# Glaciohound/Chimera-ST

Measured on AMD Instinct MI355X. Metric: train utterances/sec, MuST-C EN-DE s2t_transformer_m, 1/2/4/8 MI355X, higher is better.
Workload: dtype bf16

## Files before the change

chimera-st_amd/csrc/gemm.hip:

```cpp
#include "gemm_common.h"
#include <vector>
#include <stdlib.h>
#include <string.h>
#include <type_traits>

namespace {
using namespace cstg;

template <int BM_, int BN_, int WM_, int WN_, int KV_ = 8>
struct Cfg {
  static constexpr int BM = BM_, BN = BN_, WM = WM_, WN = WN_, NT = 64 * WM_ * WN_, TM = BM_ / WM_ / 32, TN = BN_ / WN_ / 32;
  static constexpr int KV = KV_;
  static_assert(BM_ <= GEMM_MAX_BM && GEMM_MAX_BM % BM_ == 0, "conv0.hip (cst_conv_row_limits) sizes live frames from GEMM_MAX_BM");
};
using CfgSmall = Cfg<128, 128, 2, 2>;
using CfgSkinny = Cfg<64, 64, 2, 2>;
using CfgNarrowN = Cfg<128, 64, 2, 2>;
using CfgNarrowM = Cfg<64, 128, 2, 2>;
using CfgLarge = Cfg<256, 256, 4, 4>;

template <typename T, bool A_KMAJOR, bool B_KMAJOR, bool SEG, typename C, bool CS = false>
__global__ __launch_bounds__(C::NT) void gemm_kernel(GemmParams p) {
  constexpr int BM = C::BM, BN = C::BN, NTHREADS = C::NT, TM = C::TM, TN = C::TN;
  constexpr int VEC = DT<T>::VEC;
  constexpr int KV = C::KV, BK = KV * VEC;
  constexpr int LDK = BK + VEC;
  constexpr int LDMA = sizeof(T) == 2 ? BM + 32 : BM + VEC;
  constexpr int LDMB = sizeof(T) == 2 ? BN + 32 : BN + VEC;
  constexpr int A_ELEMS = A_KMAJOR ? BM * LDK : BK * LDMA;
  constexpr int B_ELEMS = B_KMAJOR ? BN * LDK : BK * LDMB;
  constexpr int MVA = BM / VEC, MVB = BN / VEC;
  constexpr int NVA = BM * KV / NTHREADS, NVB = BN * KV / NTHREADS;
  extern __shared__ __attribute__((aligned(16))) char smem_raw[];
  T* smem = reinterpret_cast<T*>(smem_raw);
  constexpr int STAGE = A_ELEMS + B_ELEMS;

  const int tid = threadIdx.x, lane = tid & 63, wave = tid >> 6;
  const int wm = wave / C::WN, wn = wave % C::WN;

  const int ntiles = p.tiles_m * p.tiles_n;
  int tm, tn, z;
  if (p.split_order) {
    const int total = ntiles * p.splits, L = (int)blockIdx.x + (int)gridDim.x * (int)blockIdx.z;
    const int q = total / 8, r = total % 8, xcd = L % 8, loc = L / 8;
    const int item = (xcd < r ? xcd * (q + 1) : r * (q + 1) + (xcd - r) * q) + loc;
    z = item / ntiles;
    const int t = item % ntiles;
    tm = t / p.tiles_n;
    tn = t % p.tiles_n;
  } else {
    int id = blockIdx.x;
    {
      const int q = ntiles / 8, r = ntiles % 8, xcd = id % 8, loc = id / 8;
      id = (xcd < r ? xcd * (q + 1) : r * (q + 1) + (xcd - r) * q) + loc;
    }
    constexpr int GROUP_M = 8;
    const int per_group = GROUP_M * p.tiles_n;
    const int grp = id / per_group, rem = id % per_group;
    const int gm0 = grp * GROUP_M;
    const int gsz = (p.tiles_m - gm0 < GROUP_M) ? (p.tiles_m - gm0) : GROUP_M;
    tm = gm0 + rem % gsz;
    tn = rem / gsz;
    z = blockIdx.z;
  }
  const int64_t m0 = (int64_t)tm * BM, n0 = (int64_t)tn * BN;

  const int split = z % p.splits;
  const int64_t bidx = z / p.splits;
  const int64_t b0 = bidx / p.batch1, b1 = bidx % p.batch1;
  const T* A = (const T*)p.A + b0 * p.sa0 + b1 * p.sa1;
  const T* B = (const T*)p.B + b0 * p.sb0 + b1 * p.sb1;
  const int64_t cofs = b0 * p.sc0 + b1 * p.sc1;
  const int64_t bofs = b0 * p.sbias0 + b1 * p.sbias1;

  int ktiles = (int)((p.K + BK - 1) / BK);
  const int kfull = (int)(p.K / BK);
  if (p.k_len) {
    typedef const __attribute__((address_space(4))) int32_t* cptr_t;
    const int kl = ((cptr_t)p.k_len)[b0];
    const int live = kl <= 0 ? 0 : (kl + BK - 1) / BK;
    ktiles = live < ktiles ? live : ktiles;
  }
  const int per = (ktiles + p.splits - 1) / p.splits;
  const int kt0 = split * per;
  const int kt1 = (kt0 + per < ktiles) ? kt0 + per : ktiles;

  u32x4 ra[NVA], rb[NVB];
  const T* pa[NVA];
  const T* pb[NVB];
  int ka[NVA], kb[NVB];
  int aq[NVA], ar[NVA], bq[NVB], br[NVB];
#pragma unroll
  for (int i = 0; i < NVA; ++i) {
    const int v = tid + NTHREADS * i;
    if (A_KMAJOR) {
      int64_t row = m0 + v / KV;
      row = row < p.M ? row : p.M - 1;
      ka[i] = kt0 * BK + (v % KV) * VEC;
      if (SEG && p.a_seg) { aq[i] = ka[i] / (int)p.a_seg; ar[i] = ka[i] % (int)p.a_seg; pa[i] = A + row * p.lda; }
      else { aq[i] = 0; ar[i] = 0; pa[i] = A + row * p.lda + ka[i]; }
    } else {
      int64_t m = m0 + (int64_t)(v % MVA) * VEC;
      m = m < p.M ? m : p.M - VEC;
      ka[i] = kt0 * BK + v / MVA;
      aq[i] = 0; ar[i] = 0;
      pa[i] = A + (int64_t)ka[i] * p.lda + segaddr(m, p.a_seg, p.a_seg_stride);
    }
  }
#pragma unroll
  for (int i = 0; i < NVB; ++i) {
    const int v = tid + NTHREADS * i;
    if (B_KMAJOR) {
      int64_t row = n0 + v / KV;
      row = row < p.N ? row : p.N - 1;
      kb[i] = kt0 * BK + (v % KV) * VEC;
      if (SEG && p.b_seg) { bq[i] = kb[i] / (int)p.b_seg; br[i] = kb[i] % (int)p.b_seg; pb[i] = B + row * p.ldb; }
      else { bq[i] = 0; br[i] = 0; pb[i] = B + row * p.ldb + kb[i]; }
    } else {
      int64_t n = n0 + (int64_t)(v % MVB) * VEC;
      n = n < p.N ? n : p.N - VEC;
      kb[i] = kt0 * BK + v / MVB;
      bq[i] = 0; br[i] = 0;
      pb[i] = B + (int64_t)kb[i] * p.ldb + segaddr(n, p.b_seg, p.b_seg_stride);
    }
  }
  const int64_t step_a = A_KMAJOR ? (int64_t)BK : (int64_t)BK * p.lda;
  const int64_t step_b = B_KMAJOR ? (int64_t)BK : (int64_t)BK * p.ldb;

  auto load_tile = [&](auto tail_tag) {
    constexpr bool TAIL = decltype(tail_tag)::value;
    const u32x4 zero = {0, 0, 0, 0};
#pragma unroll
    for (int i = 0; i < NVA; ++i) {
      const T* qa = pa[i];
      if (SEG && A_KMAJOR && p.a_seg) qa = pa[i] + (int64_t)aq[i] * p.a_seg_stride + ar[i];
      if (TAIL) {
        const bool oka = ka[i] < p.K;
        const u32x4 va = *reinterpret_cast<const u32x4*>(oka ? qa : A);
        ra[i] = oka ? va : zero;
      } else {
        ra[i] = *reinterpret_cast<const u32x4*>(qa);
      }
      ka[i] += BK;
      if (SEG && A_KMAJOR && p.a_seg) { ar[i] += BK; while (ar[i] >= (int)p.a_seg) { ar[i] -= (int)p.a_seg; ++aq[i]; } }
      else pa[i] += step_a;
    }
#pragma unroll
    for (int i = 0; i < NVB; ++i) {
      const T* qb = pb[i];
      if (SEG && B_KMAJOR && p.b_seg) qb = pb[i] + (int64_t)bq[i] * p.b_seg_stride + br[i];
      if (TAIL) {
        const bool okb = kb[i] < p.K;
        const u32x4 vb = *reinterpret_cast<const u32x4*>(okb ? qb : B);
        rb[i] = okb ? vb : zero;
      } else {
        rb[i] = *reinterpret_cast<const u32x4*>(qb);
      }
      kb[i] += BK;
      if (SEG && B_KMAJOR && p.b_seg) { br[i] += BK; while (br[i] >= (int)p.b_seg) { br[i] -= (int)p.b_seg; ++bq[i]; } }
      else pb[i] += step_b;
    }
  };
  auto load_any = [&](int kt) {
    if (kt < kfull) load_tile(std::false_type{});
    else load_tile(std::true_type{});
  };
  static_assert(!CS || (!A_KMAJOR && NTHREADS % MVA == 0), "a thread must stage the same columns of an mn-major A in every vector");
  const bool do_cs = CS && tn == 0;
  float cs[VEC];
#pragma unroll
  for (int e = 0; e < VEC; ++e) cs[e] = 0.0f;
  auto store_tile = [&](int buf) {
#pragma unroll
    for (int i = 0; i < NVA; ++i) {
      const int v = tid + NTHREADS * i;
      T* da = smem + buf * STAGE + (A_KMAJOR ? (v / KV) * LDK + (v % KV) * VEC : (v / MVA) * LDMA + (v % MVA) * VEC);
      *reinterpret_cast<u32x4*>(da) = ra[i];
      if (CS && do_cs) {
        if (sizeof(T) == 2) {
#pragma unroll
          for (int e = 0; e < 4; ++e) {
            cs[2 * e] += __uint_as_float(ra[i][e] << 16);
            cs[2 * e + 1] += __uint_as_float(ra[i][e] & 0xffff0000u);
          }
        } else {
#pragma unroll
          for (int e = 0; e < 4; ++e) cs[e] += __uint_as_float(ra[i][e]);
        }
      }
    }
#pragma unroll
    for (int i = 0; i < NVB; ++i) {
      const int v = tid + NTHREADS * i;
      T* db = smem + buf * STAGE + A_ELEMS + (B_KMAJOR ? (v / KV) * LDK + (v % KV) * VEC : (v / MVB) * LDMB + (v % MVB) * VEC);
      *reinterpret_cast<u32x4*>(db) = rb[i];
    }
  };

  f32x16 acc[TM][TN];
#pragma unroll
  for (int i = 0; i < TM; ++i)
#pragma unroll
    for (int j = 0; j < TN; ++j)
#pragma unroll
      for (int r = 0; r < 16; ++r) acc[i][j][r] = 0.0f;

  constexpr int KLIST_MAX = 1000;
  __shared__ int klist[KLIST_MAX];
  __shared__ int klist_n;
  const bool kskip = !SEG && BK == 64 && p.k_live != nullptr && per <= KLIST_MAX;
  int nk = kt1 > kt0 ? kt1 - kt0 : 0;
  if (kskip) {
    if (wave == 0) {
      int total = 0;
      for (int base = 0; base < ktiles; base += 64) {
        const int kt = base + lane;
        total += __builtin_popcountll(__builtin_amdgcn_ballot_w64(kt < ktiles && p.k_live[kt] == p.k_epoch));
      }
      const int lo = (int)(((int64_t)total * split) / p.splits), hi = (int)(((int64_t)total * (split + 1)) / p.splits);
      int seen = 0, n = 0;
      for (int base = 0; base < ktiles && seen < hi; base += 64) {
        const int kt = base + lane;
        const bool live = kt < ktiles && p.k_live[kt] == p.k_epoch;
        const uint64_t m = __builtin_amdgcn_ballot_w64(live);
        const int idx = seen + __builtin_popcountll(m & ((1ull << lane) - 1ull));
        if (live && idx >= lo && idx < hi) klist[idx - lo] = kt;
        seen += __builtin_popcountll(m);
      }
      n = hi - lo;
      if (lane == 0) klist_n = n;
    }
    __syncthreads();
    nk = klist_n;
  }
  if (p.m_live) {
    typedef const __attribute__((address_space(4))) uint32_t* cptr_t;
    cptr_t ml = (cptr_t)p.m_live;
    const int t0 = (int)(m0 >> 6), t1 = (int)((((m0 + BM < p.M) ? m0 + BM : p.M) + 63) >> 6);
    bool live = false;
    for (int t = t0; t < t1; ++t) live |= ml[t] == p.m_epoch;
    if (!live) nk = 0;
  }
  if (p.m_len) {
    typedef const __attribute__((address_space(4))) int32_t* cptr_t;
    if (m0 >= (int64_t)((cptr_t)p.m_len)[b0]) nk = 0;
  }
  int pos = kt0;
  auto fetch = [&](int kt) {
    const int d = kt - pos;
    if (d) {
#pragma unroll
      for (int i = 0; i < NVA; ++i) { pa[i] += (int64_t)d * step_a; ka[i] += d * BK; }
#pragma unroll
      for (int i = 0; i < NVB; ++i) { pb[i] += (int64_t)d * step_b; kb[i] += d * BK; }
    }
    load_any(kt);
    pos = kt + 1;
  };
  auto tile_at = [&](int it) { return kskip ? klist[it] : kt0 + it; };

  if (nk > 0) {
    fetch(tile_at(0));
    store_tile(0);
  }
  __syncthreads();
  int cur = 0;
  const int lrow = lane & 31, lk = 8 * (lane >> 5);
  constexpr int WROWS = TM * 32, WCOLS = TN * 32;
  for (int it = 0; it < nk; ++it) {
    const bool more = it + 1 < nk;
    if (more) fetch(tile_at(it + 1));
    const T* sa = smem + cur * STAGE;
    const T* sb = sa + A_ELEMS;
#pragma unroll
    for (int kk = 0; kk < BK; kk += 16) {
      Frag<T> fa[TM], fb[TN];
#pragma unroll
      for (int i = 0; i < TM; ++i) {
        if (A_KMAJOR) frag_load_contig(fa[i], sa + (wm * WROWS + i * 32 + lrow) * LDK + kk + lk);
        else frag_load_tr(fa[i], sa, LDMA, wm * WROWS + i * 32, kk + lk, kk + lk + 4, lane);
      }
#pragma unroll
      for (int j = 0; j < TN; ++j) {
        if (B_KMAJOR) frag_load_contig(fb[j], sb + (wn * WCOLS + j * 32 + lrow) * LDK + kk + lk);
        else frag_load_tr(fb[j], sb, LDMB, wn * WCOLS + j * 32, kk + lk, kk + lk + 4, lane);
      }
#pragma unroll
      for (int i = 0; i < TM; ++i)
#pragma unroll
        for (int j = 0; j < TN; ++j) mma16(acc[i][j], fa[i], fb[j]);
    }
    if (more) store_tile(cur ^ 1);
    __syncthreads();
    cur ^= 1;
  }

  if (CS && do_cs) {
    float* red = reinterpret_cast<float*>(smem_raw);
#pragma unroll
    for (int e = 0; e < VEC; ++e) red[(tid / MVA) * BM + (tid % MVA) * VEC + e] = cs[e];
    __syncthreads();
    if (tid < BM && m0 + tid < p.M) {
      float tot = 0.0f;
      for (int r = 0; r < NTHREADS / MVA; ++r) tot += red[r * BM + tid];
      if (p.splits > 1) p.colsum_ws[((int64_t)bidx * p.splits + split) * p.M + m0 + tid] = tot;
      else DT<T>::st((T*)p.colsum + bidx * p.M + m0 + tid, tot);
    }
  }

  constexpr int LDC = BN + 4;
  constexpr int VPR = BN / 8;
  constexpr int NPASS = BM / 64;
  constexpr int ITERS = 64 * VPR / NTHREADS;
  float* stage = reinterpret_cast<float*>(smem_raw);
  float* wsp = p.splits > 1 ? p.ws + ((int64_t)z) * p.M * p.N : nullptr;
  const bool ws_vec = (p.N % 4) == 0;
#pragma unroll
  for (int ps = 0; ps < NPASS; ++ps) {
    __syncthreads();
#pragma unroll
    for (int i = 0; i < TM; ++i) {
      const int trow = wm * WROWS + i * 32;
      if (trow / 64 == ps) {
#pragma unroll
        for (int j = 0; j < TN; ++j)
#pragma unroll
          for (int r = 0; r < 16; ++r)
            stage[(trow - 64 * ps + acc_row(r, lane)) * LDC + wn * WCOLS + j * 32 + lrow] = acc[i][j][r];
      }
    }
    __syncthreads();
#pragma unroll 2
    for (int it = 0; it < ITERS; ++it) {
      const int v = tid + NTHREADS * it;
      const int rl = v / VPR, cl = (v % VPR) * 8;
      const int64_t row = m0 + 64 * ps + rl, col = n0 + cl;
      if (row >= p.M || col >= p.N) continue;
      float x[8];
      {
        const f32x4 a = *reinterpret_cast<const f32x4*>(stage + rl * LDC + cl);
        const f32x4 b = *reinterpret_cast<const f32x4*>(stage + rl * LDC + cl + 4);
        x[0] = a[0]; x[1] = a[1]; x[2] = a[2]; x[3] = a[3]; x[4] = b[0]; x[5] = b[1]; x[6] = b[2]; x[7] = b[3];
      }
      const bool full = col + 8 <= p.N;
      if (wsp) {
        if (full && ws_vec) store8(wsp + row * p.N + col, x);
        else
          for (int e = 0; e < 8 && col + e < p.N; ++e) wsp[row * p.N + col + e] = x[e];
      } else if (full && p.vec_epi) {
        epilogue_store8<T>(p, cofs, bofs, row, col, x);
      } else {
        for (int e = 0; e < 8 && col + e < p.N; ++e) epilogue_store<T>(p, cofs, bofs, row, col + e, x[e]);
      }
    }
  }
}

template <int N>
__device__ __forceinline__ void wait_vmcnt() { asm volatile("s_waitcnt vmcnt(%0)" ::"n"(N) : "memory"); }

template <typename T, bool A_KMAJOR, bool B_KMAJOR, typename C, int NS>
__global__ __launch_bounds__(C::NT) void gemm_glds_kernel(GemmParams p) {
  constexpr int BM = C::BM, BN = C::BN, NTHREADS = C::NT, TM = C::TM, TN = C::TN, NWAVES = C::NT / 64;
  constexpr int ES = sizeof(T), VEC = DT<T>::VEC, BK = 128 / ES;
  constexpr int A_BYTES = A_KMAJOR ? BM * 128 : BK * BM * ES;
  constexpr int B_BYTES = B_KMAJOR ? BN * 128 : BK * BN * ES;
  constexpr int STAGE_BYTES = A_BYTES + B_BYTES;
  constexpr int GA = A_BYTES / 1024 / NWAVES, GB = B_BYTES / 1024 / NWAVES;
  extern __shared__ __attribute__((aligned(16))) char smem_raw[];

  const int tid = threadIdx.x, lane = tid & 63, wave = tid >> 6;
  const int wm = wave / C::WN, wn = wave % C::WN;
  const int ntiles = p.tiles_m * p.tiles_n;
  int id = blockIdx.x;
  {
    const int q = ntiles / 8, r = ntiles % 8, xcd = id % 8, loc = id / 8;
    id = (xcd < r ? xcd * (q + 1) : r * (q + 1) + (xcd - r) * q) + loc;
  }
  constexpr int GROUP_M = 8;
  int tm, tn;
  {
    const int per_group = GROUP_M * p.tiles_n;
    const int grp = id / per_group, rem = id % per_group;
    const int gm0 = grp * GROUP_M;
    const int gsz = (p.tiles_m - gm0 < GROUP_M) ? (p.tiles_m - gm0) : GROUP_M;
    tm = gm0 + rem % gsz;
    tn = rem / gsz;
  }
  const int64_t m0 = (int64_t)tm * BM, n0 = (int64_t)tn * BN;
  const int z = blockIdx.z;
  const int split = z % p.splits;
  const int64_t bidx = z / p.splits;
  const int64_t b0 = bidx / p.batch1, b1 = bidx % p.batch1;
  const T* A = (const T*)p.A + b0 * p.sa0 + b1 * p.sa1;
  const T* B = (const T*)p.B + b0 * p.sb0 + b1 * p.sb1;
  const int64_t cofs = b0 * p.sc0 + b1 * p.sc1;
  const int64_t bofs = b0 * p.sbias0 + b1 * p.sbias1;
  const int ktiles = (int)((p.K + BK - 1) / BK);
  const int kfull = (int)(p.K / BK);
  const int per = (ktiles + p.splits - 1) / p.splits;
  const int kt0 = split * per;
  const int kt1 = (kt0 + per < ktiles) ? kt0 + per : ktiles;
  int nt = kt1 - kt0;
  if (p.m_len) {
    typedef const __attribute__((address_space(4))) int32_t* cptr_t;
    if (m0 >= (int64_t)((cptr_t)p.m_len)[b0]) nt = 0;
  }

  const T* pa[GA];
  const T* pb[GB];
  int ka[GA], kb[GB];
#pragma unroll
  for (int i = 0; i < GA; ++i) {
    const int g = wave + NWAVES * i;
    if (A_KMAJOR) {
      const int r = 8 * g + (lane >> 3), c = (lane & 7) ^ ((r >> 1) & 7);
      int64_t row = m0 + r;
      row = row < p.M ? row : p.M - 1;
      ka[i] = kt0 * BK + c * VEC;
      pa[i] = A + row * p.lda + ka[i];
    } else {
      constexpr int RB = BM * ES, RPG = 1024 / RB > 0 ? 1024 / RB : 1, CPR = RB / 16;
      const int kl = g * RPG + (lane * 16) / RB, pc = ((lane * 16) % RB) / 16;
      const int c = ES == 2 ? (pc ^ (4 * (kl & 3))) : pc;
      int64_t m = m0 + (int64_t)c * VEC;
      m = m < p.M ? m : p.M - VEC;
      ka[i] = kt0 * BK + kl;
      pa[i] = A + (int64_t)ka[i] * p.lda + segaddr(m, p.a_seg, p.a_seg_stride);
      (void)CPR;
    }
  }
#pragma unroll
  for (int i = 0; i < GB; ++i) {
    const int g = wave + NWAVES * i;
    if (B_KMAJOR) {
      const int r = 8 * g + (lane >> 3), c = (lane & 7) ^ ((r >> 1) & 7);
      int64_t row = n0 + r;
      row = row < p.N ? row : p.N - 1;
      kb[i] = kt0 * BK + c * VEC;
      pb[i] = B + row * p.ldb + kb[i];
    } else {
      constexpr int RB = BN * ES, RPG = 1024 / RB > 0 ? 1024 / RB : 1;
      const int kl = g * RPG + (lane * 16) / RB, pc = ((lane * 16) % RB) / 16;
      const int c = ES == 2 ? (pc ^ (4 * (kl & 3))) : pc;
      int64_t n = n0 + (int64_t)c * VEC;
      n = n < p.N ? n : p.N - VEC;
      kb[i] = kt0 * BK + kl;
      pb[i] = B + (int64_t)kb[i] * p.ldb + segaddr(n, p.b_seg, p.b_seg_stride);
    }
  }
  const int64_t step_a = A_KMAJOR ? (int64_t)BK : (int64_t)BK * p.lda;
  const int64_t step_b = B_KMAJOR ? (int64_t)BK : (int64_t)BK * p.ldb;

  auto issue = [&](int kt, int stage) {
    char* sbase = smem_raw + stage * STAGE_BYTES;
    if (kt < kfull) {
#pragma unroll
      for (int i = 0; i < GA; ++i) {
        __builtin_amdgcn_global_load_lds((const __attribute__((address_space(1))) void*)pa[i],
                                         (__attribute__((address_space(3))) void*)(sbase + (wave + NWAVES * i) * 1024), 16, 0, 0);
        pa[i] += step_a;
        ka[i] += BK;
      }
#pragma unroll
      for (int i = 0; i < GB; ++i) {
        __builtin_amdgcn_global_load_lds((const __attribute__((address_space(1))) void*)pb[i],
                                         (__attribute__((address_space(3))) void*)(sbase + A_BYTES + (wave + NWAVES * i) * 1024), 16, 0, 0);
        pb[i] += step_b;
        kb[i] += BK;
      }
    } else {
      const u32x4 zero = {0, 0, 0, 0};
#pragma unroll
      for (int i = 0; i < GA; ++i) {
        const bool ok = ka[i] < p.K;
        const u32x4 v = *reinterpret_cast<const u32x4*>(ok ? pa[i] : A);
        *reinterpret_cast<u32x4*>(sbase + (wave + NWAVES * i) * 1024 + lane * 16) = ok ? v : zero;
        pa[i] += step_a;
        ka[i] += BK;
      }
#pragma unroll
      for (int i = 0; i < GB; ++i) {
        const bool ok = kb[i] < p.K;
        const u32x4 v = *reinterpret_cast<const u32x4*>(ok ? pb[i] : B);
        *reinterpret_cast<u32x4*>(sbase + A_BYTES + (wave + NWAVES * i) * 1024 + lane * 16) = ok ? v : zero;
        pb[i] += step_b;
        kb[i] += BK;
      }
    }
  };

  f32x16 acc[TM][TN];
#pragma unroll
  for (int i = 0; i < TM; ++i)
#pragma unroll
    for (int j = 0; j < TN; ++j)
#pragma unroll
      for (int r = 0; r < 16; ++r) acc[i][j][r] = 0.0f;

  const int lrow = lane & 31, hi = lane >> 5;
  constexpr int WROWS = TM * 32, WCOLS = TN * 32;
  constexpr int G = GA + GB;

#pragma unroll
  for (int s = 0; s < NS - 1; ++s)
    if (s < nt) issue(kt0 + s, s);

  constexpr bool PIN = NTHREADS == 256 && TM == 4 && NS == 2 && A_KMAJOR && B_KMAJOR && sizeof(T) == 2;
// ... 28 lines not shown
        if (f < TM) frag_load_kswz(fa[buf][f], sa, wm * WROWS + f * 32 + lrow, kk * 16 + 8 * hi);
        else frag_load_kswz(fb[buf][f - TM], sb, wn * WCOLS + (f - TM) * 32 + lrow, kk * 16 + 8 * hi);
      };
#pragma unroll
      for (int f = 0; f < NFR; ++f) read_one(f, 0, 0);
      __builtin_amdgcn_sched_barrier(0);
#pragma unroll
      for (int kk = 0; kk < 4; ++kk) {
#pragma unroll
        for (int sl = 0; sl < NSLOT; ++sl) {
#pragma unroll
          for (int u = 0; u < 2; ++u) {
            const int m = 2 * sl + u, i = m / TN, j = m % TN;
            mma16(acc[i][j], fb[kk & 1][j], fa[kk & 1][i]);
          }
          if (kk < 3) {
            if (sl < NFR) read_one(sl, kk + 1, (kk + 1) & 1);
            if (sl == 0 && NFR > NSLOT) {
#pragma unroll
              for (int f = NSLOT; f < NFR; ++f) read_one(f, kk + 1, (kk + 1) & 1);
            }
          }
          if (kk * NSLOT + sl < G && dma_ok) issue_one(kk * NSLOT + sl, nbase);
          __builtin_amdgcn_sched_barrier(0);
        }
      }
    }
  } else
  for (int it = 0; it < nt; ++it) {
    const int issued = (it + NS - 1 < nt) ? it + NS - 1 : nt;
    if (NS > 2 && issued - it - 1 == NS - 2) wait_vmcnt<(NS - 2) * G>();
    else wait_vmcnt<0>();
    __builtin_amdgcn_s_barrier();
    if (it + NS - 1 < nt) issue(kt0 + it + NS - 1, (it + NS - 1) % NS);
    const char* sbase = smem_raw + (it % NS) * STAGE_BYTES;
    const T* sa = reinterpret_cast<const T*>(sbase);
    const T* sb = reinterpret_cast<const T*>(sbase + A_BYTES);
#pragma unroll
    for (int kk = 0; kk < BK; kk += 16) {
      Frag<T> fa[TM], fb[TN];
#pragma unroll
      for (int i = 0; i < TM; ++i) {
        if (A_KMAJOR) {
          const int r = wm * WROWS + i * 32 + lrow;
          frag_load_kswz(fa[i], sa, r, kk + 8 * hi);
        } else {
          frag_load_tr_swz(fa[i], sa, BM, wm * WROWS + i * 32, kk + 8 * hi, lane);
        }
      }
#pragma unroll
      for (int j = 0; j < TN; ++j) {
        if (B_KMAJOR) {
          const int r = wn * WCOLS + j * 32 + lrow;
          frag_load_kswz(fb[j], sb, r, kk + 8 * hi);
        } else {
          frag_load_tr_swz(fb[j], sb, BN, wn * WCOLS + j * 32, kk + 8 * hi, lane);
        }
      }
#pragma unroll
      for (int i = 0; i < TM; ++i)
#pragma unroll
        for (int j = 0; j < TN; ++j) mma16(acc[i][j], fa[i], fb[j]);
    }
  }

  float* wsp = p.splits > 1 ? p.ws + ((int64_t)z) * p.M * p.N : nullptr;
  const bool ws_vec = (p.N % 4) == 0;
  if constexpr (PIN) {
    constexpr int LDW = WCOLS + 4, VPRW = WCOLS / 8, RITER = 32 * VPRW / 64;
    static_assert(4 * 32 * LDW * 4 <= NS * STAGE_BYTES && (32 * VPRW) % 64 == 0, "the four waves' images live in the stage buffers");
    __syncthreads();
    float* img = reinterpret_cast<float*>(smem_raw) + wave * (32 * LDW);
#pragma unroll
    for (int i = 0; i < TM; ++i) {
#pragma unroll
      for (int j = 0; j < TN; ++j)
#pragma unroll
        for (int q = 0; q < 4; ++q) {
          const f32x4 v = {acc[i][j][4 * q], acc[i][j][4 * q + 1], acc[i][j][4 * q + 2], acc[i][j][4 * q + 3]};
          *reinterpret_cast<f32x4*>(img + lrow * LDW + j * 32 + 8 * q + 4 * hi) = v;
        }
#pragma unroll 2
      for (int tv = 0; tv < RITER; ++tv) {
        const int v = tv * 64 + lane;
        const int rl = v / VPRW, cl = (v % VPRW) * 8;
        const int64_t row = m0 + wm * WROWS + i * 32 + rl, col = n0 + wn * WCOLS + cl;
        if (row >= p.M || col >= p.N) continue;
        float x[8];
        {
          const f32x4 a = *reinterpret_cast<const f32x4*>(img + rl * LDW + cl);
          const f32x4 b = *reinterpret_cast<const f32x4*>(img + rl * LDW + cl + 4);
          x[0] = a[0]; x[1] = a[1]; x[2] = a[2]; x[3] = a[3]; x[4] = b[0]; x[5] = b[1]; x[6] = b[2]; x[7] = b[3];
        }
        const bool full = col + 8 <= p.N;
        if (wsp) {
          if (full && ws_vec) store8(wsp + row * p.N + col, x);
          else
            for (int e = 0; e < 8 && col + e < p.N; ++e) wsp[row * p.N + col + e] = x[e];
        } else if (full && p.vec_epi) {
          epilogue_store8<T>(p, cofs, bofs, row, col, x);
        } else {
          for (int e = 0; e < 8 && col + e < p.N; ++e) epilogue_store<T>(p, cofs, bofs, row, col + e, x[e]);
        }
      }
    }
    return;
  }
  constexpr int LDC = BN + 4;
  constexpr int VPR = BN / 8;
  constexpr int NPASS = BM / 64;
  constexpr int ITERS = 64 * VPR / NTHREADS;
  float* stage = reinterpret_cast<float*>(smem_raw);
#pragma unroll
  for (int ps = 0; ps < NPASS; ++ps) {
    __syncthreads();
#pragma unroll
    for (int i = 0; i < TM; ++i) {
      const int trow = wm * WROWS + i * 32;
      if (trow / 64 == ps) {
#pragma unroll
        for (int j = 0; j < TN; ++j)
#pragma unroll
          for (int r = 0; r < 16; ++r)
            stage[(trow - 64 * ps + acc_row(r, lane)) * LDC + wn * WCOLS + j * 32 + lrow] = acc[i][j][r];
      }
    }
    __syncthreads();
#pragma unroll 2
    for (int itv = 0; itv < ITERS; ++itv) {
      const int v = tid + NTHREADS * itv;
      const int rl = v / VPR, cl = (v % VPR) * 8;
      const int64_t row = m0 + 64 * ps + rl, col = n0 + cl;
      if (row >= p.M || col >= p.N) continue;
      float x[8];
      {
        const f32x4 a = *reinterpret_cast<const f32x4*>(stage + rl * LDC + cl);
        const f32x4 b = *reinterpret_cast<const f32x4*>(stage + rl * LDC + cl + 4);
        x[0] = a[0]; x[1] = a[1]; x[2] = a[2]; x[3] = a[3]; x[4] = b[0]; x[5] = b[1]; x[6] = b[2]; x[7] = b[3];
      }
      const bool full = col + 8 <= p.N;
      if (wsp) {
        if (full && ws_vec) store8(wsp + row * p.N + col, x);
        else
          for (int e = 0; e < 8 && col + e < p.N; ++e) wsp[row * p.N + col + e] = x[e];
      } else if (full && p.vec_epi) {
        epilogue_store8<T>(p, cofs, bofs, row, col, x);
      } else {
        for (int e = 0; e < 8 && col + e < p.N; ++e) epilogue_store<T>(p, cofs, bofs, row, col + e, x[e]);
      }
    }
  }
}

template <typename T>
__global__ void splitk_reduce_kernel(GemmParams p) {
  const int64_t total = p.M * p.N;
  const int64_t bidx = blockIdx.y;
  const int64_t b0 = bidx / p.batch1, b1 = bidx % p.batch1;
  const int64_t cofs = b0 * p.sc0 + b1 * p.sc1;
  const int64_t bofs = b0 * p.sbias0 + b1 * p.sbias1;
  const float* ws = p.ws + bidx * p.splits * total;
  if (p.colsum) {
    for (int64_t m = (int64_t)blockIdx.x * blockDim.x + threadIdx.x; m < p.M; m += (int64_t)gridDim.x * blockDim.x) {
      float v = 0.0f;
      for (int s = 0; s < p.splits; ++s) v += p.colsum_ws[(bidx * p.splits + s) * p.M + m];
      DT<T>::st((T*)p.colsum + bidx * p.M + m, v);
    }
  }
  if (p.vec_epi && (p.N % 8) == 0) {
    const int64_t total8 = total >> 3;
    for (int64_t i8 = (int64_t)blockIdx.x * blockDim.x + threadIdx.x; i8 < total8; i8 += (int64_t)gridDim.x * blockDim.x) {
      const float* src = ws + i8 * 8;
      float v[8] = {0.0f, 0.0f, 0.0f, 0.0f, 0.0f, 0.0f, 0.0f, 0.0f};
      int sp = 0;
      for (; sp + 4 <= p.splits; sp += 4) {
        f32x4 a[4][2];
#pragma unroll
        for (int u = 0; u < 4; ++u) {
          a[u][0] = *reinterpret_cast<const f32x4*>(src + (int64_t)(sp + u) * total);
          a[u][1] = *reinterpret_cast<const f32x4*>(src + (int64_t)(sp + u) * total + 4);
        }
#pragma unroll
        for (int u = 0; u < 4; ++u)
#pragma unroll
          for (int e = 0; e < 4; ++e) { v[e] += a[u][0][e]; v[4 + e] += a[u][1][e]; }
      }
      for (; sp < p.splits; ++sp) {
        const f32x4 a0 = *reinterpret_cast<const f32x4*>(src + (int64_t)sp * total), a1 = *reinterpret_cast<const f32x4*>(src + (int64_t)sp * total + 4);
#pragma unroll
        for (int e = 0; e < 4; ++e) { v[e] += a0[e]; v[4 + e] += a1[e]; }
      }
      const int64_t i = i8 * 8, row = i / p.N;
      epilogue_store8<T>(p, cofs, bofs, row, i - row * p.N, v);
    }
    return;
  }
  for (int64_t i = (int64_t)blockIdx.x * blockDim.x + threadIdx.x; i < total; i += (int64_t)gridDim.x * blockDim.x) {
    float v = 0.0f;
    for (int s = 0; s < p.splits; ++s) v += ws[s * total + i];
    epilogue_store<T>(p, cofs, bofs, i / p.N, i % p.N, v);
  }
}

template <typename T, bool AK, bool BK_, bool SEG, typename C>
int launch(GemmParams p, int64_t M, int64_t N, int64_t nbatch, hipStream_t s) {
  constexpr int VEC = DT<T>::VEC;
  constexpr int BKc = C::KV * VEC, LDK = BKc + VEC;
  constexpr int LDMA = sizeof(T) == 2 ? C::BM + 32 : C::BM + VEC, LDMB = sizeof(T) == 2 ? C::BN + 32 : C::BN + VEC;
  constexpr int A_ELEMS = AK ? C::BM * LDK : BKc * LDMA;
  constexpr int B_ELEMS = BK_ ? C::BN * LDK : BKc * LDMB;
  size_t lds = 2 * (size_t)(A_ELEMS + B_ELEMS) * sizeof(T);
  const size_t stage_bytes = (size_t)64 * (C::BN + 4) * sizeof(float);
  if (lds < stage_bytes) lds = stage_bytes;
  static bool attr_set = false;
  if (!attr_set) {
    (void)hipFuncSetAttribute(reinterpret_cast<const void*>(&gemm_kernel<T, AK, BK_, SEG, C>), hipFuncAttributeMaxDynamicSharedMemorySize, 160 * 1024 - 4096);
    attr_set = true;
  }
  p.tiles_m = (int)cst_ceil_div(M, C::BM);
  p.tiles_n = (int)cst_ceil_div(N, C::BN);
  p.split_order = (p.splits > 1 && nbatch == 1) ? 1 : 0;
  dim3 grid(p.tiles_m * p.tiles_n, 1, (unsigned)(nbatch * p.splits));
  if constexpr (!AK && !BK_ && !SEG && C::NT <= 256) {
    if (p.colsum) {
      static bool attr_cs = false;
      if (!attr_cs) {
        (void)hipFuncSetAttribute(reinterpret_cast<const void*>(&gemm_kernel<T, AK, BK_, SEG, C, true>), hipFuncAttributeMaxDynamicSharedMemorySize, 160 * 1024 - 4096);
        attr_cs = true;
      }
      hipLaunchKernelGGL((gemm_kernel<T, AK, BK_, SEG, C, true>), grid, dim3(C::NT), lds, s, p);
      return cst_check_launch("cst_gemm");
    }
  }
  if (p.colsum) { cst_set_error("cst_gemm: internal: column sums requested from a configuration that does not build them"); return CST_ERR_UNSUPPORTED; }
  hipLaunchKernelGGL((gemm_kernel<T, AK, BK_, SEG, C>), grid, dim3(C::NT), lds, s, p);
  return cst_check_launch("cst_gemm");
}

template <typename T, bool AK, bool BK_, typename C, int NS>
int launch_glds(GemmParams p, int64_t M, int64_t N, int64_t nbatch, hipStream_t s) {
  constexpr int ES = sizeof(T), BKc = 128 / ES;
  constexpr int A_BYTES = AK ? C::BM * 128 : BKc * C::BM * ES, B_BYTES = BK_ ? C::BN * 128 : BKc * C::BN * ES;
  size_t lds = (size_t)NS * (A_BYTES + B_BYTES);
  const size_t stage_bytes = (size_t)64 * (C::BN + 4) * sizeof(float);
  if (lds < stage_bytes) lds = stage_bytes;
  static bool attr_set = false;
  if (!attr_set) {
    (void)hipFuncSetAttribute(reinterpret_cast<const void*>(&gemm_glds_kernel<T, AK, BK_, C, NS>), hipFuncAttributeMaxDynamicSharedMemorySize, 160 * 1024);
    attr_set = true;
  }
  p.tiles_m = (int)cst_ceil_div(M, C::BM);
  p.tiles_n = (int)cst_ceil_div(N, C::BN);
  dim3 grid(p.tiles_m * p.tiles_n, 1, (unsigned)(nbatch * p.splits));
  hipLaunchKernelGGL((gemm_glds_kernel<T, AK, BK_, C, NS>), grid, dim3(C::NT), lds, s, p);
  return cst_check_launch("cst_gemm");
}


struct GemmSwitches {
  bool no_klive;
  int group_m;
  bool no_narrow;
  bool no_4w;
  bool experiment;
  const char* force_cfg;
};

GemmSwitches gemm_switches() {
  static const GemmSwitches once = [] {
    GemmSwitches w;
    w.no_klive = getenv("CST_GEMM_NO_KLIVE") != nullptr;
    const char* gm = getenv("CST_GEMM8P_GROUP_M");
    w.group_m = gm && atoi(gm) > 0 ? atoi(gm) : 4;
    w.no_narrow = getenv("CST_GEMM_NO_NARROW") != nullptr;
    w.no_4w = getenv("CST_GEMM_NO_4W") != nullptr;
    w.experiment = getenv("CST_GEMM_EXPERIMENT") != nullptr;
    w.force_cfg = nullptr;
    return w;
  }();
  GemmSwitches w = once;
  if (w.experiment) {
    const char* f = getenv("CST_GEMM_FORCE_CFG");
    w.force_cfg = f && *f ? f : nullptr;
  }
  return w;
}

enum class Family { Reg, Dma, Persistent8, FourWave };
enum class Tile { Small, Large, Skinny, NarrowN, NarrowM, Big4, Big4N, Unknown };
enum class Colsum { None, Fused, Separate };
using CfgBig4 = Cfg<256, 256, 2, 2>;
using CfgBig4N = Cfg<256, 192, 2, 2>;

struct GemmRoute {
  Family family;
  Tile tile;
  bool bf16, ak, bk;
  bool seg;
  int stages;
  int splits;
  Colsum colsum;
};

struct TileDims { int bm, bn, nt; };
template <typename C> constexpr TileDims dims_of() { return {C::BM, C::BN, C::NT}; }
constexpr TileDims kTileDims[] = {dims_of<CfgSmall>(),   dims_of<CfgLarge>(), dims_of<CfgSkinny>(), dims_of<CfgNarrowN>(),
                                  dims_of<CfgNarrowM>(), dims_of<CfgBig4>(),  dims_of<CfgBig4N>(),  {0, 0, 0}};

bool use_large(const cst_gemm_desc* d, bool seg, int splits) {
  if (seg) return false;
  const int64_t tiles = cst_ceil_div(d->M, 256) * cst_ceil_div(d->N, 256) * d->batch0 * d->batch1 * splits;
  return d->M >= 256 && d->N >= 256 && tiles >= 200;
}

int choose_splits(const cst_gemm_desc* d) {
  if (d->split_k > 1) return d->split_k;
  if (d->split_k == 0 || d->split_k == 1) return 1;
  const int bk = d->dtype == CST_BF16 ? 64 : 32;
  const int64_t ktiles = cst_ceil_div(d->K, bk);
  const int64_t nb = d->batch0 * d->batch1;
  if (d->M >= 256 && d->N >= 256) {
    const int64_t tl = cst_ceil_div(d->M, 256) * cst_ceil_div(d->N, 256) * nb;
    if (tl >= 200) return 1;
    int64_t s = 256 / tl;
    if (s > ktiles / 16) s = ktiles / 16;
    if (s > 32) s = 32;
    if (s >= 1 && tl * s >= 200) return (int)s;
  }
  const int64_t tiles = cst_ceil_div(d->M, 128) * cst_ceil_div(d->N, 128) * nb;
  if (tiles >= 256 || ktiles < 16) return 1;
  const int64_t cap = ktiles / 8 < 32 ? ktiles / 8 : 32;
  int64_t s1 = 256 / tiles, s2 = 512 / tiles;
  if (s1 > cap) s1 = cap;
  if (s2 > cap) s2 = cap;
  if (s1 < 1) s1 = 1;
  if (s2 < 1) s2 = 1;
  const int64_t s = (2.0 / (double)s2 < 0.9 / (double)s1) ? s2 : s1;
  return (int)s;
}

struct Forced { const char* name; bool kk; Family family; Tile tile; int stages; };
const Forced kForced[] = {
    {"small", false, Family::Reg, Tile::Small, 0},     {"narrowm", false, Family::Reg, Tile::NarrowM, 0},
    {"narrown", false, Family::Reg, Tile::NarrowN, 0}, {"skinny", false, Family::Reg, Tile::Skinny, 0},
    {"large", false, Family::Reg, Tile::Large, 0},     {"big4r", false, Family::Reg, Tile::Big4, 0},
    {"skinny4", true, Family::Dma, Tile::Skinny, 4},   {"skinny2", true, Family::Dma, Tile::Skinny, 2},
    {"small2", true, Family::Dma, Tile::Small, 2},     {"small3", true, Family::Dma, Tile::Small, 3},
    {"big4", true, Family::Dma, Tile::Big4, 2},        {"big4n", true, Family::Dma, Tile::Big4N, 2},
    {"big4r", true, Family::Reg, Tile::Big4, 0},       {"large", true, Family::Reg, Tile::Large, 0},
    {"8p", true, Family::Persistent8, Tile::Large, 0}, {"4w", true, Family::FourWave, Tile::Big4N, 0},
};

GemmRoute gemm_route(const cst_gemm_desc* d, const GemmParams& p, const GemmSwitches& sw) {
  GemmRoute r;
  r.bf16 = d->dtype == CST_BF16;
  r.ak = d->a_kmajor != 0;
  r.bk = d->b_kmajor != 0;
  r.seg = (r.ak && d->a_seg) || (r.bk && d->b_seg);
  r.stages = 2;
  r.splits = choose_splits(d);
  const bool kk = r.ak && r.bk, mm = !r.ak && !r.bk;
  const bool large = use_large(d, r.seg, r.splits);
  const int64_t nbatch = d->batch0 * d->batch1;
  r.colsum = !d->colsum ? Colsum::None : (mm && !d->a_seg && !d->b_seg && !large) ? Colsum::Fused : Colsum::Separate;
  auto take = [&r](Family f, Tile t, int stages = 2) { r.family = f; r.tile = t; r.stages = stages; return r; };

  if (!sw.no_narrow && !r.seg && !large && kk && d->N <= 64 && d->M > 256) return take(Family::Dma, Tile::NarrowN);
  if (!sw.no_narrow && !r.seg && !large && mm && d->M <= 64 && d->N > 256) return take(Family::Reg, Tile::NarrowM);

  GemmParams q = p;
  q.splits = r.splits;
  const bool unsplit1 = !r.seg && nbatch == 1 && r.splits == 1;
  if (sw.force_cfg && r.bf16 && !r.seg && nbatch == 1 && (mm || (kk && r.splits == 1))) {
    for (const Forced& f : kForced) {
      if (f.kk != kk || strcmp(f.name, sw.force_cfg) != 0) continue;
      if (f.family == Family::Persistent8 && !cst_gemm8p_supported(q, r.ak, r.bk, nbatch)) break;
      if (f.family == Family::FourWave && !cst_gemm4w_supported(q, r.ak, r.bk, nbatch)) break;
      return take(f.family, f.tile, f.stages);
    }
    return take(Family::Reg, Tile::Unknown);
  }

  const bool mid8p = kk && unsplit1 && d->M >= 256 && d->N >= 256 && cst_ceil_div(d->M, 256) * cst_ceil_div(d->N, 256) >= 150;
  if (kk && unsplit1 && (d->M <= 256 || (!large && !mid8p && cst_ceil_div(d->M, 128) * cst_ceil_div(d->N, 128) < 256))) {
    const bool two_stage = d->M > 256 && cst_ceil_div(d->M, 64) * cst_ceil_div(d->N, 64) > 512;
    return take(Family::Dma, Tile::Skinny, two_stage ? 2 : 4);
  }
  if (r.bf16 && !r.seg && !d->colsum) {
    if (!sw.no_4w && cst_gemm4w_supported(q, r.ak, r.bk, nbatch)) return take(Family::FourWave, Tile::Big4N);
    if (r.ak && (!d->dact || (!d->resid && !d->aux_out)) && (large || mid8p) && cst_gemm8p_supported(q, r.ak, r.bk, nbatch))
      return take(Family::Persistent8, Tile::Large);
  }
  const Tile t = large ? Tile::Large : Tile::Small;
  if (r.seg) return take(Family::Reg, Tile::Small);
  return take(kk && !d->colsum ? Family::Dma : Family::Reg, t);
}

void route_text(const GemmRoute& r, char* out, int64_t n) {
  const TileDims t = kTileDims[(int)r.tile];
  const char* dt = r.bf16 ? "bf16" : "f32";
  const char a = r.ak ? 'k' : 'm', b = r.bk ? 'k' : 'm';
  switch (r.family) {
    case Family::Reg:
      snprintf(out, (size_t)n, "reg %s %c%c%s %dx%d nt%d%s split%d", dt, a, b, r.seg ? " seg" : "", t.bm, t.bn, t.nt,
               r.colsum == Colsum::Fused ? " colsum" : "", r.splits);
      break;
    case Family::Dma: snprintf(out, (size_t)n, "glds %s %c%c %dx%d nt%d ns%d split%d", dt, a, b, t.bm, t.bn, t.nt, r.stages, r.splits); break;
    case Family::Persistent8: snprintf(out, (size_t)n, "8p %c%c", a, b); break;
    case Family::FourWave: snprintf(out, (size_t)n, "4w"); break;
  }
}

}

extern "C" int64_t cst_colsum_workspace(int64_t rows, int64_t cols);
extern "C" int cst_colsum_typed(const void* x, int64_t ldx, void* out, void* workspace, int64_t rows, int64_t cols, int dtype, int out_dtype, cst_stream stream);
extern "C" int cst_colsum_typed_live(const void* x, int64_t ldx, void* out, void* workspace, int64_t rows, int64_t cols, int dtype, int out_dtype,
                                     const uint32_t* row_live, uint32_t epoch, cst_stream stream);

namespace {

int validate(const cst_gemm_desc* d) {
  CST_REQUIRE(d && d->A && d->B && d->C, "cst_gemm: null operand");
  CST_REQUIRE(d->dtype == CST_F32 || d->dtype == CST_BF16, "cst_gemm: bad dtype %d", d->dtype);
  CST_REQUIRE(d->c_dtype == d->dtype || d->c_dtype == CST_F32, "cst_gemm: c_dtype must be dtype or f32");
  CST_REQUIRE(d->M > 0 && d->N > 0 && d->K > 0, "cst_gemm: empty problem M=%lld N=%lld K=%lld", (long long)d->M,
              (long long)d->N, (long long)d->K);
  const int vec = d->dtype == CST_BF16 ? 8 : 4;
  if (d->a_kmajor) CST_REQUIRE(d->K % vec == 0 && d->lda % vec == 0, "cst_gemm: k-major A needs K,lda %% %d == 0 (K=%lld lda=%lld)", vec, (long long)d->K, (long long)d->lda);
  else CST_REQUIRE(d->M % vec == 0 && d->lda % vec == 0, "cst_gemm: mn-major A needs M,lda %% %d == 0 (M=%lld lda=%lld)", vec, (long long)d->M, (long long)d->lda);
  if (d->b_kmajor) CST_REQUIRE(d->K % vec == 0 && d->ldb % vec == 0, "cst_gemm: k-major B needs K,ldb %% %d == 0 (K=%lld ldb=%lld)", vec, (long long)d->K, (long long)d->ldb);
  else CST_REQUIRE(d->N % vec == 0 && d->ldb % vec == 0, "cst_gemm: mn-major B needs N,ldb %% %d == 0 (N=%lld ldb=%lld)", vec, (long long)d->N, (long long)d->ldb);
  CST_REQUIRE(d->a_seg % vec == 0 && d->b_seg % vec == 0 && d->a_seg_stride % vec == 0 && d->b_seg_stride % vec == 0,
              "cst_gemm: segment sizes must be multiples of %d", vec);
  CST_REQUIRE(((uintptr_t)d->A % 16 == 0) && ((uintptr_t)d->B % 16 == 0), "cst_gemm: A/B must be 16-byte aligned");
  CST_REQUIRE(d->sa0 % vec == 0 && d->sa1 % vec == 0 && d->sb0 % vec == 0 && d->sb1 % vec == 0, "cst_gemm: batch strides of A/B must be multiples of %d", vec);
  CST_REQUIRE(d->batch0 >= 1 && d->batch1 >= 1, "cst_gemm: batch counts must be >= 1");
  CST_REQUIRE(!d->dact || d->aux_in, "cst_gemm: dact needs aux_in");
  CST_REQUIRE(d->drop_p >= 0.0f && d->drop_p < 1.0f, "cst_gemm: drop_p must be in [0, 1)");
  CST_REQUIRE(d->drop_p == 0.0f || d->batch0 * d->batch1 == 1, "cst_gemm: fused dropout needs an unbatched problem");
  CST_REQUIRE(!d->colsum || (!d->a_kmajor && !d->a_seg), "cst_gemm: colsum needs an mn-major, unsegmented A");
  return CST_OK;
}

GemmParams fill_params(const cst_gemm_desc* d, const GemmSwitches& sw) {
  GemmParams p;
  p.M = d->M; p.N = d->N; p.K = d->K;
  p.A = d->A; p.lda = d->lda; p.a_seg = d->a_seg; p.a_seg_stride = d->a_seg_stride;
  p.B = d->B; p.ldb = d->ldb; p.b_seg = d->b_seg; p.b_seg_stride = d->b_seg_stride;
  p.C = d->C; p.ldc = d->ldc;
  p.bias = d->bias; p.bias_mode = d->bias ? d->bias_mode : CST_BIAS_NONE; p.sbias0 = d->sbias0; p.sbias1 = d->sbias1;
  p.act = d->act;
  p.aux_out = d->aux_out; p.ld_aux_out = d->ld_aux_out;
  p.dact = d->dact; p.aux_in = d->aux_in; p.ld_aux_in = d->ld_aux_in;
  p.resid = d->resid; p.ld_resid = d->ld_resid;
  p.alpha = d->alpha;
  p.drop_thr = d->drop_p > 0.0f ? cst_drop_thr16(d->drop_p) : 0u;
  p.drop_key = d->drop_key;
  p.drop_scale = d->drop_p > 0.0f ? 1.0f / (1.0f - d->drop_p) : 1.0f;
  p.drop_row0 = 0;
  p.batch1 = d->batch1;
  p.sa0 = d->sa0; p.sa1 = d->sa1; p.sb0 = d->sb0; p.sb1 = d->sb1; p.sc0 = d->sc0; p.sc1 = d->sc1;
  p.c_f32 = (d->c_dtype == CST_F32 && d->dtype != CST_F32) ? 1 : 0;
  {
    auto al16 = [](const void* q) { return q == nullptr || ((uintptr_t)q % 16) == 0; };
    bool ok = d->ldc % 8 == 0 && d->sc0 % 8 == 0 && d->sc1 % 8 == 0 && al16(d->C) && al16(d->bias) && al16(d->aux_out) && al16(d->aux_in) && al16(d->resid);
    if (d->bias && d->bias_mode == CST_BIAS_COL) ok = ok && d->sbias0 % 8 == 0 && d->sbias1 % 8 == 0;
    if (d->aux_out) ok = ok && d->ld_aux_out % 8 == 0;
    if (d->aux_in) ok = ok && d->ld_aux_in % 8 == 0;
    if (d->resid) ok = ok && d->ld_resid % 8 == 0;
    if (d->drop_p > 0.0f) ok = ok && (d->N % 2 == 0);
    p.vec_epi = ok ? 1 : 0;
  }
  p.tiles_m = p.tiles_n = 0;
  p.split_order = 0;
  p.sched = nullptr;
  p.gperm_full = 0;
  p.mrot = 0;
  p.k_live = sw.no_klive ? nullptr : d->k_live;
  p.k_epoch = d->k_epoch;
  p.m_live = sw.no_klive ? nullptr : d->m_live;
  p.m_epoch = d->m_epoch;
  p.k_len = sw.no_klive ? nullptr : d->k_len;
  p.m_len = sw.no_klive ? nullptr : d->m_len;
  p.group_m = sw.group_m;
  p.splits = 1;
  p.ws = nullptr;
  p.colsum = nullptr;
  p.colsum_ws = nullptr;
  return p;
}

int64_t route_workspace(const cst_gemm_desc* d, const GemmRoute& r) {
  const int64_t s = r.splits, nb = d->batch0 * d->batch1;
  int64_t bytes = s > 1 ? s * d->M * d->N * nb * (int64_t)sizeof(float) : 0;
  if (r.colsum == Colsum::Fused) bytes += s > 1 ? s * d->M * nb * (int64_t)sizeof(float) : 0;
  else if (r.colsum == Colsum::Separate) bytes += cst_colsum_workspace(d->K, d->M);
  return bytes;
}

int take_route(const cst_gemm_desc* d, const GemmSwitches& sw, GemmParams& p, GemmRoute& r) {
  r = gemm_route(d, p, sw);
  const int64_t nbatch = d->batch0 * d->batch1;
  CST_REQUIRE(r.colsum != Colsum::Separate || (nbatch == 1 && d->M % 8 == 0 && d->lda % 8 == 0),
              "cst_gemm: colsum of this configuration runs as a separate column sum: unbatched, M and lda multiples of 8");
  CST_REQUIRE(cst_ceil_div(d->M, 128) * cst_ceil_div(d->N, 128) < (1ll << 31) && nbatch * r.splits < 65536, "cst_gemm: grid too large");
  p.splits = r.splits;
  p.colsum = r.colsum == Colsum::Fused ? d->colsum : nullptr;
#ifdef CST_TRACE
  if (p.splits == 1 && d->workspace) p.ws = (float*)d->workspace;
#endif
  const int64_t need = route_workspace(d, r);
  if (need > 0 && (!d->workspace || d->workspace_bytes < need)) {
    if (r.splits > 1) cst_set_error("cst_gemm: split_k=%d needs %lld workspace bytes, got %lld", r.splits, (long long)need, (long long)d->workspace_bytes);
    else cst_set_error("cst_gemm: colsum needs %lld workspace bytes, got %lld", (long long)need, (long long)d->workspace_bytes);
    return CST_ERR_WORKSPACE;
  }
  if (r.splits > 1) {
    p.ws = (float*)d->workspace;
    p.colsum_ws = p.ws + (int64_t)r.splits * d->M * d->N * nbatch;
  }
  return CST_OK;
}

template <typename W>
bool read_back(hipStream_t s, const W* dev, int64_t n, std::vector<W>& host) {
  host.resize((size_t)n);
  return hipStreamSynchronize(s) == hipSuccess && hipMemcpy(host.data(), dev, sizeof(W) * n, hipMemcpyDeviceToHost) == hipSuccess;
}

struct Work { double flops, bytes; };
Work credited_work(const cst_gemm_desc* d, const GemmParams& p, hipStream_t s) {
  double frac = 1.0;
  if (cst_prof_is_on()) {
    std::vector<uint32_t> st;
    std::vector<int32_t> len;
    const int64_t mtiles = cst_ceil_div(d->M, 256);
    if (p.k_live && read_back(s, p.k_live, cst_ceil_div(d->K, 64), st)) {
      int64_t live = 0;
      for (uint32_t v : st) live += v == p.k_epoch;
      frac *= (double)live / (double)st.size();
    }
    if (p.k_len && read_back(s, p.k_len, d->batch0, len)) {
      double sum = 0.0;
      for (int32_t v : len) sum += (double)(v < 0 ? 0 : (v < d->K ? v : d->K));
      frac *= sum / ((double)d->batch0 * (double)d->K);
    }
    if (p.m_len && read_back(s, p.m_len, d->batch0, len)) {
      double live = 0.0;
      for (int32_t v : len) {
        const int64_t t = v <= 0 ? 0 : cst_ceil_div((int64_t)v, 256);
        live += (double)(t < mtiles ? t : mtiles);
      }
      frac *= live / ((double)d->batch0 * (double)mtiles);
    }
    if (p.m_live && read_back(s, p.m_live, cst_ceil_div(d->M, 64), st)) {
      const int64_t nt = (int64_t)st.size();
      int64_t live = 0;
      for (int64_t t = 0; t < mtiles; ++t) {
        bool l = false;
        for (int64_t i = 4 * t; i < 4 * t + 4 && i < nt; ++i) l |= st[i] == p.m_epoch;
        live += l;
      }
      frac *= (double)live / (double)mtiles;
    }
  }
  const double nbatch = (double)(d->batch0 * d->batch1), esz = (double)cst_dtype_size(d->dtype);
  return {2.0 * (double)d->M * (double)d->N * (double)d->K * nbatch * frac,
          ((double)d->M * d->K + (double)d->N * d->K) * esz * nbatch * frac + (double)d->M * d->N * cst_dtype_size(d->c_dtype) * nbatch};
}

int unlaunchable(const GemmRoute& r, const GemmSwitches& sw) {
  if (r.tile == Tile::Unknown) {
    cst_set_error("cst_gemm: unknown CST_GEMM_FORCE_CFG %s", sw.force_cfg ? sw.force_cfg : "");
    return CST_ERR_BAD_ARG;
  }
  if (r.family == Family::Reg && r.colsum == Colsum::Fused && kTileDims[(int)r.tile].nt > 256) {
    cst_set_error("cst_gemm: internal: column sums requested from a configuration that does not build them");
    return CST_ERR_UNSUPPORTED;
  }
  return CST_OK;
}

template <typename T, bool SEG, typename C>
int launch_reg(const GemmRoute& r, const GemmParams& p, int64_t nbatch, hipStream_t s) {
  return r.ak ? (r.bk ? launch<T, true, true, SEG, C>(p, p.M, p.N, nbatch, s) : launch<T, true, false, SEG, C>(p, p.M, p.N, nbatch, s))
              : (r.bk ? launch<T, false, true, SEG, C>(p, p.M, p.N, nbatch, s) : launch<T, false, false, SEG, C>(p, p.M, p.N, nbatch, s));
}

constexpr int arm(Family f, Tile t, int stages = 0) { return ((int)f << 8) | ((int)t << 4) | stages; }

template <typename T>
int launch_route(const GemmRoute& r, const GemmParams& p, int64_t nbatch, hipStream_t s, const GemmSwitches& sw) {
  constexpr bool HOOK = std::is_same<T, bf16_t>::value;
  const int64_t M = p.M, N = p.N;
  switch (arm(r.family, r.tile, r.family == Family::Dma ? r.stages : 0)) {
    case arm(Family::Persistent8, Tile::Large): return cst_gemm8p_launch(p, r.ak, r.bk, nbatch, s);
    case arm(Family::FourWave, Tile::Big4N): return cst_gemm4w_launch(p, s);
    case arm(Family::Reg, Tile::Small): return r.seg ? launch_reg<T, true, CfgSmall>(r, p, nbatch, s) : launch_reg<T, false, CfgSmall>(r, p, nbatch, s);
    case arm(Family::Reg, Tile::Large): return launch_reg<T, false, CfgLarge>(r, p, nbatch, s);
    case arm(Family::Reg, Tile::NarrowM): return launch<T, false, false, false, CfgNarrowM>(p, M, N, nbatch, s);
    case arm(Family::Dma, Tile::Small, 2): return launch_glds<T, true, true, CfgSmall, 2>(p, M, N, nbatch, s);
    case arm(Family::Dma, Tile::Large, 2): return launch_glds<T, true, true, CfgLarge, 2>(p, M, N, nbatch, s);
    case arm(Family::Dma, Tile::NarrowN, 2): return launch_glds<T, true, true, CfgNarrowN, 2>(p, M, N, nbatch, s);
    case arm(Family::Dma, Tile::Skinny, 2): return launch_glds<T, true, true, CfgSkinny, 2>(p, M, N, nbatch, s);
    case arm(Family::Dma, Tile::Skinny, 4): return launch_glds<T, true, true, CfgSkinny, 4>(p, M, N, nbatch, s);
    case arm(Family::Reg, Tile::NarrowN): if constexpr (HOOK) return launch<T, false, false, false, CfgNarrowN>(p, M, N, nbatch, s); break;
    case arm(Family::Reg, Tile::Skinny): if constexpr (HOOK) return launch<T, false, false, false, CfgSkinny>(p, M, N, nbatch, s); break;
    case arm(Family::Reg, Tile::Big4):
      if constexpr (HOOK) return r.ak ? launch<T, true, true, false, CfgBig4>(p, M, N, nbatch, s) : launch<T, false, false, false, CfgBig4>(p, M, N, nbatch, s);
      break;
    case arm(Family::Dma, Tile::Small, 3): if constexpr (HOOK) return launch_glds<T, true, true, CfgSmall, 3>(p, M, N, nbatch, s); break;
    case arm(Family::Dma, Tile::Big4, 2): if constexpr (HOOK) return launch_glds<T, true, true, CfgBig4, 2>(p, M, N, nbatch, s); break;
    case arm(Family::Dma, Tile::Big4N, 2): if constexpr (HOOK) return launch_glds<T, true, true, CfgBig4N, 2>(p, M, N, nbatch, s); break;
    default: break;
  }
  const int rc = unlaunchable(r, sw);
  if (rc == CST_OK) cst_set_error("cst_gemm: internal: a route without a launch arm");
  return rc == CST_OK ? CST_ERR_UNSUPPORTED : rc;
}

int finish(const cst_gemm_desc* d, const GemmRoute& r, const GemmParams& p, cst_stream stream) {
  const int64_t nbatch = d->batch0 * d->batch1;
  if (p.splits > 1 && d->defer_reduce) {
    CST_REQUIRE((nbatch == 1 || !d->colsum) && d->alpha == 1.0f && !d->bias && !d->act && !d->dact && !d->aux_out && !d->resid && d->drop_p == 0.0f && d->ldc == d->N &&
                    d->N % 8 == 0 && r.colsum != Colsum::Separate,
                "cst_gemm: defer_reduce needs a plain epilogue and a dense C (batched: no colsum; the slabs are [batch][split][M][N])");
    return CST_OK;
  }
  int rc = CST_OK;
  if (p.splits > 1) {
    const int64_t total = d->M * d->N;
    const int64_t work = (p.vec_epi && d->N % 8 == 0) ? total / 8 : total;
    int blocks = (int)(cst_ceil_div(work, 256) < 2048 ? cst_ceil_div(work, 256) : 2048);
    dim3 grid(blocks, (unsigned)nbatch);
    if (d->dtype == CST_BF16) hipLaunchKernelGGL(splitk_reduce_kernel<bf16_t>, grid, dim3(256), 0, (hipStream_t)stream, p);
    else hipLaunchKernelGGL(splitk_reduce_kernel<float>, grid, dim3(256), 0, (hipStream_t)stream, p);
    rc = cst_check_launch("cst_gemm split-k reduce");
  }
  if (rc == CST_OK && r.colsum == Colsum::Separate) {
    void* cws = (char*)d->workspace + (p.splits > 1 ? (int64_t)p.splits * d->M * d->N * (int64_t)sizeof(float) : 0);
    rc = p.k_live ? cst_colsum_typed_live(d->A, d->lda, d->colsum, cws, d->K, d->M, d->dtype, d->dtype, p.k_live, p.k_epoch, stream)
                  : cst_colsum_typed(d->A, d->lda, d->colsum, cws, d->K, d->M, d->dtype, d->dtype, stream);
  }
  return rc;
}

int gemm_one(const cst_gemm_desc* d, cst_stream stream) {
  int rc = validate(d);
  if (rc != CST_OK) return rc;
  const GemmSwitches sw = gemm_switches();
  GemmParams p = fill_params(d, sw);
  GemmRoute r;
  if ((rc = take_route(d, sw, p, r)) != CST_OK) return rc;
  hipStream_t s = (hipStream_t)stream;
  const int64_t nbatch = d->batch0 * d->batch1;
  const Work w = credited_work(d, p, s);
  CstProfScope prof(CST_K_GEMM, s, w.flops, w.bytes);
  rc = r.bf16 ? launch_route<bf16_t>(r, p, nbatch, s, sw) : launch_route<float>(r, p, nbatch, s, sw);
  if (cst_prof_is_on())
    prof.tag("M=%lld N=%lld K=%lld b=%lld a%c b%c split=%d%s%s%s%s%s%s%s", (long long)d->M, (long long)d->N, (long long)d->K, (long long)nbatch, r.ak ? 'k' : 'm',
             r.bk ? 'k' : 'm', p.splits, d->bias ? " bias" : "", d->act ? " act" : "", d->aux_out ? " aux_out" : "", d->dact ? " dact" : "",
             d->resid ? " resid" : "", d->drop_p > 0 ? " drop" : "", (d->k_live || d->m_live || d->k_len || d->m_len) ? " live" : "");
  return rc != CST_OK ? rc : finish(d, r, p, stream);
}

GemmRoute query_route(const cst_gemm_desc* d) {
  const GemmSwitches sw = gemm_switches();
  return gemm_route(d, fill_params(d, sw), sw);
}

}

extern "C" int cst_gemm_splits(const cst_gemm_desc* d) { return d ? query_route(d).splits : 0; }

extern "C" int cst_gemm_colsum_is_fused(const cst_gemm_desc* d) { return d && query_route(d).colsum == Colsum::Fused ? 1 : 0; }

extern "C" int64_t cst_gemm_workspace(const cst_gemm_desc* d) { return route_workspace(d, query_route(d)); }

extern "C" int cst_gemm_route(const cst_gemm_desc* d, char* out, int64_t out_bytes) {
  if (out && out_bytes > 0) out[0] = 0;
  int rc = validate(d);
  if (rc != CST_OK) return rc;
  CST_REQUIRE(out && out_bytes > 0, "cst_gemm_route: no room for the text");
  const GemmSwitches sw = gemm_switches();
  GemmParams p = fill_params(d, sw);
  GemmRoute r;
  if ((rc = take_route(d, sw, p, r)) != CST_OK) return rc;
  if ((rc = unlaunchable(r, sw)) != CST_OK) return rc;
  route_text(r, out, out_bytes);
  return CST_OK;
}

extern "C" int cst_gemm(const cst_gemm_desc* d, cst_stream stream) { return gemm_one(d, stream); }
```

chimera-st_amd/functional.py:

```python
import os as _os
import weakref as _weakref

import torch

from . import kernels as K
from . import lib as L

_ACT = {None: L.ACT_NONE, "none": L.ACT_NONE, "relu": L.ACT_RELU, "gelu": L.ACT_GELU}


def _flat2d(x):
    return x.reshape(-1, x.shape[-1]).contiguous()


def _vec(dtype):
    return 8 if dtype == torch.bfloat16 else 4


def _with_tiles(t, tiles):
    if t.is_contiguous():
        t._cst_live_tiles = (tiles[0], tiles[1], t.data_ptr(), t.numel(), t.shape[-1], t._version)
        if t._base is not None:
            t._base._cst_live_tiles = t._cst_live_tiles
    return t
# ... 23 lines not shown


class _WeightTransposes:

    def __init__(self):
        self.entries = {}
        self.tables = {}
        self.refreshes = 0
        self.persistent = {}

    def register_storage(self, owner, flat):
        sp = flat.untyped_storage().data_ptr()
        self.persistent[sp] = _weakref.ref(owner)
        _weakref.finalize(owner, self._drop_storage, sp)

    def _drop_storage(self, sp):
        self.persistent.pop(sp, None)
        for k in [k for k, e in self.entries.items() if e[4] == sp]:
            del self.entries[k]
        self.tables.clear()

    def invalidate(self):
        self.entries.clear()
        self.tables.clear()

    @staticmethod
    def _src(e):
        return e[0]() if isinstance(e[0], _weakref.ref) else e[0]

    def get(self, w):
        from .optim import PARAM_EPOCH
        epoch = PARAM_EPOCH[0]
        key = (w.data_ptr(), tuple(w.shape), w.dtype)
        e = self.entries.get(key)
        if e is not None and self._src(e) is None:
            del self.entries[key]
            self.tables.pop((w.device, w.dtype), None)
            e = None
        if e is None:
            sp = w.untyped_storage().data_ptr()
            owner = self.persistent.get(sp)
            if owner is not None and owner() is not None:
                src = w.detach()
                parts = getattr(w, "_cst_parts", None)
                if parts is not None:
                    src._cst_parts = parts
            elif isinstance(w, torch.nn.Parameter):
                src, sp = _weakref.ref(w), None
            else:
                return K.transpose2d(w)
            e = self.entries[key] = [src, K.transpose2d(w), _wversion(w), epoch, sp]
            self.tables.pop((w.device, w.dtype), None)
            return e[1]
        if e[2] != _wversion(w):
            K.transpose2d(w, e[1])
            e[2], e[3] = _wversion(w), epoch
            return e[1]
        if e[3] != epoch:
            kind = (w.device, w.dtype)
            stale = []
            for k, v in list(self.entries.items()):
                t = self._src(v)
                if t is None or t.data_ptr() != k[0]:
                    del self.entries[k]
                    self.tables.pop(kind, None)
                elif t.device == w.device and k[2] == w.dtype and v[3] != epoch:
                    stale.append(v)
            ids = [id(v) for v in stale]
            t = self.tables.get(kind)
            if t is None or t[5] != ids:
                t = self.tables[kind] = K.transpose_table([(self._src(v), v[1]) for v in stale]) + (ids,)
            K.transpose2d_multi(t)
            self.refreshes += 1
            for v in stale:
                v[2], v[3] = _wversion(self._src(v)), epoch
        return e[1]


WEIGHT_TRANSPOSES = _WeightTransposes()


def _may_defer(*params):
    if not K.DEFER.on:
        return False
    for w in params:
        if w is None:
            continue
        for p in (getattr(w, "_cst_parts_params", None) or (w,)):
            if not isinstance(p, torch.nn.Parameter) or p.grad is not None or getattr(p, "_cst_shared", False):
                return False
    return True


def _grad_out(w):
    if _os.environ.get("CST_NO_GRAD_SLOT"):
        return None
    from .optim import grad_slot
    return grad_slot(w)


class _LinearFn(torch.autograd.Function):
    @staticmethod
    def forward(ctx, x, weight, bias, resid, act, drop_p, drop_key):
        x2 = _flat2d(x)
        M, Kd = x2.shape
        N = weight.shape[0]
        w = weight.contiguous()
        ctx.bias_obj = bias
        Np = (N + _vec(x.dtype) - 1) // _vec(x.dtype) * _vec(x.dtype)
        if Np != N:
            wp = torch.zeros(Np, Kd, dtype=w.dtype, device=w.device)
            wp[:N] = w
            w = wp
            if bias is not None:
                bp = torch.zeros(Np, dtype=bias.dtype, device=bias.device)
                bp[:N] = bias
                bias = bp
            assert resid is None and drop_p == 0.0
        y = torch.empty(M, Np, dtype=x.dtype, device=x.device)
        z = torch.empty_like(y) if act != L.ACT_NONE else None
        r2 = _flat2d(resid) if resid is not None else None
        K.gemm(x2, w, y, M, Np, Kd, a_kmajor=1, b_kmajor=1, lda=Kd, ldb=Kd, ldc=Np, bias=bias, act=act, aux_out=z, ld_aux_out=Np,
               resid=r2, ld_resid=Np, split_k=1, drop_p=drop_p, drop_key=drop_key)
        ctx.save_for_backward(x2, w, z)
        ctx.act, ctx.has_bias, ctx.has_resid = act, bias is not None, resid is not None
        ctx.drop = (drop_p, drop_key)
        ctx.xshape, ctx.N = x.shape, N
        if Np != N:
            y = y[:, :N].contiguous()
        return y.view(*x.shape[:-1], N)

    @staticmethod
    def backward(ctx, dy):
        return _linear_backward(ctx, dy, None)


def _dx_gemm(dz, w, M, *, use_wt, like, resid=None, dact=L.ACT_NONE, aux_in=None, drop=(0.0, 0), m_live=None):
    n_out, n_in = w.shape
    dx = torch.empty(M, n_in, dtype=like.dtype, device=like.device)
    b, b_kmajor, ldb = (WEIGHT_TRANSPOSES.get(w), 1, n_out) if use_wt else (w, 0, n_in)
    K.gemm(dz, b, dx, M, n_in, n_out, a_kmajor=1, b_kmajor=b_kmajor, lda=n_out, ldb=ldb, ldc=n_in, dact=dact, aux_in=aux_in, ld_aux_in=n_in,
           resid=resid, ld_resid=n_in, split_k=1, drop_p=drop[0], drop_key=drop[1], m_live=m_live)
    return dx


def _dw_gemm(dz, x2, w, bias_obj, M, *, db_in_dw, live, dz_travels_on, allow_slot=True, allow_defer=True):
    n_out, n_in = w.shape
    dw = _grad_out(w) if allow_slot else None
    if dw is None:
        dw = torch.empty(n_out, n_in, dtype=w.dtype, device=w.device)
    db = torch.empty(n_out, dtype=w.dtype, device=w.device) if db_in_dw else None
    may = allow_defer and _may_defer(w, bias_obj if db_in_dw else None)
    big = not may or not K.dw_colsum_is_fused(n_out, n_in, M, w.dtype) or dz_travels_on
    K.side_gemm(big, (dz, x2, live[0] if live is not None else None), dz, x2, dw, n_out, n_in, M, a_kmajor=0, b_kmajor=0, lda=n_out, ldb=n_in,
                ldc=n_in, split_k=-1, k_live=live, colsum=db, defer=may)
    return dw, db


def _drop_grad(dy2, drop, out_dtype, live, *, with_colsum, defer):
    if with_colsum and not _os.environ.get("CST_NO_DROP_COLSUM"):
        return K.dropout_colsum(dy2.contiguous(), drop[0], drop[1], out_dtype, live, defer=defer)
    return K.dropout(dy2.contiguous(), *drop), None


def _linear_backward(ctx, dy, dxp):
    x2, w, z = ctx.saved_tensors
    M, Kd = x2.shape
    Np, N = w.shape[0], ctx.N
    if dy is None:
        return dxp, None, None, None, None, None, None
    dy2 = _flat2d(dy)
    live = _tiles_of(dy, M)
    if Np != N:
        dyp = torch.zeros(M, Np, dtype=dy2.dtype, device=dy2.device)
        dyp[:, :N] = dy2
        dy2 = dyp
    db_fused = None
    want_db = ctx.has_bias and ctx.needs_input_grad[2]
    db_in_dw = want_db and ctx.needs_input_grad[1] and Np % 8 == 0 and not _os.environ.get("CST_NO_GEMM_COLSUM") and K.dw_colsum_is_fused(Np, Kd, M, w.dtype)
    may_b = want_db and Np == N and _may_defer(w, ctx.bias_obj)
    if ctx.drop[0] > 0.0:
        dy2, db_fused = _drop_grad(dy2, ctx.drop, w.dtype, live, defer=may_b,
                                   with_colsum=not db_in_dw and ctx.act == L.ACT_NONE and want_db and Np == N and N % 8 == 0)
    dz = K.act_bwd(dy2, z, ctx.act) if ctx.act != L.ACT_NONE else dy2
    dx = dw = db = dres = None
    if ctx.needs_input_grad[0]:
        dx = _dx_gemm(dz, w, M, use_wt=_want_wt(M, w), like=x2, resid=_flat2d(dxp) if dxp is not None else None,
                      m_live=live).view(ctx.xshape)
        if live is not None and dxp is None:
            dx = _with_tiles(dx, live)
    if ctx.needs_input_grad[1]:
        dw, db = _dw_gemm(dz, x2, w, ctx.bias_obj, M, db_in_dw=db_in_dw, live=live, dz_travels_on=dz.data_ptr() == dy.data_ptr() and ctx.has_resid,
                          allow_slot=Np == N, allow_defer=Np == N)
        dw = dw[:N]
        if db is not None:
            db = db[:N]
    if want_db and db is None:
        db = db_fused if db_fused is not None else K.colsum(dz, w.dtype, live, defer=may_b)[:N]
    if ctx.has_resid and ctx.needs_input_grad[3]:
        dres = dy
    return dx, dw, db, dres, None, None, None


class _LinearPassFn(torch.autograd.Function):

    @staticmethod
    def forward(ctx, x, weight, bias, act, drop_p, drop_key):
        y = _LinearFn.forward(ctx, x, weight, bias, None, act, drop_p, drop_key)
        ctx.set_materialize_grads(False)
        return y, x.view_as(x)

    @staticmethod
    def backward(ctx, dy, dxp):
        g = _linear_backward(ctx, dy, dxp)
        return g[0], g[1], g[2], None, None, None


def linear_pass(x, weight, bias=None, act=None, dropout_p=0.0):
    return _LinearPassFn.apply(x, weight, bias, _ACT[act], *_drop_args(dropout_p))


def linear(x, weight, bias=None, act=None, resid=None, dropout_p=0.0):
    return _LinearFn.apply(x, weight, bias, resid, _ACT[act], *_drop_args(dropout_p))


class _FFNFn(torch.autograd.Function):

    @staticmethod
    def forward(ctx, x, w1, b1, w2, b2, resid, act, p_act, key_act, p_out, key_out):
        x2 = _flat2d(x)
        M, d = x2.shape
        F_ = w1.shape[0]
        dout = w2.shape[0]
        z1 = torch.empty(M, F_, dtype=x.dtype, device=x.device)
        h = torch.empty_like(z1)
        K.gemm(x2, w1, h, M, F_, d, a_kmajor=1, b_kmajor=1, lda=d, ldb=d, ldc=F_, bias=b1, act=act, aux_out=z1, ld_aux_out=F_, split_k=1,
               drop_p=p_act, drop_key=key_act)
        y = torch.empty(M, dout, dtype=x.dtype, device=x.device)
        r2 = _flat2d(resid) if resid is not None else None
        K.gemm(h, w2, y, M, dout, F_, a_kmajor=1, b_kmajor=1, lda=F_, ldb=F_, ldc=dout, bias=b2, resid=r2, ld_resid=dout, split_k=1,
               drop_p=p_out, drop_key=key_out)
        ctx.save_for_backward(x2, w1, w2, z1, h)
        ctx.cfg = (act, b1 is not None, b2 is not None, resid is not None, x.shape)
        ctx.res_is_x = (resid is not None and resid.data_ptr() == x.data_ptr() and resid.shape == x.shape
                        and resid.stride() == x.stride() and dout == d)
        ctx.drop = (p_act, key_act, p_out, key_out)
        ctx.bias_objs = (b1, b2)
        return y.view(*x.shape[:-1], dout)

    @staticmethod
    def backward(ctx, dy):
        x2, w1, w2, z1, h = ctx.saved_tensors
        act, has_b1, has_b2, has_res, xshape = ctx.cfg
        M, d = x2.shape
        F_, dout = w1.shape[0], w2.shape[0]
        dy2 = _flat2d(dy)
        live = _tiles_of(dy, M)
        p_act, key_act, p_out, key_out = ctx.drop
        b1, b2 = ctx.bias_objs
        db2_fused = None
        gcs = not _os.environ.get("CST_NO_GEMM_COLSUM")
        db2_in_dw = gcs and has_b2 and ctx.needs_input_grad[4] and ctx.needs_input_grad[3] and dout % 8 == 0 and K.dw_colsum_is_fused(dout, F_, M, w2.dtype)
        db1_in_dw = gcs and has_b1 and ctx.needs_input_grad[2] and ctx.needs_input_grad[1] and F_ % 8 == 0 and K.dw_colsum_is_fused(F_, d, M, w1.dtype)
        if p_out > 0.0:
            dy2, db2_fused = _drop_grad(dy2, (p_out, key_out), w2.dtype, live, defer=_may_defer(w2, b2),
                                        with_colsum=not db2_in_dw and has_b2 and ctx.needs_input_grad[4] and dout % 8 == 0)
        use_wt = _want_wt(M, w2) and _want_wt(M, w1)
        dz1 = _dx_gemm(dy2, w2, M, use_wt=use_wt, like=dy2, dact=act, aux_in=z1, drop=(p_act, key_act), m_live=live)
        dx = dw1 = db1 = dw2 = db2 = None
        if ctx.needs_input_grad[3]:
            dw2, db2 = _dw_gemm(dy2, h, w2, b2, M, db_in_dw=db2_in_dw, live=live, dz_travels_on=dy2.data_ptr() == dy.data_ptr() and has_res)
        if has_b2 and ctx.needs_input_grad[4] and db2 is None:
            db2 = db2_fused if db2_fused is not None else K.colsum(dy2, w2.dtype, live, defer=_may_defer(w2, b2))
        if ctx.needs_input_grad[0]:
            dx = _dx_gemm(dz1, w1, M, use_wt=use_wt, like=x2, resid=_flat2d(dy) if ctx.res_is_x else None, m_live=live).view(xshape)
        if ctx.needs_input_grad[1]:
            dw1, db1 = _dw_gemm(dz1, x2, w1, b1, M, db_in_dw=db1_in_dw, live=live, dz_travels_on=False)
        if has_b1 and ctx.needs_input_grad[2] and db1 is None:
            db1 = K.colsum(dz1, w1.dtype, live, defer=_may_defer(w1, b1))
        dres = dy if has_res and ctx.needs_input_grad[5] and not (ctx.res_is_x and ctx.needs_input_grad[0]) else None
        return dx, dw1, db1, dw2, db2, dres, None, None, None, None, None


def ffn(x, w1, b1, w2, b2, act, resid=None, activation_dropout_p=0.0, dropout_p=0.0):
    assert _ACT[act] != L.ACT_NONE
    return _FFNFn.apply(x, w1.contiguous(), b1, w2.contiguous(), b2, resid, _ACT[act], *_drop_args(activation_dropout_p), *_drop_args(dropout_p))


class _LayerNormFn(torch.autograd.Function):
    @staticmethod
    def forward(ctx, x, res, gamma, beta, eps):
        x2 = _flat2d(x)
        r2 = _flat2d(res) if res is not None else None
        y, s, mean, rstd = K.layernorm_fwd(x2, r2, gamma, beta, eps, want_sum=True)
        src = s if res is not None else x2
        ctx.save_for_backward(src, gamma, mean, rstd)
        ctx.has_res = res is not None
        ctx.shape = x.shape
        ctx.set_materialize_grads(False)
        if res is not None:
            return y.view(x.shape), s.view(x.shape)
        return y.view(x.shape), None

    @staticmethod
    def backward(ctx, dy, ds):
        src, gamma, mean, rstd = ctx.saved_tensors
# ... 958 lines not shown
```

chimera-st_amd/kernels.py:

```python
import ctypes
import os

import torch

from . import lib as L

_ws = {}
STATS = {}


def workspace(nbytes: int, device) -> torch.Tensor:
    key = (device.index, L.stream_ptr().value)
    t = _ws.get(key)
    if t is None or t.numel() < nbytes:
        t = torch.empty(max(nbytes, 1 << 20), dtype=torch.uint8, device=device)
        _ws[key] = t
    return t


class _Deferred:

    MAX_BYTES = 32 << 20

    def __init__(self):
        self.on, self.items, self.keep, self.flushes = 0, [], [], 0
        self.main = None
        self.side = None
        self.side_used = False
        self.poison = False

    def push(self, src_ptr, dst, stride, Lr, P, keep, order=0):
        if self.poison:
            dst.fill_(float("nan"))
        if self.side_used and torch.is_tensor(keep) and torch.cuda.current_stream() != self.main:
            keep.record_stream(self.main)
        self.items.append((src_ptr, dst.data_ptr(), stride, Lr, P, L.dtype_code(dst.dtype), order))
        self.keep.append((keep, dst.detach()))

    def join(self):
        if self.side_used:
            torch.cuda.current_stream().wait_stream(self.side)
            self.side_used = False

    def flush(self):
        self.join()
        if self.items:
            reduce_multi(self.items)
            self.flushes += 1
            self.items, self.keep = [], []


DEFER = _Deferred()


def reduce_multi(items):
    lib = L.load()
    for at in range(0, len(items), 64):
        chunk = items[at:at + 64]
        arr = (L.ReduceItem * len(chunk))()
        for a, (src, dst, stride, Lr, P, dt, order) in zip(arr, chunk):
            a.src, a.dst, a.stride, a.L, a.P, a.dst_dtype, a.order = src, dst, stride, Lr, P, dt, order
        L.check(lib.cst_reduce_multi(arr, len(chunk), L.stream_ptr()), "cst_reduce_multi")


class deferred_reductions:

    def __init__(self, enabled=True):
        self.enabled = bool(enabled) and not os.environ.get("CST_NO_DEFER")

    def __enter__(self):
        if self.enabled:
            DEFER.on += 1
            DEFER.main = torch.cuda.current_stream()
            DEFER.poison = bool(os.environ.get("CST_DEFER_POISON"))
        return self

    def __exit__(self, *exc):
        if self.enabled:
            DEFER.on -= 1
            if DEFER.on == 0:
                DEFER.flush()
        return False


def side_gemm(big, reads, *args, **kw):
    if big or not DEFER.on or DEFER.main is None or not os.environ.get("CST_SIDE_STREAM") or torch.cuda.current_stream() != DEFER.main:
        return gemm(*args, **kw)
    if DEFER.side is None:
        DEFER.side = torch.cuda.Stream()
    side = DEFER.side
    side.wait_stream(DEFER.main)
    DEFER.side_used = True
    with torch.cuda.stream(side):
        out = gemm(*args, **kw)
    for t in reads:
        if t is not None:
            t.record_stream(side)
    STATS["side_gemm"] = STATS.get("side_gemm", 0) + 1
    return out


def _2d(t):
    assert t.dim() == 2 and t.stride(1) == 1, "expected a row-major 2-D tensor, got %s / %s" % (tuple(t.shape), t.stride())
    return t


def _stamps(live, extent, stat):
    if live is None:
        return None, 0
    assert live[0].numel() * 64 >= extent and live[0].dtype == torch.int32
    STATS[stat] = STATS.get(stat, 0) + 1
    return live[0].data_ptr(), live[1]


def _per_batch(v, batch0, stat):
    if v is None:
        return None
    assert v.dtype == torch.int32 and v.numel() == batch0 and v.is_contiguous()
    STATS[stat] = STATS.get(stat, 0) + 1
    return v.data_ptr()


def gemm(A, B, C, M, N, K, *, a_kmajor, b_kmajor, lda, ldb, ldc, bias=None, bias_mode=L.BIAS_COL, act=L.ACT_NONE,
         aux_out=None, ld_aux_out=0, dact=L.ACT_NONE, aux_in=None, ld_aux_in=0, resid=None, ld_resid=0, alpha=1.0,
         batch0=1, batch1=1, sa=(0, 0), sb=(0, 0), sc=(0, 0), sbias=(0, 0), a_seg=0, a_seg_stride=0, b_seg=0,
         b_seg_stride=0, split_k=-1, a_off=0, b_off=0, c_off=0, drop_p=0.0, drop_key=0, k_live=None, m_live=None, k_len=None, m_len=None,
         ws=None, colsum=None, defer=False, reduce_to=None):
    lib = L.load()
    d = L.GemmDesc()
    d.dtype = L.dtype_code(A.dtype)
    assert B.dtype == A.dtype, "A/B dtype mismatch"
    d.c_dtype = L.dtype_code(C.dtype)
    d.a_kmajor, d.b_kmajor = int(a_kmajor), int(b_kmajor)
    d.M, d.N, d.K = M, N, K
    es = A.element_size()
    d.A = A.data_ptr() + a_off * es
    d.lda, d.a_seg, d.a_seg_stride = lda, a_seg, a_seg_stride
    d.B = B.data_ptr() + b_off * es
    d.ldb, d.b_seg, d.b_seg_stride = ldb, b_seg, b_seg_stride
    d.C = C.data_ptr() + c_off * C.element_size()
    d.ldc = ldc
    if bias is not None:
        assert bias.dtype == A.dtype
        d.bias, d.bias_mode = bias.data_ptr(), bias_mode
    else:
        d.bias, d.bias_mode = None, L.BIAS_NONE
    d.sbias0, d.sbias1 = sbias
    d.act = act
    d.aux_out = None if aux_out is None else aux_out.data_ptr() + c_off * es
    d.ld_aux_out = ld_aux_out
    d.dact = dact
    d.aux_in = None if aux_in is None else aux_in.data_ptr() + c_off * es
    d.ld_aux_in = ld_aux_in
    d.resid = None if resid is None else resid.data_ptr() + c_off * es
    d.ld_resid = ld_resid
    d.alpha = alpha
    d.drop_p, d.drop_key = float(drop_p), int(drop_key) & 0xFFFFFFFF
    d.batch0, d.batch1 = batch0, batch1
    d.sa0, d.sa1 = sa
    d.sb0, d.sb1 = sb
    d.sc0, d.sc1 = sc
    d.split_k = split_k
    d.k_live, d.k_epoch = _stamps(k_live, K, "gemm_k_live")
    d.m_live, d.m_epoch = _stamps(m_live, M, "gemm_m_live")
    d.k_len = _per_batch(k_len, batch0, "gemm_k_len")
    d.m_len = _per_batch(m_len, batch0, "gemm_m_len")
    if colsum is not None:
        assert not a_kmajor and colsum.dtype == A.dtype and colsum.is_contiguous() and colsum.numel() == M * batch0 * batch1
        d.colsum = colsum.data_ptr()
    else:
        d.colsum = None
    d.defer_reduce = 0
    splits = 1
    need = lib.cst_gemm_workspace(ctypes.byref(d))
    nb = batch0 * batch1
    deferred = False
    if need > 0 and (reduce_to is not None or (defer and DEFER.on and nb == 1 and need <= DEFER.MAX_BYTES and ldc == N and N % 8 == 0)):
        splits = lib.cst_gemm_splits(ctypes.byref(d))
        if splits > 1:
            assert ws is None and bias is None and act == L.ACT_NONE and dact == L.ACT_NONE and resid is None and aux_out is None and alpha == 1.0
            ws = torch.empty(need, dtype=torch.uint8, device=A.device)
            d.defer_reduce = 1
            deferred = True
    if need > 0:
        if ws is None:
            ws = workspace(need, A.device)
        assert ws.dtype == torch.uint8 and ws.numel() >= need, "split-K scratch too small: %d < %d" % (ws.numel(), need)
        d.workspace, d.workspace_bytes = ws.data_ptr(), ws.numel()
    else:
        d.workspace, d.workspace_bytes = None, 0
    L.check(lib.cst_gemm(ctypes.byref(d), L.stream_ptr()), "cst_gemm")
    if reduce_to is not None:
        assert C.dtype == torch.float32 and sc == (M * N, 0) and ldc == N and reduce_to.numel() == M * N and reduce_to.is_contiguous() and colsum is None
        item = ((ws.data_ptr(), reduce_to, M * N, M * N, nb * splits, ws) if deferred else (C.data_ptr(), reduce_to, M * N, M * N, nb, C))
        if defer and DEFER.on:
            DEFER.push(*item)
        else:
            reduce_multi([(item[0], item[1].data_ptr(), item[2], item[3], item[4], L.dtype_code(reduce_to.dtype), 0)])
    elif deferred:
        DEFER.push(ws.data_ptr(), C, M * N, M * N, splits, ws)
        if colsum is not None:
            DEFER.push(ws.data_ptr() + 4 * splits * M * N, colsum, M, M, splits, ws)
    return C


_DW_FUSED = {}


def dw_colsum_is_fused(n_out, k_in, tokens, dtype):
    key = (n_out, k_in, tokens, dtype)
    r = _DW_FUSED.get(key)
    if r is None:
        d = L.GemmDesc()
        d.dtype = d.c_dtype = L.dtype_code(dtype)
        d.a_kmajor = d.b_kmajor = 0
        d.M, d.N, d.K = n_out, k_in, tokens
        d.batch0 = d.batch1 = 1
        d.split_k = -1
        d.colsum = 1
        r = _DW_FUSED[key] = bool(L.load().cst_gemm_colsum_is_fused(ctypes.byref(d)))
        if len(_DW_FUSED) > 4096:
            _DW_FUSED.clear()
    return r


def layernorm_fwd(x, res, gamma, beta, eps, want_sum=False):
    x = _2d(x)
    rows, cols = x.shape
    y = torch.empty_like(x)
    s = torch.empty_like(x) if (want_sum and res is not None) else None
    mean = torch.empty(rows, dtype=torch.float32, device=x.device)
    rstd = torch.empty(rows, dtype=torch.float32, device=x.device)
    L.check(L.load().cst_layernorm_fwd(L.ptr(x), L.ptr(res), L.ptr(gamma), L.ptr(beta), L.ptr(y), L.ptr(s), L.ptr(mean),
                                       L.ptr(rstd), rows, cols, eps, L.dtype_code(x.dtype), L.stream_ptr()), "cst_layernorm_fwd")
    return y, s, mean, rstd


_EPOCH = [0x3C6EF372]


def next_epoch():
    _EPOCH[0] = (_EPOCH[0] % 0xFFFFFFFE) + 1
    return _EPOCH[0]


def _two_stage(wbytes, outs, defer, launch):
    deferred = bool(defer) and DEFER.on > 0
    dev = outs[0].device
    ws = torch.empty(wbytes, dtype=torch.uint8, device=dev) if deferred else workspace(wbytes, dev)
    launch(ws, *[None if deferred else L.ptr(o) for o in outs])
    if deferred:
        n, cols = len(outs), outs[0].numel()
        for i, o in enumerate(outs):
            DEFER.push(ws.data_ptr() + 4 * cols * i, o, n * cols, cols, wbytes // (4 * n * cols), ws, order=1)


def layernorm_bwd(dy, s, gamma, mean, rstd, dres=None, grad_dtype=torch.float32, want_tiles=False, defer=False):
    dy, s = _2d(dy), _2d(s)
    rows, cols = s.shape
    lib = L.load()
    dx = torch.empty_like(s)
    dg = torch.empty(cols, dtype=grad_dtype, device=s.device)
    db = torch.empty(cols, dtype=grad_dtype, device=s.device)
    stamps, epoch = (torch.empty((rows + 63) // 64, dtype=torch.int32, device=s.device), next_epoch()) if want_tiles else (None, 0)

    def launch(ws, pg, pb):
        if want_tiles:
            L.check(lib.cst_layernorm_bwd_tiles(L.ptr(dy), L.ptr(s), L.ptr(gamma), L.ptr(mean), L.ptr(rstd), L.ptr(dres), L.ptr(dx), pg,
                                                pb, L.ptr(ws), rows, cols, L.dtype_code(s.dtype), L.dtype_code(grad_dtype),
                                                L.ptr(stamps), epoch, L.stream_ptr()), "cst_layernorm_bwd_tiles")
        else:
            L.check(lib.cst_layernorm_bwd(L.ptr(dy), L.ptr(s), L.ptr(gamma), L.ptr(mean), L.ptr(rstd), L.ptr(dres), L.ptr(dx), pg,
                                          pb, L.ptr(ws), rows, cols, L.dtype_code(s.dtype), L.dtype_code(grad_dtype), L.stream_ptr()),
                    "cst_layernorm_bwd")

    _two_stage(lib.cst_layernorm_bwd_workspace(rows, cols), (dg, db), defer, launch)
    return (dx, dg, db, (stamps, epoch)) if want_tiles else (dx, dg, db)


def _bhtd_strides(t, layout):
    assert t.stride(-1) == 1
    if layout == "bt":
        return t.stride(0), None, t.stride(1)
    return t.stride(1), None, t.stride(0)


def attn_desc(q, k, v, o, lse, H, D, kpm, causal, scale, layout_q="bt", layout_kv="bt", drop_p=0.0, drop_key=0, kv_len=None, seq=None):
    d = L.AttnDesc()
    d.dtype = L.dtype_code(q.dtype)
    if layout_q == "bt":
        B, Tq = q.shape[0], q.shape[1]
    else:
        Tq, B = q.shape[0], q.shape[1]
    Tk = k.shape[1] if layout_kv == "bt" else k.shape[0]
    if seq is not None:
        assert layout_q == "bt" and layout_kv == "bt" and B == 1 and kpm is None
        assert seq[0].dtype == torch.int32 and seq[0].is_contiguous()
        B, Tq, Tk = seq[0].numel() - 1, int(seq[1]), int(seq[1])
        d.seq_offsets = seq[0].data_ptr()
        STATS["attn_packed"] = STATS.get("attn_packed", 0) + 1
    else:
        d.seq_offsets = None
    d.B, d.H, d.Tq, d.Tk, d.D = B, H, Tq, Tk, D

    def st(t, lay):
        sb, _, stt = _bhtd_strides(t, lay)
        return sb, D, stt

    d.Q = q.data_ptr(); d.q_sb, d.q_sh, d.q_st = st(q, layout_q)
    d.K = k.data_ptr(); d.k_sb, d.k_sh, d.k_st = st(k, layout_kv)
    d.V = v.data_ptr(); d.v_sb, d.v_sh, d.v_st = st(v, layout_kv)
    d.O = o.data_ptr(); d.o_sb, d.o_sh, d.o_st = st(o, layout_q)
    d.lse = lse.data_ptr()
    if kpm is not None:
        assert kpm.dtype == torch.uint8 and kpm.stride(1) == 1 and kpm.shape == (B, Tk)
        d.key_padding_mask, d.kpm_stride = kpm.data_ptr(), kpm.stride(0)
        bits = kpm_bits(kpm)
        d.kpm_bits = bits.data_ptr()
        d._kpm_bits_owner = bits
    else:
        d.key_padding_mask, d.kpm_stride = None, 0
        d.kpm_bits = None
    d.bwd_ws = None
    d.causal, d.scale = int(causal), scale
    if q.dtype == torch.bfloat16 and D == 64 and not causal and not os.environ.get("CST_ATTN_GENERIC"):
        STATS["attn_fast"] = STATS.get("attn_fast", 0) + 1
    d.drop_p, d.drop_key = float(drop_p), int(drop_key) & 0xFFFFFFFF
    if kv_len is not None:
        assert (kpm is not None or seq is not None) and kv_len.dtype == torch.int32 and kv_len.numel() == B and kv_len.is_contiguous()
        d.kv_len = kv_len.data_ptr()
        STATS["attn_kv_len"] = STATS.get("attn_kv_len", 0) + 1
    else:
        d.kv_len = None
    return d


_KPM_BITS = []
_BIT_WEIGHTS = {}


def kpm_bits(kpm):
    key = (kpm.data_ptr(), tuple(kpm.shape), kpm._version)
    for ptr, shape, ver, _, bits in _KPM_BITS:
        if (ptr, shape, ver) == key:
            return bits
    B, Tk = kpm.shape
    nw = (Tk + 63) // 64
    m = kpm != 0
    if nw * 64 != Tk:
        m = torch.cat([m, torch.ones(B, nw * 64 - Tk, dtype=torch.bool, device=kpm.device)], 1)
    w = _BIT_WEIGHTS.get(kpm.device)
    if w is None:
        w = _BIT_WEIGHTS[kpm.device] = torch.ones(64, dtype=torch.int64, device=kpm.device) << torch.arange(64, dtype=torch.int64, device=kpm.device)
    bits = (m.view(B, nw, 64).to(torch.int64) * w).sum(-1).contiguous()
    _KPM_BITS.append(key + (kpm, bits))
    if len(_KPM_BITS) > 8:
        _KPM_BITS.pop(0)
    return bits
# ... 710 lines not shown
```

chimera-st_amd/lib.py:

```python
import ctypes
import os

import torch

_HERE = os.path.dirname(os.path.abspath(__file__))
LIB_PATH = os.path.join(_HERE, "libcst_hip.so")
ABI_VERSION = 13

F32, BF16 = 0, 1
ACT_NONE, ACT_RELU, ACT_GELU = 0, 1, 2
BIAS_NONE, BIAS_COL, BIAS_ROW = 0, 1, 2
K_GEMM, K_ATTN_FWD, K_ATTN_BWD, K_LAYERNORM, K_CONV0, K_ELEMENTWISE, K_LOSS, K_OPTIM = range(8)
KERNEL_CLASSES = ["gemm", "attn_fwd", "attn_bwd", "layernorm", "conv0", "elementwise", "loss", "optim"]

c_i64, c_int, c_f, c_p = ctypes.c_int64, ctypes.c_int, ctypes.c_float, ctypes.c_void_p


class GemmDesc(ctypes.Structure):
    _fields_ = [
        ("dtype", c_int), ("c_dtype", c_int), ("a_kmajor", c_int), ("b_kmajor", c_int),
        ("M", c_i64), ("N", c_i64), ("K", c_i64),
        ("A", c_p), ("lda", c_i64), ("a_seg", c_i64), ("a_seg_stride", c_i64),
        ("B", c_p), ("ldb", c_i64), ("b_seg", c_i64), ("b_seg_stride", c_i64),
        ("C", c_p), ("ldc", c_i64),
        ("bias", c_p), ("bias_mode", c_int), ("sbias0", c_i64), ("sbias1", c_i64),
        ("act", c_int),
        ("aux_out", c_p), ("ld_aux_out", c_i64),
        ("dact", c_int),
        ("aux_in", c_p), ("ld_aux_in", c_i64),
        ("resid", c_p), ("ld_resid", c_i64),
        ("alpha", c_f),
        ("drop_p", c_f), ("drop_key", ctypes.c_uint32),
        ("batch0", c_i64), ("batch1", c_i64),
        ("sa0", c_i64), ("sa1", c_i64), ("sb0", c_i64), ("sb1", c_i64), ("sc0", c_i64), ("sc1", c_i64),
        ("split_k", c_int),
        ("workspace", c_p), ("workspace_bytes", c_i64),
        ("k_live", c_p), ("k_epoch", ctypes.c_uint32),
        ("m_live", c_p), ("m_epoch", ctypes.c_uint32),
        ("k_len", c_p),
        ("m_len", c_p),
        ("colsum", c_p),
        ("defer_reduce", c_int),
    ]


class ReduceItem(ctypes.Structure):
    _fields_ = [("src", c_p), ("dst", c_p), ("stride", c_i64), ("L", c_i64), ("P", ctypes.c_int32), ("dst_dtype", ctypes.c_int32),
                ("block0", ctypes.c_int32), ("order", ctypes.c_int32)]


class AttnDesc(ctypes.Structure):
    _fields_ = [
        ("dtype", c_int),
        ("B", c_i64), ("H", c_i64), ("Tq", c_i64), ("Tk", c_i64), ("D", c_i64),
        ("Q", c_p), ("q_sb", c_i64), ("q_sh", c_i64), ("q_st", c_i64),
        ("K", c_p), ("k_sb", c_i64), ("k_sh", c_i64), ("k_st", c_i64),
        ("V", c_p), ("v_sb", c_i64), ("v_sh", c_i64), ("v_st", c_i64),
        ("O", c_p), ("o_sb", c_i64), ("o_sh", c_i64), ("o_st", c_i64),
        ("lse", c_p),
        ("key_padding_mask", c_p), ("kpm_stride", c_i64),
        ("causal", c_int), ("scale", c_f),
        ("drop_p", c_f), ("drop_key", ctypes.c_uint32),
        ("dO", c_p), ("do_sb", c_i64), ("do_sh", c_i64), ("do_st", c_i64),
        ("dQ", c_p), ("dq_sb", c_i64), ("dq_sh", c_i64), ("dq_st", c_i64),
        ("dK", c_p), ("dk_sb", c_i64), ("dk_sh", c_i64), ("dk_st", c_i64),
        ("dV", c_p), ("dv_sb", c_i64), ("dv_sh", c_i64), ("dv_st", c_i64),
        ("delta", c_p),
        ("kv_len", c_p),
        ("q_flags", c_p),
        ("seq_offsets", c_p),
        ("kpm_bits", c_p),
        ("bwd_ws", c_p),
    ]


class BeamDesc(ctypes.Structure):
    _fields_ = [
        ("dtype", c_int),
        ("bsz", c_i64), ("beam", c_i64), ("vocab", c_i64), ("max_len", c_i64),
        ("pad", c_i64), ("unk", c_i64), ("eos", c_i64), ("min_len", c_i64),
        ("unk_penalty", c_f), ("len_penalty", c_f), ("temperature", c_f),
        ("normalize_scores", c_int),
        ("logits", c_p), ("ld_logits", c_i64),
        ("step", c_p),
        ("tokens", c_p), ("scores", c_p), ("anc", c_p),
        ("cands_to_ignore", c_p), ("finished", c_p), ("nfinal", c_p), ("num_remaining", c_p),
        ("fin_tokens", c_p), ("fin_pos", c_p), ("fin_score", c_p), ("fin_len", c_p),
        ("workspace", c_p),
        ("members", c_i64), ("logits_n", c_p * 7), ("lprobs_out", c_p),
        ("no_repeat_ngram", c_i64), ("prefix_tokens", c_p), ("prefix_len", c_i64),
        ("sampling", c_i64), ("sample_topk", c_i64), ("sample_topp", c_f), ("sample_key", c_p),
        ("diverse_groups", c_i64), ("diverse_strength", c_f), ("diverse_siblings", c_i64), ("sibling_rate", c_f),
        ("fin_anc", c_p),
    ]


class LmFusionDesc(ctypes.Structure):
    _fields_ = [("lm_logits", c_p), ("lm_weight", c_f), ("lprobs_out", c_p)]


class LexDesc(ctypes.Structure):
    _fields_ = [("representation", c_i64), ("constraints", c_p), ("width", c_i64), ("workspace", c_p)]


LEX_TBL_W, LEX_SW, LEX_NEXT_MAX, LEX_WIDTH_MAX = 136, 44, 16, 65


def lex_states(workspace, bsz, beam):
    words = workspace.view(torch.int32)
    return words[bsz * LEX_TBL_W:bsz * LEX_TBL_W + 2 * bsz * beam * LEX_SW].view(2, bsz * beam, LEX_SW)


class FbankDesc(ctypes.Structure):
    _fields_ = [
        ("B", c_i64), ("S", c_i64), ("T", c_i64),
        ("wave", c_p), ("n_samples", c_p), ("out", c_p), ("n_frames", c_p),
        ("utterance_cmvn", c_int), ("norm_means", c_int), ("norm_vars", c_int),
        ("global_mean", c_p), ("global_std", c_p),
        ("global_first", c_int),
        ("specaugment", c_int),
        ("n_fmask", c_int), ("n_tmask", c_int),
        ("fmask", c_p), ("tmask", c_p),
        ("mask_mean", c_int), ("mask_value", c_f),
        ("workspace", c_p), ("workspace_bytes", c_i64),
    ]


SYMBOLS = [
    ("cst_last_error", ctypes.c_char_p, []),
    ("cst_version", c_int, []),
    ("cst_device_arch_ok", c_int, []),
    ("cst_prof_enable", None, [c_int]),
    ("cst_prof_query", c_i64, [c_int, ctypes.POINTER(ctypes.c_double), ctypes.POINTER(ctypes.c_double), ctypes.POINTER(ctypes.c_double)]),
    ("cst_layernorm_fwd", c_int, [c_p, c_p, c_p, c_p, c_p, c_p, c_p, c_p, c_i64, c_i64, c_f, c_int, c_p]),
    ("cst_layernorm_bwd_workspace", c_i64, [c_i64, c_i64]),
    ("cst_layernorm_bwd", c_int, [c_p, c_p, c_p, c_p, c_p, c_p, c_p, c_p, c_p, c_p, c_i64, c_i64, c_int, c_int, c_p]),
    ("cst_layernorm_bwd_tiles", c_int, [c_p, c_p, c_p, c_p, c_p, c_p, c_p, c_p, c_p, c_p, c_i64, c_i64, c_int, c_int, c_p, ctypes.c_uint32, c_p]),
    ("cst_gemm_workspace", c_i64, [ctypes.POINTER(GemmDesc)]),
    ("cst_gemm_colsum_is_fused", c_int, [ctypes.POINTER(GemmDesc)]),
    ("cst_gemm_splits", c_int, [ctypes.POINTER(GemmDesc)]),
    ("cst_gemm_route", c_int, [ctypes.POINTER(GemmDesc), ctypes.c_char_p, c_i64]),
    ("cst_reduce_multi", c_int, [ctypes.POINTER(ReduceItem), c_int, c_p]),
    ("cst_gemm", c_int, [ctypes.POINTER(GemmDesc), c_p]),
    ("cst_posconv_fwd", c_int, [c_p, c_p, c_p, c_p, c_p, c_p, c_i64, c_i64, c_i64, c_i64, c_i64, c_p]),
    ("cst_posconv_dx", c_int, [c_p, c_p, c_p, c_p, c_p, c_i64, c_i64, c_i64, c_i64, c_i64, c_p]),
    ("cst_posconv_dw", c_int, [c_p, c_p, c_p, c_p, c_p, ctypes.c_uint32, c_i64, c_i64, c_i64, c_i64, c_i64, c_p]),
    ("cst_prof_dump", c_i64, [c_int, ctypes.c_char_p, c_i64]),
    ("cst_gemm_reserve_cus", c_int, [c_int]),
    ("cst_transpose2d", c_int, [c_p, c_p, c_i64, c_i64, c_int, c_p]),
    ("cst_transpose2d_multi", c_int, [c_p, c_int, c_i64, c_int, c_p]),
    ("cst_weight_norm_workspace", c_i64, [c_i64, c_i64]),
    ("cst_weight_norm_fwd", c_int, [c_p, c_p, c_p, c_p, c_p, c_i64, c_i64, c_int, c_p]),
    ("cst_weight_norm_bwd", c_int, [c_p, c_p, c_p, c_p, c_p, c_p, c_p, c_i64, c_i64, c_int, c_p]),
    ("cst_attn_bwd_workspace", c_i64, [ctypes.POINTER(AttnDesc)]),
    ("cst_attn_fwd", c_int, [ctypes.POINTER(AttnDesc), c_p]),
    ("cst_attn_bwd", c_int, [ctypes.POINTER(AttnDesc), c_p]),
    ("cst_conv0_fwd_workspace", c_i64, [c_i64, c_i64, c_int, c_int]),
    ("cst_conv0_gn_gelu_fwd", c_int, [c_p, c_p, c_p, c_p, c_p, c_p, c_p, c_p, c_p, c_p, c_i64, c_i64, c_i64, c_int, c_int, c_f, c_int, c_p]),
    ("cst_conv0_bwd_workspace", c_i64, [c_i64, c_i64, c_i64, c_int, c_int]),
    ("cst_conv0_gn_gelu_bwd", c_int, [c_p, c_p, c_p, c_p, c_p, c_p, c_p, c_p, c_p, c_p, c_p, c_p, c_p, c_i64, c_i64, c_i64, c_int, c_int, c_int, c_p]),
    ("cst_conv0_ln_gelu_fwd", c_int, [c_p, c_p, c_p, c_p, c_p, c_p, c_p, c_p, c_p, c_i64, c_i64, c_i64, c_int, c_int, c_f, c_int, c_p]),
    ("cst_conv0_ln_bwd_workspace", c_i64, [c_i64, c_i64, c_i64, c_int, c_int]),
    ("cst_conv0_ln_gelu_bwd", c_int, [c_p, c_p, c_p, c_p, c_p, c_p, c_p, c_p, c_p, c_p, c_p, c_p, c_p, c_p, c_i64, c_i64, c_i64, c_int, c_int, c_int, c_p]),
    ("cst_ln_gelu_fwd", c_int, [c_p, c_p, c_p, c_p, c_p, c_p, c_p, c_i64, c_i64, c_i64, c_f, c_int, c_p]),
    ("cst_ln_gelu_bwd_workspace", c_i64, [c_i64, c_i64]),
    ("cst_ln_gelu_bwd", c_int, [c_p, c_p, c_p, c_p, c_p, c_p, c_p, c_i64, c_p, c_p, c_p, c_p, c_p, c_i64, c_i64, c_i64, c_int, c_p]),
    ("cst_glu_fwd", c_int, [c_p, c_p, c_i64, c_i64, c_int, c_p]),
    ("cst_glu_bwd", c_int, [c_p, c_p, c_p, c_i64, c_i64, c_int, c_p]),
    ("cst_act_bwd", c_int, [c_p, c_p, c_p, c_i64, c_int, c_int, c_p]),
    ("cst_act_fwd", c_int, [c_p, c_p, c_i64, c_int, c_int, c_p]),
    ("cst_colsum", c_int, [c_p, c_i64, c_p, c_i64, c_i64, c_int, c_p]),
    ("cst_colsum_workspace", c_i64, [c_i64, c_i64]),
    ("cst_colsum_typed", c_int, [c_p, c_i64, c_p, c_p, c_i64, c_i64, c_int, c_int, c_p]),
    ("cst_colsum_typed_live", c_int, [c_p, c_i64, c_p, c_p, c_i64, c_i64, c_int, c_int, c_p, ctypes.c_uint32, c_p]),
    ("cst_col2im1d", c_int, [c_p, c_p, c_p, c_i64, c_i64, c_i64, c_i64, c_int, c_int, c_int, c_int, c_int, c_p]),
    ("cst_mask_rows", c_int, [c_p, c_p, c_p, c_i64, c_i64, c_int, c_p]),
    ("cst_dropout", c_int, [c_p, c_p, c_i64, c_f, ctypes.c_uint32, c_int, c_p]),
    ("cst_rows_pack", c_int, [c_p, c_p, c_p, c_i64, c_i64, c_i64, c_int, c_int, c_p]),
    ("cst_rows_unpack", c_int, [c_p, c_p, c_p, c_i64, c_i64, c_i64, c_int, c_int, c_p]),
    ("cst_dec_linear", c_int, [c_p, c_p, c_p, c_p, c_p, c_i64, c_i64, c_i64, c_i64, c_i64, c_i64, c_int, c_p, c_i64, c_int, c_p]),
    ("cst_dec_ln_linear", c_int, [c_p, c_p, c_p, c_p, c_f, c_p, c_p, c_i64, c_i64, c_i64, c_i64, c_i64, c_i64, c_int, c_p, c_i64, c_int, c_p]),
    ("cst_dropout_colsum", c_int, [c_p, c_p, c_p, c_p, c_i64, c_i64, c_int, c_int, c_f, ctypes.c_uint32, c_p, ctypes.c_uint32, c_p]),
    ("cst_conv_row_limits", c_int, [c_p, c_p, c_p, c_int, c_i64, c_p, c_i64, c_int, c_p]),
    ("cst_dropout_scale", c_int, [c_p, c_p, c_i64, c_f, c_f, ctypes.c_uint32, c_int, c_p]),
    ("cst_embed_pos_fwd", c_int, [c_p, c_p, c_p, c_p, c_p, c_f, c_i64, c_p, c_i64, c_i64, c_i64, c_i64, c_i64, c_f, ctypes.c_uint32, c_int, c_p]),
    ("cst_embed_bwd", c_int, [c_p, c_p, c_p, c_f, c_i64, c_i64, c_i64, c_i64, c_f, ctypes.c_uint32, c_int, c_int, c_p]),
    ("cst_ls_ce_fwd", c_int, [c_p, c_p, c_p, c_p, c_p, c_i64, c_i64, c_f, c_i64, c_int, c_p]),
    ("cst_ls_ce_bwd", c_int, [c_p, c_p, c_p, c_p, c_p, c_i64, c_i64, c_f, c_i64, c_int, c_p]),
    ("cst_score_tokens", c_int, [c_p, ctypes.POINTER(c_p), c_i64, c_i64, c_p, c_i64, c_p, c_p, c_p, c_i64, c_i64, c_i64, c_int, c_p]),
    ("cst_ctc_fwd", c_int, [c_p, c_i64, c_i64, c_p, c_i64, c_p, c_p, c_i64, c_int, c_p, c_p, c_p, c_p, c_p, c_p, c_i64, c_i64, c_i64, c_int, c_p]),
    ("cst_ctc_bwd", c_int, [c_p, c_i64, c_i64, c_p, c_i64, c_p, c_p, c_i64, c_int, c_p, c_p, c_p, c_p, c_p, c_p, c_i64, c_i64, c_i64, c_i64, c_i64,
                            c_int, c_p]),
    ("cst_ctc_greedy", c_int, [c_p, c_i64, c_i64, c_p, c_i64, c_p, c_p, c_p, c_i64, c_i64, c_i64, c_int, c_p]),
    ("cst_w2v_negatives", c_int, [ctypes.c_uint32, c_i64, c_i64, c_i64, c_i64, c_p, c_p]),
    ("cst_infonce_fwd", c_int, [c_p, c_p, c_p, c_f, c_p, c_p, c_p, c_p, c_p, c_p, c_p, c_p, c_i64, c_i64, c_i64, c_int, c_p]),
    ("cst_infonce_bwd_x", c_int, [c_p, c_p, c_p, c_f, c_p, c_p, c_p, c_p, c_p, c_p, c_i64, c_i64, c_i64, c_int, c_p]),
    ("cst_infonce_bwd_y", c_int, [c_p, c_p, c_p, c_p, c_p, c_p, c_p, c_p, c_i64, c_i64, c_i64, c_int, c_p]),
    ("cst_gumbel_vq_workspace", c_i64, [c_i64, c_i64, c_i64]),
    ("cst_gumbel_vq_fwd", c_int, [c_p, c_p, c_p, ctypes.c_uint32, c_int, c_p, c_p, c_p, c_p, c_p, c_p, c_p, c_i64, c_i64, c_i64, c_i64, c_int, c_p]),
    ("cst_gumbel_vq_bwd", c_int, [c_p, c_p, ctypes.c_uint32, c_f, c_p, c_p, c_p, c_p, c_p, c_i64, c_i64, c_i64, c_int, c_p]),
    ("cst_contrastive_fwd", c_int, [c_p, c_p, c_p, c_p, c_p, c_p, c_p, c_i64, c_i64, c_i64, c_f, c_int, c_p]),
    ("cst_contrastive_bwd", c_int, [c_p, c_p, c_p, c_p, c_p, c_p, c_p, c_p, c_i64, c_i64, c_i64, c_f, c_int, c_p]),
    ("cst_sumsq_workspace", c_i64, []),
    ("cst_sumsq", c_int, [c_p, c_i64, c_p, c_p, c_int, c_p]),
    ("cst_adam_step", c_int, [c_p, c_p, c_p, c_p, c_p, c_i64, c_f, c_f, c_f, c_f, c_f, c_i64, c_p, c_int, c_int, c_p]),
    ("cst_beam_workspace", c_i64, [c_i64, c_i64]),
    ("cst_beam_init", c_int, [ctypes.POINTER(BeamDesc), c_p]),
    ("cst_beam_step", c_int, [ctypes.POINTER(BeamDesc), c_p]),
    ("cst_beam_step_lm", c_int, [ctypes.POINTER(BeamDesc), ctypes.POINTER(LmFusionDesc), c_p]),
    ("cst_lex_workspace", c_i64, [c_i64, c_i64, c_i64]),
    ("cst_lex_init", c_int, [ctypes.POINTER(BeamDesc), ctypes.POINTER(LexDesc), c_p]),
    ("cst_beam_step_lex", c_int, [ctypes.POINTER(BeamDesc), ctypes.POINTER(LmFusionDesc), ctypes.POINTER(LexDesc), c_p]),
    ("cst_dec_embed", c_int, [c_p, c_p, c_p, c_p, c_f, c_i64, c_p, c_i64, c_i64, c_i64, c_i64, c_int, c_p]),
    ("cst_dec_self_attn", c_int, [c_p, c_p, c_p, c_p, c_p, c_p, c_i64, c_i64, c_i64, c_i64, c_f, c_int, c_p]),
    ("cst_batch_by_size", c_i64, [c_p, c_i64, c_i64, c_i64, ctypes.c_int32, c_p]),
    ("cst_wav_info", c_int, [ctypes.c_char_p, c_p, c_p, c_p, c_p]),
    ("cst_wav_read_f32", c_i64, [ctypes.c_char_p, c_i64, c_i64, c_p, c_i64]),
    ("cst_edit_distance", c_i64, [c_p, c_i64, c_p, c_i64]),
    ("cst_dec_cross_attn", c_int, [c_p, c_p, c_p, c_p, c_p, c_p, c_i64, c_i64, c_i64, c_i64, c_i64, c_i64, c_f, c_int, c_p]),
    ("cst_fbank_workspace_bytes", c_i64, [c_i64, c_i64]),
    ("cst_fbank", c_int, [ctypes.POINTER(FbankDesc), c_p]),
    ("cst_dec_ln_q_cross_attn", c_int, [c_p, c_i64, c_p, c_p, c_p, c_f, c_p, c_p, c_p, c_p, c_p, c_i64, c_i64, c_i64, c_i64, c_i64, c_i64, c_f, c_int, c_p]),
    ("cst_attn_avg_probs", c_int, [c_p, c_i64, c_p, c_i64, c_i64, c_i64, c_p, c_p, c_i64, c_p, c_i64, c_i64, c_i64, c_i64, c_i64, c_i64, c_f, c_f,
                                   c_int, c_int, c_p]),
    ("cst_collate_pairs", c_int, [c_p, c_p, c_int, c_p, c_p, c_i64, c_p, c_i64, c_i64, c_i64, c_i64, c_i64, c_int, c_int, c_p, c_p]),
    ("cst_token_block_slices", c_i64, [c_p, c_i64, c_int, c_i64, c_i64, c_p, c_i64]),
    ("cst_token_block_index", c_int, [c_p, c_i64, c_p, c_i64, c_p]),
    ("cst_collate_blocks", c_int, [c_p, c_int, c_p, c_i64, c_p, c_i64, c_i64, c_i64, c_i64, c_p, c_p]),
]

_lib = None


def load():
    global _lib
    if _lib is not None:
        return _lib
    if not os.path.exists(LIB_PATH):
        raise RuntimeError(
            "chimera-st_amd: %s is missing — the HIP extension is the product path and there is no fallback. "
            "Build it with `python -c 'import __graft_entry__ as g; g.build()'` or `make -C chimera-st_amd/csrc`." % LIB_PATH)
    lib = ctypes.CDLL(LIB_PATH)
    for name, res, args in SYMBOLS:
        fn = getattr(lib, name)
        fn.restype = res
        fn.argtypes = args
    built = lib.cst_version()
    if built != ABI_VERSION:
        raise RuntimeError("chimera-st_amd: %s was built for ABI version %d, this package binds version %d (include/cst.h "
                           "CST_ABI_VERSION) — rebuild it with `make -C chimera-st_amd/csrc`." % (LIB_PATH, built, ABI_VERSION))
    _lib = lib
    return lib


def check(rc, what=""):
    if rc != 0:
        msg = load().cst_last_error()
        raise RuntimeError("libcst_hip %s failed (%d): %s" % (what, rc, msg.decode() if msg else "?"))


def dtype_code(t: torch.dtype) -> int:
    if t == torch.float32:
        return F32
    if t == torch.bfloat16:
        return BF16
    raise TypeError("chimera-st_amd kernels compute in float32 or bfloat16 storage, got %s" % t)


_DEV_INDEX = None


def stream_ptr():
    global _DEV_INDEX
    if _DEV_INDEX is None:
        _DEV_INDEX = torch.cuda.current_device()
    return ctypes.c_void_p(torch._C._cuda_getCurrentRawStream(_DEV_INDEX))


def ptr(t):
    if t is None:
        return None
    if not t.is_cuda:
        raise RuntimeError("chimera-st_amd: tensor is not on the GPU — the HIP path has no CPU fallback")
    return ctypes.c_void_p(t.data_ptr())


def prof_enable(on: bool):
    load().cst_prof_enable(1 if on else 0)


def prof_query():
    lib = load()
    out = {}
    for i, name in enumerate(KERNEL_CLASSES):
        ms, fl, by = ctypes.c_double(), ctypes.c_double(), ctypes.c_double()
        n = lib.cst_prof_query(i, ctypes.byref(ms), ctypes.byref(fl), ctypes.byref(by))
# ... 15 lines not shown
```

include/cst.h:

```cpp
#ifndef CST_H
#define CST_H

#include <stdint.h>

#ifdef __cplusplus
extern "C" {
#endif

#define CST_ABI_VERSION 13

typedef enum { CST_F32 = 0, CST_BF16 = 1 } cst_dtype;

typedef enum {
  CST_OK = 0,
  CST_ERR_BAD_ARG = -1,
  CST_ERR_LAUNCH = -2,
  CST_ERR_WORKSPACE = -3,
  CST_ERR_UNSUPPORTED = -4
} cst_status;

typedef void* cst_stream;

const char* cst_last_error(void);
int cst_version(void);
int cst_device_arch_ok(void);

typedef enum {
  CST_K_GEMM = 0, CST_K_ATTN_FWD, CST_K_ATTN_BWD, CST_K_LAYERNORM, CST_K_CONV0, CST_K_ELEMENTWISE,
  CST_K_LOSS, CST_K_OPTIM, CST_K_NUM
} cst_kernel_class;
void cst_prof_enable(int on);
int64_t cst_prof_query(int kernel_class, double* total_ms, double* flops, double* bytes);
int64_t cst_prof_dump(int kernel_class, char* buf, int64_t cap);

int cst_layernorm_fwd(const void* x, const void* res, const void* gamma, const void* beta,
                      void* y, void* sum_out, float* mean, float* rstd,
                      int64_t rows, int64_t cols, float eps, int dtype, cst_stream stream);
int64_t cst_layernorm_bwd_workspace(int64_t rows, int64_t cols);
int cst_layernorm_bwd(const void* dy, const void* s, const void* gamma, const float* mean,
                      const float* rstd, const void* dres, void* dx, void* dgamma, void* dbeta,
                      void* workspace, int64_t rows, int64_t cols, int dtype, int grad_dtype, cst_stream stream);
int cst_layernorm_bwd_tiles(const void* dy, const void* s, const void* gamma, const float* mean,
                            const float* rstd, const void* dres, void* dx, void* dgamma, void* dbeta,
                            void* workspace, int64_t rows, int64_t cols, int dtype, int grad_dtype,
                            uint32_t* tile_live, uint32_t epoch, cst_stream stream);

typedef enum { CST_ACT_NONE = 0, CST_ACT_RELU = 1, CST_ACT_GELU = 2 } cst_act;
typedef enum { CST_BIAS_NONE = 0, CST_BIAS_COL = 1, CST_BIAS_ROW = 2 } cst_bias_mode;

typedef struct {
  int dtype;
  int c_dtype;
  int a_kmajor, b_kmajor;
  int64_t M, N, K;
  const void* A; int64_t lda, a_seg, a_seg_stride;
  const void* B; int64_t ldb, b_seg, b_seg_stride;
  void* C; int64_t ldc;
  const void* bias; int bias_mode;
  int64_t sbias0, sbias1;
  int act;
  void* aux_out; int64_t ld_aux_out;
  int dact;
  const void* aux_in; int64_t ld_aux_in;
  const void* resid; int64_t ld_resid;
  float alpha;
  float drop_p; uint32_t drop_key;
  int64_t batch0, batch1;
  int64_t sa0, sa1, sb0, sb1, sc0, sc1;
  int split_k;
  void* workspace; int64_t workspace_bytes;
  const uint32_t* k_live; uint32_t k_epoch;
  const uint32_t* m_live; uint32_t m_epoch;
  const int32_t* k_len;
  const int32_t* m_len;
  void* colsum;
  int defer_reduce;
} cst_gemm_desc;

int64_t cst_gemm_workspace(const cst_gemm_desc* d);
int cst_gemm_colsum_is_fused(const cst_gemm_desc* d);
int cst_gemm_splits(const cst_gemm_desc* d);
int cst_gemm_route(const cst_gemm_desc* d, char* out, int64_t out_bytes);
int cst_gemm_reserve_cus(int n);
int cst_gemm(const cst_gemm_desc* d, cst_stream stream);

int cst_posconv_fwd(const void* x, const void* w, const void* bias, void* y, void* z, const int32_t* m_len, int64_t B, int64_t T,
                    int64_t C, int64_t groups, int64_t k, cst_stream stream);
int cst_posconv_dx(const void* dz, const void* wflip, const void* dy, void* dx, const int32_t* m_len, int64_t B, int64_t T,
                   int64_t C, int64_t groups, int64_t k, cst_stream stream);
int cst_posconv_dw(const void* dz, const void* x, void* dw, void* db, const uint32_t* k_live, uint32_t k_epoch, int64_t B,
                   int64_t T, int64_t C, int64_t groups, int64_t k, cst_stream stream);

typedef struct {
  int dtype;
  int64_t B, H, Tq, Tk, D;
  const void* Q; int64_t q_sb, q_sh, q_st;
  const void* K; int64_t k_sb, k_sh, k_st;
  const void* V; int64_t v_sb, v_sh, v_st;
  void* O; int64_t o_sb, o_sh, o_st;
  float* lse;
  const uint8_t* key_padding_mask; int64_t kpm_stride;
  int causal;
  float scale;
  float drop_p; uint32_t drop_key;
  const void* dO; int64_t do_sb, do_sh, do_st;
  void* dQ; int64_t dq_sb, dq_sh, dq_st;
  void* dK; int64_t dk_sb, dk_sh, dk_st;
  void* dV; int64_t dv_sb, dv_sh, dv_st;
  float* delta;
  const int32_t* kv_len;
  uint8_t* q_flags;
  const int32_t* seq_offsets;
  const uint64_t* kpm_bits;
  void* bwd_ws;
} cst_attn_desc;

int64_t cst_attn_bwd_workspace(const cst_attn_desc* d);
int cst_attn_fwd(const cst_attn_desc* d, cst_stream stream);
int cst_attn_bwd(const cst_attn_desc* d, cst_stream stream);

int cst_conv_row_limits(const int32_t* nz_last, const int32_t* k, const int32_t* stride, int L, int64_t S, int32_t* out, int64_t B,
                        int smax, cst_stream stream);
int64_t cst_conv0_fwd_workspace(int64_t B, int64_t S, int k, int stride);
int cst_conv0_gn_gelu_fwd(const float* wav, const void* w, const void* gamma, const void* beta,
                          void* y, float* mean, float* rstd, float* gram, float* workspace, const int32_t* frame_limit, int64_t B,
                          int64_t S, int64_t C, int k, int stride, float eps, int dtype, cst_stream stream);
int64_t cst_conv0_bwd_workspace(int64_t B, int64_t S, int64_t C, int k, int stride);
int cst_conv0_gn_gelu_bwd(const void* dy, const float* wav, const void* w, const void* gamma,
                          const void* beta, const float* mean, const float* rstd, const float* gram,
                          float* dw, float* dgamma, float* dbeta, float* workspace, const int32_t* frame_limit,
                          int64_t B, int64_t S, int64_t C, int k, int stride, int dtype,
                          cst_stream stream);

int cst_conv0_ln_gelu_fwd(const float* wav, const void* w, const void* bias, const void* gamma, const void* beta, void* y,
                          float* mean, float* rstd, const int32_t* frame_limit, int64_t B, int64_t S, int64_t C, int k,
                          int stride, float eps, int dtype, cst_stream stream);
int64_t cst_conv0_ln_bwd_workspace(int64_t B, int64_t S, int64_t C, int k, int stride);
int cst_conv0_ln_gelu_bwd(const void* dy, const float* wav, const void* w, const void* bias, const void* gamma, const void* beta,
                          const float* mean, const float* rstd, float* dw, float* dbias, float* dgamma, float* dbeta,
                          float* workspace, const int32_t* frame_limit, int64_t B, int64_t S, int64_t C, int k, int stride,
                          int dtype, cst_stream stream);
int cst_ln_gelu_fwd(const void* u, const void* gamma, const void* beta, void* y, float* mean, float* rstd,
                    const int32_t* row_limit, int64_t B, int64_t L, int64_t C, float eps, int dtype, cst_stream stream);
int64_t cst_ln_gelu_bwd_workspace(int64_t rows, int64_t C);
int cst_ln_gelu_bwd(const void* dy, const void* u, const void* gamma, const void* beta, const float* mean, const float* rstd,
                    void* du, int64_t du_batch_stride, float* dgamma, float* dbeta, float* dcolsum, float* workspace,
                    const int32_t* row_limit, int64_t B, int64_t L, int64_t C, int dtype, cst_stream stream);

int cst_glu_fwd(const void* z, void* y, int64_t rows, int64_t C, int dtype, cst_stream stream);
int cst_glu_bwd(const void* dy, const void* z, void* dz, int64_t rows, int64_t C, int dtype, cst_stream stream);
int cst_act_bwd(const void* dy, const void* z, void* dx, int64_t n, int act, int dtype, cst_stream stream);
int cst_act_fwd(const void* x, void* y, int64_t n, int act, int dtype, cst_stream stream);
int cst_colsum(const void* x, int64_t ldx, float* out, int64_t rows, int64_t cols, int dtype, cst_stream stream);
int cst_dropout_colsum(const void* x, void* xd, void* out, void* workspace, int64_t rows, int64_t cols, int dtype, int out_dtype,
                       float p, uint32_t key, const uint32_t* row_live, uint32_t epoch, cst_stream stream);
int64_t cst_colsum_workspace(int64_t rows, int64_t cols);
int cst_colsum_typed(const void* x, int64_t ldx, void* out, void* workspace, int64_t rows, int64_t cols, int dtype, int out_dtype,
                     cst_stream stream);
int cst_colsum_typed_live(const void* x, int64_t ldx, void* out, void* workspace, int64_t rows, int64_t cols, int dtype,
                          int out_dtype, const uint32_t* row_live, uint32_t epoch, cst_stream stream);
int cst_col2im1d(const void* dcol, const void* z, void* dx, int64_t B, int64_t Lin, int64_t Lout,
                 int64_t C, int k, int stride, int pad, int dact, int dtype, cst_stream stream);
int64_t cst_weight_norm_workspace(int64_t R, int64_t C);
int cst_weight_norm_fwd(const void* v, const void* g, void* w, float* norm, void* workspace, int64_t R, int64_t C, int dtype, cst_stream stream);
int cst_weight_norm_bwd(const void* v, const void* g, const void* dw, const float* norm, void* dv, void* dg, void* workspace, int64_t R,
                        int64_t C, int dtype, cst_stream stream);
int cst_transpose2d(const void* src, void* dst, int64_t R, int64_t C, int dtype, cst_stream stream);
typedef struct cst_transpose_item {
  const void* src; void* dst;
  int64_t R, C;
  int64_t tile0;
} cst_transpose_item;
int cst_transpose2d_multi(const cst_transpose_item* items_dev, int n, int64_t total_tiles, int dtype, cst_stream stream);
#define CST_REDUCE_MAX_ITEMS 64
typedef struct cst_reduce_item {
  const float* src; void* dst;
  int64_t stride, L;
  int32_t P, dst_dtype, block0, order;
} cst_reduce_item;
int cst_reduce_multi(const cst_reduce_item* items, int n, cst_stream stream);
int cst_mask_rows(const void* x, const uint8_t* mask, void* y, int64_t rows, int64_t cols, int dtype, cst_stream stream);

int cst_rows_pack(const void* src, const int32_t* seq_off, void* dst, int64_t B, int64_t T, int64_t C, int tail_sum, int dtype,
                  cst_stream stream);
int cst_rows_unpack(const void* src, const int32_t* seq_off, void* dst, int64_t B, int64_t T, int64_t C, int tail_broadcast, int dtype,
                    cst_stream stream);

int cst_dropout(const void* x, void* y, int64_t n, float p, uint32_t key, int dtype, cst_stream stream);
int cst_dropout_scale(const void* x, void* y, int64_t n, float alpha, float p, uint32_t key, int dtype, cst_stream stream);

int cst_embed_pos_fwd(const int64_t* tokens, const uint8_t* pad_mask, const void* embed, const void* x, const float* pos_table,
                      float scale, int64_t pad_idx, void* out, int64_t B, int64_t T, int64_t C, int64_t V, int64_t pos_rows,
                      float drop_p, uint32_t drop_key, int dtype, cst_stream stream);
int cst_embed_bwd(const void* dy, const int64_t* tokens, void* dE, float scale, int64_t pad_idx, int64_t n, int64_t C, int64_t V,
                  float drop_p, uint32_t drop_key, int dtype, int grad_dtype, cst_stream stream);

int cst_ls_ce_fwd(const void* logits, const int64_t* target, float* out2, float* lse, float* row_ws,
                  int64_t rows, int64_t V, float eps, int64_t pad_idx, int dtype, cst_stream stream);
int cst_ls_ce_bwd(const void* logits, const int64_t* target, const float* lse, const float* gscale,
                  void* dlogits, int64_t rows, int64_t V, float eps, int64_t pad_idx, int dtype,
                  cst_stream stream);

int cst_score_tokens(const void* logits, const void* const* logits_n, int64_t members, int64_t ld, const int64_t* target, int64_t pad,
                     float* pos, float* score, int32_t* len, int64_t B, int64_t T, int64_t V, int dtype, cst_stream stream);

int cst_ctc_fwd(const void* logits, int64_t stride_t, int64_t stride_b, const int64_t* targets, int64_t Lmax, const int64_t* target_len,
                const int64_t* input_len, int64_t blank, int zero_infinity, float* nll, float* loss, float* lse, float* emit, float* alpha,
                float* beta, int64_t T, int64_t B, int64_t V, int dtype, cst_stream stream);
int cst_ctc_bwd(const void* logits, int64_t stride_t, int64_t stride_b, const int64_t* targets, int64_t Lmax, const int64_t* target_len,
                const int64_t* input_len, int64_t blank, int zero_infinity, const float* nll, const float* lse, const float* alpha,
                const float* beta, const float* gscale, void* dlogits, int64_t dstride_t, int64_t dstride_b, int64_t T, int64_t B,
                int64_t V, int dtype, cst_stream stream);
int cst_ctc_greedy(const void* logits, int64_t stride_t, int64_t stride_b, const int64_t* input_len, int64_t blank, int32_t* argmax_ws,
                   int32_t* ids, int32_t* counts, int64_t T, int64_t B, int64_t V, int dtype, cst_stream stream);

int cst_w2v_negatives(uint32_t key, int64_t B, int64_t M, int64_t K, int64_t Kx, int32_t* out, cst_stream stream);
int cst_infonce_fwd(const void* x, const void* y, const int32_t* idx, float inv_temp, float* nll, float* loss, int32_t* counters,
                    float* lse, float* nx, float* ny, int32_t* flags, float* logits_dbg, int64_t N, int64_t KP, int64_t D, int dtype,
                    cst_stream stream);
int cst_infonce_bwd_x(const void* x, const void* y, const int32_t* idx, float inv_temp, const float* lse, const float* nx,
                      const float* ny, const float* gscale, void* dx, float* pairs, int64_t N, int64_t KP, int64_t D, int dtype,
                      cst_stream stream);
int cst_infonce_bwd_y(const void* x, const void* y, const int64_t* perm, const int32_t* offs, const float* pairs, const float* nx,
                      const float* ny, void* dy, int64_t N, int64_t KP, int64_t D, int dtype, cst_stream stream);

int64_t cst_gumbel_vq_workspace(int64_t N, int64_t G, int64_t V);
int cst_gumbel_vq_fwd(const void* logits, const void* vars, const float* noise, uint32_t key, int training, void* q, int32_t* idx,
                      void* onehot, float* avg_probs, float* stats, float* exph, void* workspace, int64_t N, int64_t G, int64_t V, int64_t d,
                      int dtype, cst_stream stream);
int cst_gumbel_vq_bwd(const void* logits, const float* noise, uint32_t key, float inv_tau, const void* gy, const float* avg_probs,
                      const float* exph, const float* dppl, void* dl, int64_t N, int64_t G, int64_t V, int dtype, cst_stream stream);

int cst_contrastive_fwd(const void* a, const void* t, float* loss, float* loss_rows, float* sim, float* na, float* nt,
                        int64_t B, int64_t M, int64_t C, float temp, int dtype, cst_stream stream);
int cst_contrastive_bwd(const void* a, const void* t, const float* sim, const float* na, const float* nt,
                        const float* gscale, void* da, void* dt, int64_t B, int64_t M, int64_t C, float temp,
                        int dtype, cst_stream stream);
// ... 117 lines not shown
```

Measured before the change: 505.5.

## Batch same-shape deferred weight-gradient GEMMs into one grouped list launch

Small weight-gradient GEMMs that previously launched one by one are now deferred and grouped by shape. Each group runs as a single pointer-list GEMM kernel whose blockIdx.z selects the problem, and a list variant of split-K reduce handles the outputs. The goal is to fill the GPU's compute units when each dW GEMM alone has too few tiles, and to cut launch overhead. In exchange it keeps the dz/x tensors alive longer (up to a 4 GB cap), adds a kernel body shared through an include file, and defers the writes of dW and db until the flush.

```diff
diff --git a/chimera-st_amd/csrc/gemm.hip b/chimera-st_amd/csrc/gemm.hip
--- a/chimera-st_amd/csrc/gemm.hip
+++ b/chimera-st_amd/csrc/gemm.hip
@@ -21,339 +21,31 @@
 
 template <typename T, bool A_KMAJOR, bool B_KMAJOR, bool SEG, typename C, bool CS = false>
 __global__ __launch_bounds__(C::NT) void gemm_kernel(GemmParams p) {
-  constexpr int BM = C::BM, BN = C::BN, NTHREADS = C::NT, TM = C::TM, TN = C::TN;
-  constexpr int VEC = DT<T>::VEC;
-  constexpr int KV = C::KV, BK = KV * VEC;
-  constexpr int LDK = BK + VEC;
-  constexpr int LDMA = sizeof(T) == 2 ? BM + 32 : BM + VEC;
-  constexpr int LDMB = sizeof(T) == 2 ? BN + 32 : BN + VEC;
-  constexpr int A_ELEMS = A_KMAJOR ? BM * LDK : BK * LDMA;
-  constexpr int B_ELEMS = B_KMAJOR ? BN * LDK : BK * LDMB;
-  constexpr int MVA = BM / VEC, MVB = BN / VEC;
-  constexpr int NVA = BM * KV / NTHREADS, NVB = BN * KV / NTHREADS;
-  extern __shared__ __attribute__((aligned(16))) char smem_raw[];
-  T* smem = reinterpret_cast<T*>(smem_raw);
-  constexpr int STAGE = A_ELEMS + B_ELEMS;
-
-  const int tid = threadIdx.x, lane = tid & 63, wave = tid >> 6;
-  const int wm = wave / C::WN, wn = wave % C::WN;
-
-  const int ntiles = p.tiles_m * p.tiles_n;
-  int tm, tn, z;
-  if (p.split_order) {
-    const int total = ntiles * p.splits, L = (int)blockIdx.x + (int)gridDim.x * (int)blockIdx.z;
-    const int q = total / 8, r = total % 8, xcd = L % 8, loc = L / 8;
-    const int item = (xcd < r ? xcd * (q + 1) : r * (q + 1) + (xcd - r) * q) + loc;
-    z = item / ntiles;
-    const int t = item % ntiles;
-    tm = t / p.tiles_n;
-    tn = t % p.tiles_n;
-  } else {
-    int id = blockIdx.x;
-    {
-      const int q = ntiles / 8, r = ntiles % 8, xcd = id % 8, loc = id / 8;
-      id = (xcd < r ? xcd * (q + 1) : r * (q + 1) + (xcd - r) * q) + loc;
-    }
-    constexpr int GROUP_M = 8;
-    const int per_group = GROUP_M * p.tiles_n;
-    const int grp = id / per_group, rem = id % per_group;
-    const int gm0 = grp * GROUP_M;
-    const int gsz = (p.tiles_m - gm0 < GROUP_M) ? (p.tiles_m - gm0) : GROUP_M;
-    tm = gm0 + rem % gsz;
-    tn = rem / gsz;
-    z = blockIdx.z;
-  }
-  const int64_t m0 = (int64_t)tm * BM, n0 = (int64_t)tn * BN;
-
-  const int split = z % p.splits;
-  const int64_t bidx = z / p.splits;
-  const int64_t b0 = bidx / p.batch1, b1 = bidx % p.batch1;
-  const T* A = (const T*)p.A + b0 * p.sa0 + b1 * p.sa1;
-  const T* B = (const T*)p.B + b0 * p.sb0 + b1 * p.sb1;
-  const int64_t cofs = b0 * p.sc0 + b1 * p.sc1;
-  const int64_t bofs = b0 * p.sbias0 + b1 * p.sbias1;
-
-  int ktiles = (int)((p.K + BK - 1) / BK);
-  const int kfull = (int)(p.K / BK);
-  if (p.k_len) {
-    typedef const __attribute__((address_space(4))) int32_t* cptr_t;
-    const int kl = ((cptr_t)p.k_len)[b0];
-    const int live = kl <= 0 ? 0 : (kl + BK - 1) / BK;
-    ktiles = live < ktiles ? live : ktiles;
-  }
-  const int per = (ktiles + p.splits - 1) / p.splits;
-  const int kt0 = split * per;
-  const int kt1 = (kt0 + per < ktiles) ? kt0 + per : ktiles;
-
-  u32x4 ra[NVA], rb[NVB];
-  const T* pa[NVA];
-  const T* pb[NVB];
-  int ka[NVA], kb[NVB];
-  int aq[NVA], ar[NVA], bq[NVB], br[NVB];
-#pragma unroll
-  for (int i = 0; i < NVA; ++i) {
-    const int v = tid + NTHREADS * i;
-    if (A_KMAJOR) {
-      int64_t row = m0 + v / KV;
-      row = row < p.M ? row : p.M - 1;
-      ka[i] = kt0 * BK + (v % KV) * VEC;
-      if (SEG && p.a_seg) { aq[i] = ka[i] / (int)p.a_seg; ar[i] = ka[i] % (int)p.a_seg; pa[i] = A + row * p.lda; }
-      else { aq[i] = 0; ar[i] = 0; pa[i] = A + row * p.lda + ka[i]; }
-    } else {
-      int64_t m = m0 + (int64_t)(v % MVA) * VEC;
-      m = m < p.M ? m : p.M - VEC;
-      ka[i] = kt0 * BK + v / MVA;
-      aq[i] = 0; ar[i] = 0;
-      pa[i] = A + (int64_t)ka[i] * p.lda + segaddr(m, p.a_seg, p.a_seg_stride);
-    }
-  }
-#pragma unroll
-  for (int i = 0; i < NVB; ++i) {
-    const int v = tid + NTHREADS * i;
-    if (B_KMAJOR) {
-      int64_t row = n0 + v / KV;
-      row = row < p.N ? row : p.N - 1;
-      kb[i] = kt0 * BK + (v % KV) * VEC;
-      if (SEG && p.b_seg) { bq[i] = kb[i] / (int)p.b_seg; br[i] = kb[i] % (int)p.b_seg; pb[i] = B + row * p.ldb; }
-      else { bq[i] = 0; br[i] = 0; pb[i] = B + row * p.ldb + kb[i]; }
-    } else {
-      int64_t n = n0 + (int64_t)(v % MVB) * VEC;
-      n = n < p.N ? n : p.N - VEC;
-      kb[i] = kt0 * BK + v / MVB;
-      bq[i] = 0; br[i] = 0;
-      pb[i] = B + (int64_t)kb[i] * p.ldb + segaddr(n, p.b_seg, p.b_seg_stride);
-    }
-  }
-  const int64_t step_a = A_KMAJOR ? (int64_t)BK : (int64_t)BK * p.lda;
-  const int64_t step_b = B_KMAJOR ? (int64_t)BK : (int64_t)BK * p.ldb;
-
-  auto load_tile = [&](auto tail_tag) {
-    constexpr bool TAIL = decltype(tail_tag)::value;
-    const u32x4 zero = {0, 0, 0, 0};
-#pragma unroll
-    for (int i = 0; i < NVA; ++i) {
-      const T* qa = pa[i];
-      if (SEG && A_KMAJOR && p.a_seg) qa = pa[i] + (int64_t)aq[i] * p.a_seg_stride + ar[i];
-      if (TAIL) {
-        const bool oka = ka[i] < p.K;
-        const u32x4 va = *reinterpret_cast<const u32x4*>(oka ? qa : A);
-        ra[i] = oka ? va : zero;
-      } else {
-        ra[i] = *reinterpret_cast<const u32x4*>(qa);
-      }
-      ka[i] += BK;
-      if (SEG && A_KMAJOR && p.a_seg) { ar[i] += BK; while (ar[i] >= (int)p.a_seg) { ar[i] -= (int)p.a_seg; ++aq[i]; } }
-      else pa[i] += step_a;
-    }
-#pragma unroll
-    for (int i = 0; i < NVB; ++i) {
-      const T* qb = pb[i];
-      if (SEG && B_KMAJOR && p.b_seg) qb = pb[i] + (int64_t)bq[i] * p.b_seg_stride + br[i];
-      if (TAIL) {
-        const bool okb = kb[i] < p.K;
-        const u32x4 vb = *reinterpret_cast<const u32x4*>(okb ? qb : B);
-        rb[i] = okb ? vb : zero;
-      } else {
-        rb[i] = *reinterpret_cast<const u32x4*>(qb);
-      }
-      kb[i] += BK;
-      if (SEG && B_KMAJOR && p.b_seg) { br[i] += BK; while (br[i] >= (int)p.b_seg) { br[i] -= (int)p.b_seg; ++bq[i]; } }
-      else pb[i] += step_b;
-    }
-  };
-  auto load_any = [&](int kt) {
-    if (kt < kfull) load_tile(std::false_type{});
-    else load_tile(std::true_type{});
-  };
-  static_assert(!CS || (!A_KMAJOR && NTHREADS % MVA == 0), "a thread must stage the same columns of an mn-major A in every vector");
-  const bool do_cs = CS && tn == 0;
-  float cs[VEC];
-#pragma unroll
-  for (int e = 0; e < VEC; ++e) cs[e] = 0.0f;
-  auto store_tile = [&](int buf) {
-#pragma unroll
-    for (int i = 0; i < NVA; ++i) {
-      const int v = tid + NTHREADS * i;
-      T* da = smem + buf * STAGE + (A_KMAJOR ? (v / KV) * LDK + (v % KV) * VEC : (v / MVA) * LDMA + (v % MVA) * VEC);
-      *reinterpret_cast<u32x4*>(da) = ra[i];
-      if (CS && do_cs) {
-        if (sizeof(T) == 2) {
-#pragma unroll
-          for (int e = 0; e < 4; ++e) {
-            cs[2 * e] += __uint_as_float(ra[i][e] << 16);
-            cs[2 * e + 1] += __uint_as_float(ra[i][e] & 0xffff0000u);
-          }
-        } else {
-#pragma unroll
-          for (int e = 0; e < 4; ++e) cs[e] += __uint_as_float(ra[i][e]);
-        }
-      }
-    }
-#pragma unroll
-    for (int i = 0; i < NVB; ++i) {
-      const int v = tid + NTHREADS * i;
-      T* db = smem + buf * STAGE + A_ELEMS + (B_KMAJOR ? (v / KV) * LDK + (v % KV) * VEC : (v / MVB) * LDMB + (v % MVB) * VEC);
-      *reinterpret_cast<u32x4*>(db) = rb[i];
-    }
-  };
-
-  f32x16 acc[TM][TN];
-#pragma unroll
-  for (int i = 0; i < TM; ++i)
-#pragma unroll
-    for (int j = 0; j < TN; ++j)
-#pragma unroll
-      for (int r = 0; r < 16; ++r) acc[i][j][r] = 0.0f;
-
-  constexpr int KLIST_MAX = 1000;
-  __shared__ int klist[KLIST_MAX];
-  __shared__ int klist_n;
-  const bool kskip = !SEG && BK == 64 && p.k_live != nullptr && per <= KLIST_MAX;
-  int nk = kt1 > kt0 ? kt1 - kt0 : 0;
-  if (kskip) {
-    if (wave == 0) {
-      int total = 0;
-      for (int base = 0; base < ktiles; base += 64) {
-        const int kt = base + lane;
-        total += __builtin_popcountll(__builtin_amdgcn_ballot_w64(kt < ktiles && p.k_live[kt] == p.k_epoch));
-      }
-      const int lo = (int)(((int64_t)total * split) / p.splits), hi = (int)(((int64_t)total * (split + 1)) / p.splits);
-      int seen = 0, n = 0;
-      for (int base = 0; base < ktiles && seen < hi; base += 64) {
-        const int kt = base + lane;
-        const bool live = kt < ktiles && p.k_live[kt] == p.k_epoch;
-        const uint64_t m = __builtin_amdgcn_ballot_w64(live);
-        const int idx = seen + __builtin_popcountll(m & ((1ull << lane) - 1ull));
-        if (live && idx >= lo && idx < hi) klist[idx - lo] = kt;
-        seen += __builtin_popcountll(m);
-      }
-      n = hi - lo;
-      if (lane == 0) klist_n = n;
-    }
-    __syncthreads();
-    nk = klist_n;
-  }
-  if (p.m_live) {
-    typedef const __attribute__((address_space(4))) uint32_t* cptr_t;
-    cptr_t ml = (cptr_t)p.m_live;
-    const int t0 = (int)(m0 >> 6), t1 = (int)((((m0 + BM < p.M) ? m0 + BM : p.M) + 63) >> 6);
-    bool live = false;
-    for (int t = t0; t < t1; ++t) live |= ml[t] == p.m_epoch;
-    if (!live) nk = 0;
-  }
-  if (p.m_len) {
-    typedef const __attribute__((address_space(4))) int32_t* cptr_t;
-    if (m0 >= (int64_t)((cptr_t)p.m_len)[b0]) nk = 0;
-  }
-  int pos = kt0;
-  auto fetch = [&](int kt) {
-    const int d = kt - pos;
-    if (d) {
-#pragma unroll
-      for (int i = 0; i < NVA; ++i) { pa[i] += (int64_t)d * step_a; ka[i] += d * BK; }
-#pragma unroll
-      for (int i = 0; i < NVB; ++i) { pb[i] += (int64_t)d * step_b; kb[i] += d * BK; }
-    }
-    load_any(kt);
-    pos = kt + 1;
-  };
-  auto tile_at = [&](int it) { return kskip ? klist[it] : kt0 + it; };
-
-  if (nk > 0) {
-    fetch(tile_at(0));
-    store_tile(0);
-  }
-  __syncthreads();
-  int cur = 0;
-  const int lrow = lane & 31, lk = 8 * (lane >> 5);
-  constexpr int WROWS = TM * 32, WCOLS = TN * 32;
-  for (int it = 0; it < nk; ++it) {
-    const bool more = it + 1 < nk;
-    if (more) fetch(tile_at(it + 1));
-    const T* sa = smem + cur * STAGE;
-    const T* sb = sa + A_ELEMS;
-#pragma unroll
-    for (int kk = 0; kk < BK; kk += 16) {
-      Frag<T> fa[TM], fb[TN];
-#pragma unroll
-      for (int i = 0; i < TM; ++i) {
-        if (A_KMAJOR) frag_load_contig(fa[i], sa + (wm * WROWS + i * 32 + lrow) * LDK + kk + lk);
-        else frag_load_tr(fa[i], sa, LDMA, wm * WROWS + i * 32, kk + lk, kk + lk + 4, lane);
-      }
-#pragma unroll
-      for (int j = 0; j < TN; ++j) {
-        if (B_KMAJOR) frag_load_contig(fb[j], sb + (wn * WCOLS + j * 32 + lrow) * LDK + kk + lk);
-        else frag_load_tr(fb[j], sb, LDMB, wn * WCOLS + j * 32, kk + lk, kk + lk + 4, lane);
-      }
-#pragma unroll
-      for (int i = 0; i < TM; ++i)
-#pragma unroll
-        for (int j = 0; j < TN; ++j) mma16(acc[i][j], fa[i], fb[j]);
-    }
-    if (more) store_tile(cur ^ 1);
-    __syncthreads();
-    cur ^= 1;
-  }
-
-  if (CS && do_cs) {
-    float* red = reinterpret_cast<float*>(smem_raw);
-#pragma unroll
-    for (int e = 0; e < VEC; ++e) red[(tid / MVA) * BM + (tid % MVA) * VEC + e] = cs[e];
-    __syncthreads();
-    if (tid < BM && m0 + tid < p.M) {
-      float tot = 0.0f;
-      for (int r = 0; r < NTHREADS / MVA; ++r) tot += red[r * BM + tid];
-      if (p.splits > 1) p.colsum_ws[((int64_t)bidx * p.splits + split) * p.M + m0 + tid] = tot;
-      else DT<T>::st((T*)p.colsum + bidx * p.M + m0 + tid, tot);
-    }
-  }
-
-  constexpr int LDC = BN + 4;
-  constexpr int VPR = BN / 8;
-  constexpr int NPASS = BM / 64;
-  constexpr int ITERS = 64 * VPR / NTHREADS;
-  float* stage = reinterpret_cast<float*>(smem_raw);
-  float* wsp = p.splits > 1 ? p.ws + ((int64_t)z) * p.M * p.N : nullptr;
-  const bool ws_vec = (p.N % 4) == 0;
-#pragma unroll
-  for (int ps = 0; ps < NPASS; ++ps) {
-    __syncthreads();
-#pragma unroll
-    for (int i = 0; i < TM; ++i) {
-      const int trow = wm * WROWS + i * 32;
-      if (trow / 64 == ps) {
-#pragma unroll
-        for (int j = 0; j < TN; ++j)
-#pragma unroll
-          for (int r = 0; r < 16; ++r)
-            stage[(trow - 64 * ps + acc_row(r, lane)) * LDC + wn * WCOLS + j * 32 + lrow] = acc[i][j][r];
-      }
-    }
-    __syncthreads();
-#pragma unroll 2
-    for (int it = 0; it < ITERS; ++it) {
-      const int v = tid + NTHREADS * it;
-      const int rl = v / VPR, cl = (v % VPR) * 8;
-      const int64_t row = m0 + 64 * ps + rl, col = n0 + cl;
-      if (row >= p.M || col >= p.N) continue;
-      float x[8];
-      {
-        const f32x4 a = *reinterpret_cast<const f32x4*>(stage + rl * LDC + cl);
-        const f32x4 b = *reinterpret_cast<const f32x4*>(stage + rl * LDC + cl + 4);
-        x[0] = a[0]; x[1] = a[1]; x[2] = a[2]; x[3] = a[3]; x[4] = b[0]; x[5] = b[1]; x[6] = b[2]; x[7] = b[3];
-      }
-      const bool full = col + 8 <= p.N;
-      if (wsp) {
-        if (full && ws_vec) store8(wsp + row * p.N + col, x);
-        else
-          for (int e = 0; e < 8 && col + e < p.N; ++e) wsp[row * p.N + col + e] = x[e];
-      } else if (full && p.vec_epi) {
-        epilogue_store8<T>(p, cofs, bofs, row, col, x);
-      } else {
-        for (int e = 0; e < 8 && col + e < p.N; ++e) epilogue_store<T>(p, cofs, bofs, row, col + e, x[e]);
-      }
-    }
-  }
+  constexpr bool LIST = false;
+  constexpr int serial = 0;
+#include "gemm_body.inc"
+}
+
+struct GemmList {
+  const void* A[CST_GEMM_LIST_MAX];
+  const void* B[CST_GEMM_LIST_MAX];
+  void* C[CST_GEMM_LIST_MAX];
+  void* colsum[CST_GEMM_LIST_MAX];
+  int serial;
+};
+
+template <typename T, typename C, bool CS>
+__global__ __launch_bounds__(C::NT) void gemm_kernel_list(GemmParams p, GemmList l) {
+  constexpr bool A_KMAJOR = false, B_KMAJOR = false, SEG = false, LIST = true;
+  const int serial = l.serial;
+  {
+    const int b = p.split_order ? 0 : (int)blockIdx.z / p.splits;
+    p.A = l.A[b];
+    p.B = l.B[b];
+    p.C = l.C[b];
+    if (CS) p.colsum = l.colsum[b];
+  }
+#include "gemm_body.inc"
 }
 
 template <int N>
@@ -688,8 +380,8 @@
   }
 }
 
-template <typename T>
-__global__ void splitk_reduce_kernel(GemmParams p) {
+template <typename T, bool LIST>
+__device__ __forceinline__ void splitk_reduce_body(const GemmParams& p) {
   const int64_t total = p.M * p.N;
   const int64_t bidx = blockIdx.y;
   const int64_t b0 = bidx / p.batch1, b1 = bidx % p.batch1;
@@ -700,7 +392,7 @@
     for (int64_t m = (int64_t)blockIdx.x * blockDim.x + threadIdx.x; m < p.M; m += (int64_t)gridDim.x * blockDim.x) {
       float v = 0.0f;
       for (int s = 0; s < p.splits; ++s) v += p.colsum_ws[(bidx * p.splits + s) * p.M + m];
-      DT<T>::st((T*)p.colsum + bidx * p.M + m, v);
+      DT<T>::st((T*)p.colsum + (LIST ? 0 : bidx) * p.M + m, v);
     }
   }
   if (p.vec_epi && (p.N % 8) == 0) {
@@ -738,8 +430,29 @@
   }
 }
 
+template <typename T>
+__global__ void splitk_reduce_kernel(GemmParams p) { splitk_reduce_body<T, false>(p); }
+
+template <typename T>
+__global__ void splitk_reduce_kernel_list(GemmParams p, GemmList l) {
+  p.C = l.C[blockIdx.y];
+  if (p.colsum) p.colsum = l.colsum[blockIdx.y];
+  splitk_reduce_body<T, true>(p);
+}
+
+template <typename T, typename C, bool CS>
+int launch_list(const GemmParams& p, const GemmList& l, dim3 grid, size_t lds, hipStream_t s) {
+  static bool attr_set = false;
+  if (!attr_set) {
+    (void)hipFuncSetAttribute(reinterpret_cast<const void*>(&gemm_kernel_list<T, C, CS>), hipFuncAttributeMaxDynamicSharedMemorySize, 160 * 1024 - 16384);
+    attr_set = true;
+  }
+  hipLaunchKernelGGL((gemm_kernel_list<T, C, CS>), grid, dim3(C::NT), lds, s, p, l);
+  return cst_check_launch("cst_gemm");
+}
+
 template <typename T, bool AK, bool BK_, bool SEG, typename C>
-int launch(GemmParams p, int64_t M, int64_t N, int64_t nbatch, hipStream_t s) {
+int launch(GemmParams p, int64_t M, int64_t N, int64_t nbatch, hipStream_t s, const GemmList* list = nullptr) {
   constexpr int VEC = DT<T>::VEC;
   constexpr int BKc = C::KV * VEC, LDK = BKc + VEC;
   constexpr int LDMA = sizeof(T) == 2 ? C::BM + 32 : C::BM + VEC, LDMB = sizeof(T) == 2 ? C::BN + 32 : C::BN + VEC;
@@ -757,6 +470,17 @@
   p.tiles_n = (int)cst_ceil_div(N, C::BN);
   p.split_order = (p.splits > 1 && nbatch == 1) ? 1 : 0;
   dim3 grid(p.tiles_m * p.tiles_n, 1, (unsigned)(nbatch * p.splits));
+  if (list) {
+    constexpr bool LISTABLE = !AK && !BK_ && !SEG && (std::is_same<C, CfgSmall>::value || std::is_same<C, CfgNarrowM>::value || std::is_same<C, CfgLarge>::value);
+    if constexpr (LISTABLE) {
+      if constexpr (C::NT <= 256) {
+        if (p.colsum) return launch_list<T, C, true>(p, *list, grid, lds, s);
+      }
+      if (!p.colsum) return launch_list<T, C, false>(p, *list, grid, lds, s);
+    }
+    cst_set_error("cst_gemm: internal: a listed batch on a configuration that does not take one");
+    return CST_ERR_UNSUPPORTED;
+  }
   if constexpr (!AK && !BK_ && !SEG && C::NT <= 256) {
     if (p.colsum) {
       static bool attr_cs = false;
@@ -955,6 +679,30 @@
                                      const uint32_t* row_live, uint32_t epoch, cst_stream stream);
 
 namespace {
+
+int list_view(const cst_gemm_desc* d, const cst_gemm_problem* l, cst_gemm_desc& e) {
+  CST_REQUIRE(d, "cst_gemm: null operand");
+  e = *d;
+  if (!l) return CST_OK;
+  CST_REQUIRE(d->batch0 >= 1 && d->batch1 == 1, "cst_gemm: a list gives batch0 >= 1 problems with batch1 = 1");
+  CST_REQUIRE(!d->a_kmajor && !d->b_kmajor, "cst_gemm: a list needs both operands mn-major (k-major operands are not listed)");
+  CST_REQUIRE(!d->a_seg && !d->b_seg, "cst_gemm: a list takes no segmented operands");
+  CST_REQUIRE(!d->k_live && !d->m_live && !d->k_len && !d->m_len, "cst_gemm: a list takes no live-tile stamps or row limits (k_live / m_live / k_len / m_len)");
+  CST_REQUIRE(!d->bias && !d->act && !d->aux_out && !d->dact && !d->aux_in && !d->resid && d->alpha == 1.0f, "cst_gemm: a list takes no epilogue operands (bias, act, aux_out, dact, resid, alpha)");
+  CST_REQUIRE(d->drop_p == 0.0f, "cst_gemm: a list takes no dropout");
+  CST_REQUIRE(!d->defer_reduce, "cst_gemm: a list finishes its own split-K slabs (no defer_reduce)");
+  for (int64_t z = 0; z < d->batch0; ++z) {
+    CST_REQUIRE(l[z].A && l[z].B && l[z].C, "cst_gemm: list entry %lld: null operand", (long long)z);
+    CST_REQUIRE(((uintptr_t)l[z].A % 16 == 0) && ((uintptr_t)l[z].B % 16 == 0), "cst_gemm: list entry %lld: A/B must be 16-byte aligned", (long long)z);
+    CST_REQUIRE(((uintptr_t)l[z].C % 16 == 0) == ((uintptr_t)l[0].C % 16 == 0) && (uintptr_t)l[z].C % 4 == 0 && (uintptr_t)l[z].colsum % 4 == 0,
+                "cst_gemm: list entry %lld: C / colsum aligned unlike entry 0", (long long)z);
+    CST_REQUIRE((l[z].colsum != nullptr) == (l[0].colsum != nullptr), "cst_gemm: list entry %lld: colsum in every entry or in none", (long long)z);
+  }
+  e.A = l[0].A; e.B = l[0].B; e.C = l[0].C; e.colsum = l[0].colsum;
+  e.sa0 = e.sa1 = e.sb0 = e.sb1 = e.sc0 = e.sc1 = e.sbias0 = e.sbias1 = 0;
+  e.batch0 = 1;
+  return CST_OK;
+}
 
 int validate(const cst_gemm_desc* d) {
   CST_REQUIRE(d && d->A && d->B && d->C, "cst_gemm: null operand");
@@ -1035,18 +783,21 @@
   return bytes;
 }
 
-int take_route(const cst_gemm_desc* d, const GemmSwitches& sw, GemmParams& p, GemmRoute& r) {
+int take_route(const cst_gemm_desc* d, const GemmSwitches& sw, GemmParams& p, GemmRoute& r, int64_t nlist = 0) {
   r = gemm_route(d, p, sw);
-  const int64_t nbatch = d->batch0 * d->batch1;
+  const bool listed = nlist > 0;
+  const int64_t nbatch = listed ? nlist : d->batch0 * d->batch1;
   CST_REQUIRE(r.colsum != Colsum::Separate || (nbatch == 1 && d->M % 8 == 0 && d->lda % 8 == 0),
               "cst_gemm: colsum of this configuration runs as a separate column sum: unbatched, M and lda multiples of 8");
+  CST_REQUIRE(!listed || (r.family == Family::Reg && r.colsum != Colsum::Separate),
+              "cst_gemm: a list needs the register-staged kernel and, with colsum, a configuration that builds the column sums itself");
   CST_REQUIRE(cst_ceil_div(d->M, 128) * cst_ceil_div(d->N, 128) < (1ll << 31) && nbatch * r.splits < 65536, "cst_gemm: grid too large");
   p.splits = r.splits;
   p.colsum = r.colsum == Colsum::Fused ? d->colsum : nullptr;
 #ifdef CST_TRACE
   if (p.splits == 1 && d->workspace) p.ws = (float*)d->workspace;
 #endif
-  const int64_t need = route_workspace(d, r);
+  const int64_t need = route_workspace(d, r) * (listed ? nlist : 1);
   if (need > 0 && (!d->workspace || d->workspace_bytes < need)) {
     if (r.splits > 1) cst_set_error("cst_gemm: split_k=%d needs %lld workspace bytes, got %lld", r.splits, (long long)need, (long long)d->workspace_bytes);
     else cst_set_error("cst_gemm: colsum needs %lld workspace bytes, got %lld", (long long)need, (long long)d->workspace_bytes);
@@ -1119,23 +870,23 @@
 }
 
 template <typename T, bool SEG, typename C>
-int launch_reg(const GemmRoute& r, const GemmParams& p, int64_t nbatch, hipStream_t s) {
+int launch_reg(const GemmRoute& r, const GemmParams& p, int64_t nbatch, hipStream_t s, const GemmList* list = nullptr) {
   return r.ak ? (r.bk ? launch<T, true, true, SEG, C>(p, p.M, p.N, nbatch, s) : launch<T, true, false, SEG, C>(p, p.M, p.N, nbatch, s))
-              : (r.bk ? launch<T, false, true, SEG, C>(p, p.M, p.N, nbatch, s) : launch<T, false, false, SEG, C>(p, p.M, p.N, nbatch, s));
+              : (r.bk ? launch<T, false, true, SEG, C>(p, p.M, p.N, nbatch, s) : launch<T, false, false, SEG, C>(p, p.M, p.N, nbatch, s, list));
 }
 
 constexpr int arm(Family f, Tile t, int stages = 0) { return ((int)f << 8) | ((int)t << 4) | stages; }
 
 template <typename T>
-int launch_route(const GemmRoute& r, const GemmParams& p, int64_t nbatch, hipStream_t s, const GemmSwitches& sw) {
+int launch_route(const GemmRoute& r, const GemmParams& p, int64_t nbatch, hipStream_t s, const GemmSwitches& sw, const GemmList* list = nullptr) {
   constexpr bool HOOK = std::is_same<T, bf16_t>::value;
   const int64_t M = p.M, N = p.N;
   switch (arm(r.family, r.tile, r.family == Family::Dma ? r.stages : 0)) {
     case arm(Family::Persistent8, Tile::Large): return cst_gemm8p_launch(p, r.ak, r.bk, nbatch, s);
     case arm(Family::FourWave, Tile::Big4N): return cst_gemm4w_launch(p, s);
-    case arm(Family::Reg, Tile::Small): return r.seg ? launch_reg<T, true, CfgSmall>(r, p, nbatch, s) : launch_reg<T, false, CfgSmall>(r, p, nbatch, s);
-    case arm(Family::Reg, Tile::Large): return launch_reg<T, false, CfgLarge>(r, p, nbatch, s);
-    case arm(Family::Reg, Tile::NarrowM): return launch<T, false, false, false, CfgNarrowM>(p, M, N, nbatch, s);
+    case arm(Family::Reg, Tile::Small): return r.seg ? launch_reg<T, true, CfgSmall>(r, p, nbatch, s) : launch_reg<T, false, CfgSmall>(r, p, nbatch, s, list);
+    case arm(Family::Reg, Tile::Large): return launch_reg<T, false, CfgLarge>(r, p, nbatch, s, list);
+    case arm(Family::Reg, Tile::NarrowM): return launch<T, false, false, false, CfgNarrowM>(p, M, N, nbatch, s, list);
     case arm(Family::Dma, Tile::Small, 2): return launch_glds<T, true, true, CfgSmall, 2>(p, M, N, nbatch, s);
     case arm(Family::Dma, Tile::Large, 2): return launch_glds<T, true, true, CfgLarge, 2>(p, M, N, nbatch, s);
     case arm(Family::Dma, Tile::NarrowN, 2): return launch_glds<T, true, true, CfgNarrowN, 2>(p, M, N, nbatch, s);
@@ -1156,8 +907,8 @@
   return rc == CST_OK ? CST_ERR_UNSUPPORTED : rc;
 }
 
-int finish(const cst_gemm_desc* d, const GemmRoute& r, const GemmParams& p, cst_stream stream) {
-  const int64_t nbatch = d->batch0 * d->batch1;
+int finish(const cst_gemm_desc* d, const GemmRoute& r, const GemmParams& p, cst_stream stream, const GemmList* list = nullptr, int64_t nlist = 0) {
+  const int64_t nbatch = list ? nlist : d->batch0 * d->batch1;
   if (p.splits > 1 && d->defer_reduce) {
     CST_REQUIRE((nbatch == 1 || !d->colsum) && d->alpha == 1.0f && !d->bias && !d->act && !d->dact && !d->aux_out && !d->resid && d->drop_p == 0.0f && d->ldc == d->N &&
                     d->N % 8 == 0 && r.colsum != Colsum::Separate,
@@ -1170,7 +921,10 @@
     const int64_t work = (p.vec_epi && d->N % 8 == 0) ? total / 8 : total;
     int blocks = (int)(cst_ceil_div(work, 256) < 2048 ? cst_ceil_div(work, 256) : 2048);
     dim3 grid(blocks, (unsigned)nbatch);
-    if (d->dtype == CST_BF16) hipLaunchKernelGGL(splitk_reduce_kernel<bf16_t>, grid, dim3(256), 0, (hipStream_t)stream, p);
+    if (list) {
+      if (d->dtype == CST_BF16) hipLaunchKernelGGL(splitk_reduce_kernel_list<bf16_t>, grid, dim3(256), 0, (hipStream_t)stream, p, *list);
+      else hipLaunchKernelGGL(splitk_reduce_kernel_list<float>, grid, dim3(256), 0, (hipStream_t)stream, p, *list);
+    } else if (d->dtype == CST_BF16) hipLaunchKernelGGL(splitk_reduce_kernel<bf16_t>, grid, dim3(256), 0, (hipStream_t)stream, p);
     else hipLaunchKernelGGL(splitk_reduce_kernel<float>, grid, dim3(256), 0, (hipStream_t)stream, p);
     rc = cst_check_launch("cst_gemm split-k reduce");
   }
@@ -1182,23 +936,49 @@
   return rc;
 }
 
-int gemm_one(const cst_gemm_desc* d, cst_stream stream) {
-  int rc = validate(d);
+int gemm_one(const cst_gemm_desc* d0, const cst_gemm_problem* list, cst_stream stream) {
+  cst_gemm_desc view;
+  int rc = list_view(d0, list, view);
   if (rc != CST_OK) return rc;
+  const cst_gemm_desc* d = &view;
+  if ((rc = validate(d)) != CST_OK) return rc;
   const GemmSwitches sw = gemm_switches();
   GemmParams p = fill_params(d, sw);
   GemmRoute r;
-  if ((rc = take_route(d, sw, p, r)) != CST_OK) return rc;
+  const int64_t nbatch = list ? d0->batch0 : d->batch0 * d->batch1;
+  if ((rc = take_route(d, sw, p, r, list ? (nbatch < CST_GEMM_LIST_MAX ? nbatch : CST_GEMM_LIST_MAX) : 0)) != CST_OK) return rc;
   hipStream_t s = (hipStream_t)stream;
-  const int64_t nbatch = d->batch0 * d->batch1;
-  const Work w = credited_work(d, p, s);
+  Work w = credited_work(d, p, s);
+  if (list) { w.flops *= (double)nbatch; w.bytes *= (double)nbatch; }
   CstProfScope prof(CST_K_GEMM, s, w.flops, w.bytes);
-  rc = r.bf16 ? launch_route<bf16_t>(r, p, nbatch, s, sw) : launch_route<float>(r, p, nbatch, s, sw);
+  if (list) {
+    for (int64_t z0 = 0; z0 < nbatch && rc == CST_OK; z0 += CST_GEMM_LIST_MAX) {
+      const int64_t nz = nbatch - z0 < CST_GEMM_LIST_MAX ? nbatch - z0 : CST_GEMM_LIST_MAX;
+      GemmList l;
+      for (int64_t z = 0; z < CST_GEMM_LIST_MAX; ++z) {
+        const cst_gemm_problem& e = list[z0 + (z < nz ? z : 0)];
+        l.A[z] = e.A; l.B[z] = e.B; l.C[z] = e.C; l.colsum[z] = e.colsum;
+      }
+      const TileDims td = kTileDims[(int)r.tile];
+      GemmParams pc = p;
+      l.serial = 0;
+      if (r.splits > 1 && td.nt <= 256 && cst_ceil_div(d->M, td.bm) * cst_ceil_div(d->N, td.bn) * nz >= 128) {
+        l.serial = r.splits;
+        pc.splits = 1;
+        pc.ws = nullptr;
+        pc.colsum_ws = nullptr;
+      }
+      rc = r.bf16 ? launch_route<bf16_t>(r, pc, nz, s, sw, &l) : launch_route<float>(r, pc, nz, s, sw, &l);
+      if (rc == CST_OK) rc = finish(d, r, pc, stream, &l, nz);
+    }
+  } else {
+    rc = r.bf16 ? launch_route<bf16_t>(r, p, nbatch, s, sw) : launch_route<float>(r, p, nbatch, s, sw);
+  }
   if (cst_prof_is_on())
-    prof.tag("M=%lld N=%lld K=%lld b=%lld a%c b%c split=%d%s%s%s%s%s%s%s", (long long)d->M, (long long)d->N, (long long)d->K, (long long)nbatch, r.ak ? 'k' : 'm',
+    prof.tag("M=%lld N=%lld K=%lld b=%lld a%c b%c split=%d%s%s%s%s%s%s%s%s", (long long)d->M, (long long)d->N, (long long)d->K, (long long)nbatch, r.ak ? 'k' : 'm',
              r.bk ? 'k' : 'm', p.splits, d->bias ? " bias" : "", d->act ? " act" : "", d->aux_out ? " aux_out" : "", d->dact ? " dact" : "",
-             d->resid ? " resid" : "", d->drop_p > 0 ? " drop" : "", (d->k_live || d->m_live || d->k_len || d->m_len) ? " live" : "");
-  return rc != CST_OK ? rc : finish(d, r, p, stream);
+             d->resid ? " resid" : "", d->drop_p > 0 ? " drop" : "", (d->k_live || d->m_live || d->k_len || d->m_len) ? " live" : "", list ? " list" : "");
+  return rc != CST_OK || list ? rc : finish(d, r, p, stream);
 }
 
 GemmRoute query_route(const cst_gemm_desc* d) {
@@ -1228,4 +1008,9 @@
   return CST_OK;
 }
 
-extern "C" int cst_gemm(const cst_gemm_desc* d, cst_stream stream) { return gemm_one(d, stream); }
+extern "C" int cst_gemm(const cst_gemm_desc* d, cst_stream stream) { return gemm_one(d, nullptr, stream); }
+
+extern "C" int cst_gemm_list(const cst_gemm_desc* d, const cst_gemm_problem* list, cst_stream stream) {
+  CST_REQUIRE(list, "cst_gemm_list: null list");
+  return gemm_one(d, list, stream);
+}
diff --git a/chimera-st_amd/csrc/gemm_body.inc b/chimera-st_amd/csrc/gemm_body.inc
--- /dev/null
+++ b/chimera-st_amd/csrc/gemm_body.inc
@@ -0,0 +1,380 @@
+  constexpr bool SER = LIST && C::NT <= 256;
+  const int nsl = SER && serial > 1 ? serial : 0;
+  constexpr int BM = C::BM, BN = C::BN, NTHREADS = C::NT, TM = C::TM, TN = C::TN;
+  constexpr int VEC = DT<T>::VEC;
+  constexpr int KV = C::KV, BK = KV * VEC;
+  constexpr int LDK = BK + VEC;
+  constexpr int LDMA = sizeof(T) == 2 ? BM + 32 : BM + VEC;
+  constexpr int LDMB = sizeof(T) == 2 ? BN + 32 : BN + VEC;
+  constexpr int A_ELEMS = A_KMAJOR ? BM * LDK : BK * LDMA;
+  constexpr int B_ELEMS = B_KMAJOR ? BN * LDK : BK * LDMB;
+  constexpr int MVA = BM / VEC, MVB = BN / VEC;
+  constexpr int NVA = BM * KV / NTHREADS, NVB = BN * KV / NTHREADS;
+  extern __shared__ __attribute__((aligned(16))) char smem_raw[];
+  T* smem = reinterpret_cast<T*>(smem_raw);
+  constexpr int STAGE = A_ELEMS + B_ELEMS;
+
+  const int tid = threadIdx.x, lane = tid & 63, wave = tid >> 6;
+  const int wm = wave / C::WN, wn = wave % C::WN;
+
+  const int ntiles = p.tiles_m * p.tiles_n;
+  int tm, tn, z;
+  if (p.split_order) {
+    const int total = ntiles * p.splits, L = (int)blockIdx.x + (int)gridDim.x * (int)blockIdx.z;
+    const int q = total / 8, r = total % 8, xcd = L % 8, loc = L / 8;
+    const int item = (xcd < r ? xcd * (q + 1) : r * (q + 1) + (xcd - r) * q) + loc;
+    z = item / ntiles;
+    const int t = item % ntiles;
+    tm = t / p.tiles_n;
+    tn = t % p.tiles_n;
+  } else {
+    int id = blockIdx.x;
+    {
+      const int q = ntiles / 8, r = ntiles % 8, xcd = id % 8, loc = id / 8;
+      id = (xcd < r ? xcd * (q + 1) : r * (q + 1) + (xcd - r) * q) + loc;
+    }
+    constexpr int GROUP_M = 8;
+    const int per_group = GROUP_M * p.tiles_n;
+    const int grp = id / per_group, rem = id % per_group;
+    const int gm0 = grp * GROUP_M;
+    const int gsz = (p.tiles_m - gm0 < GROUP_M) ? (p.tiles_m - gm0) : GROUP_M;
+    tm = gm0 + rem % gsz;
+    tn = rem / gsz;
+    z = blockIdx.z;
+  }
+  const int64_t m0 = (int64_t)tm * BM, n0 = (int64_t)tn * BN;
+
+  const int split = z % p.splits;
+  const int64_t bidx = z / p.splits;
+  const int64_t b0 = bidx / p.batch1, b1 = bidx % p.batch1;
+  const T* A = (const T*)p.A + b0 * p.sa0 + b1 * p.sa1;
+  const T* B = (const T*)p.B + b0 * p.sb0 + b1 * p.sb1;
+  const int64_t cofs = b0 * p.sc0 + b1 * p.sc1;
+  const int64_t bofs = b0 * p.sbias0 + b1 * p.sbias1;
+
+  int ktiles = (int)((p.K + BK - 1) / BK);
+  const int kfull = (int)(p.K / BK);
+  if (p.k_len) {
+    typedef const __attribute__((address_space(4))) int32_t* cptr_t;
+    const int kl = ((cptr_t)p.k_len)[b0];
+    const int live = kl <= 0 ? 0 : (kl + BK - 1) / BK;
+    ktiles = live < ktiles ? live : ktiles;
+  }
+  const int per = nsl ? (ktiles + nsl - 1) / nsl : (ktiles + p.splits - 1) / p.splits;
+  const int kt0 = split * per;
+  const int kt1 = (kt0 + per < ktiles && !nsl) ? kt0 + per : ktiles;
+
+  u32x4 ra[NVA], rb[NVB];
+  const T* pa[NVA];
+  const T* pb[NVB];
+  int ka[NVA], kb[NVB];
+  int aq[NVA], ar[NVA], bq[NVB], br[NVB];
+#pragma unroll
+  for (int i = 0; i < NVA; ++i) {
+    const int v = tid + NTHREADS * i;
+    if (A_KMAJOR) {
+      int64_t row = m0 + v / KV;
+      row = row < p.M ? row : p.M - 1;
+      ka[i] = kt0 * BK + (v % KV) * VEC;
+      if (SEG && p.a_seg) { aq[i] = ka[i] / (int)p.a_seg; ar[i] = ka[i] % (int)p.a_seg; pa[i] = A + row * p.lda; }
+      else { aq[i] = 0; ar[i] = 0; pa[i] = A + row * p.lda + ka[i]; }
+    } else {
+      int64_t m = m0 + (int64_t)(v % MVA) * VEC;
+      m = m < p.M ? m : p.M - VEC;
+      ka[i] = kt0 * BK + v / MVA;
+      aq[i] = 0; ar[i] = 0;
+      pa[i] = A + (int64_t)ka[i] * p.lda + segaddr(m, p.a_seg, p.a_seg_stride);
+    }
+  }
+#pragma unroll
+  for (int i = 0; i < NVB; ++i) {
+    const int v = tid + NTHREADS * i;
+    if (B_KMAJOR) {
+      int64_t row = n0 + v / KV;
+      row = row < p.N ? row : p.N - 1;
+      kb[i] = kt0 * BK + (v % KV) * VEC;
+      if (SEG && p.b_seg) { bq[i] = kb[i] / (int)p.b_seg; br[i] = kb[i] % (int)p.b_seg; pb[i] = B + row * p.ldb; }
+      else { bq[i] = 0; br[i] = 0; pb[i] = B + row * p.ldb + kb[i]; }
+    } else {
+      int64_t n = n0 + (int64_t)(v % MVB) * VEC;
+      n = n < p.N ? n : p.N - VEC;
+      kb[i] = kt0 * BK + v / MVB;
+      bq[i] = 0; br[i] = 0;
+      pb[i] = B + (int64_t)kb[i] * p.ldb + segaddr(n, p.b_seg, p.b_seg_stride);
+    }
+  }
+  const int64_t step_a = A_KMAJOR ? (int64_t)BK : (int64_t)BK * p.lda;
+  const int64_t step_b = B_KMAJOR ? (int64_t)BK : (int64_t)BK * p.ldb;
+
+  auto load_tile = [&](auto tail_tag) {
+    constexpr bool TAIL = decltype(tail_tag)::value;
+    const u32x4 zero = {0, 0, 0, 0};
+#pragma unroll
+    for (int i = 0; i < NVA; ++i) {
+      const T* qa = pa[i];
+      if (SEG && A_KMAJOR && p.a_seg) qa = pa[i] + (int64_t)aq[i] * p.a_seg_stride + ar[i];
+      if (TAIL) {
+        const bool oka = ka[i] < p.K;
+        const u32x4 va = *reinterpret_cast<const u32x4*>(oka ? qa : A);
+        ra[i] = oka ? va : zero;
+      } else {
+        ra[i] = *reinterpret_cast<const u32x4*>(qa);
+      }
+      ka[i] += BK;
+      if (SEG && A_KMAJOR && p.a_seg) { ar[i] += BK; while (ar[i] >= (int)p.a_seg) { ar[i] -= (int)p.a_seg; ++aq[i]; } }
+      else pa[i] += step_a;
+    }
+#pragma unroll
+    for (int i = 0; i < NVB; ++i) {
+      const T* qb = pb[i];
+      if (SEG && B_KMAJOR && p.b_seg) qb = pb[i] + (int64_t)bq[i] * p.b_seg_stride + br[i];
+      if (TAIL) {
+        const bool okb = kb[i] < p.K;
+        const u32x4 vb = *reinterpret_cast<const u32x4*>(okb ? qb : B);
+        rb[i] = okb ? vb : zero;
+      } else {
+        rb[i] = *reinterpret_cast<const u32x4*>(qb);
+      }
+      kb[i] += BK;
+      if (SEG && B_KMAJOR && p.b_seg) { br[i] += BK; while (br[i] >= (int)p.b_seg) { br[i] -= (int)p.b_seg; ++bq[i]; } }
+      else pb[i] += step_b;
+    }
+  };
+  auto load_any = [&](int kt) {
+    if (kt < kfull) load_tile(std::false_type{});
+    else load_tile(std::true_type{});
+  };
+  static_assert(!CS || (!A_KMAJOR && NTHREADS % MVA == 0), "a thread must stage the same columns of an mn-major A in every vector");
+  const bool do_cs = CS && tn == 0;
+  float cs[VEC];
+#pragma unroll
+  for (int e = 0; e < VEC; ++e) cs[e] = 0.0f;
+  auto store_tile = [&](int buf) {
+#pragma unroll
+    for (int i = 0; i < NVA; ++i) {
+      const int v = tid + NTHREADS * i;
+      T* da = smem + buf * STAGE + (A_KMAJOR ? (v / KV) * LDK + (v % KV) * VEC : (v / MVA) * LDMA + (v % MVA) * VEC);
+      *reinterpret_cast<u32x4*>(da) = ra[i];
+      if (CS && do_cs) {
+        if (sizeof(T) == 2) {
+#pragma unroll
+          for (int e = 0; e < 4; ++e) {
+            cs[2 * e] += __uint_as_float(ra[i][e] << 16);
+            cs[2 * e + 1] += __uint_as_float(ra[i][e] & 0xffff0000u);
+          }
+        } else {
+#pragma unroll
+          for (int e = 0; e < 4; ++e) cs[e] += __uint_as_float(ra[i][e]);
+        }
+      }
+    }
+#pragma unroll
+    for (int i = 0; i < NVB; ++i) {
+      const int v = tid + NTHREADS * i;
+      T* db = smem + buf * STAGE + A_ELEMS + (B_KMAJOR ? (v / KV) * LDK + (v % KV) * VEC : (v / MVB) * LDMB + (v % MVB) * VEC);
+      *reinterpret_cast<u32x4*>(db) = rb[i];
+    }
+  };
+
+  f32x16 acc[TM][TN];
+#pragma unroll
+  for (int i = 0; i < TM; ++i)
+#pragma unroll
+    for (int j = 0; j < TN; ++j)
+#pragma unroll
+      for (int r = 0; r < 16; ++r) acc[i][j][r] = 0.0f;
+
+  constexpr int KLIST_MAX = 1000;
+  __shared__ int klist[KLIST_MAX];
+  __shared__ int klist_n;
+  const bool kskip = !SEG && BK == 64 && p.k_live != nullptr && per <= KLIST_MAX;
+  int nk = kt1 > kt0 ? kt1 - kt0 : 0;
+  if (kskip) {
+    if (wave == 0) {
+      int total = 0;
+      for (int base = 0; base < ktiles; base += 64) {
+        const int kt = base + lane;
+        total += __builtin_popcountll(__builtin_amdgcn_ballot_w64(kt < ktiles && p.k_live[kt] == p.k_epoch));
+      }
+      const int lo = (int)(((int64_t)total * split) / p.splits), hi = (int)(((int64_t)total * (split + 1)) / p.splits);
+      int seen = 0, n = 0;
+      for (int base = 0; base < ktiles && seen < hi; base += 64) {
+        const int kt = base + lane;
+        const bool live = kt < ktiles && p.k_live[kt] == p.k_epoch;
+        const uint64_t m = __builtin_amdgcn_ballot_w64(live);
+        const int idx = seen + __builtin_popcountll(m & ((1ull << lane) - 1ull));
+        if (live && idx >= lo && idx < hi) klist[idx - lo] = kt;
+        seen += __builtin_popcountll(m);
+      }
+      n = hi - lo;
+      if (lane == 0) klist_n = n;
+    }
+    __syncthreads();
+    nk = klist_n;
+  }
+  if (p.m_live) {
+    typedef const __attribute__((address_space(4))) uint32_t* cptr_t;
+    cptr_t ml = (cptr_t)p.m_live;
+    const int t0 = (int)(m0 >> 6), t1 = (int)((((m0 + BM < p.M) ? m0 + BM : p.M) + 63) >> 6);
+    bool live = false;
+    for (int t = t0; t < t1; ++t) live |= ml[t] == p.m_epoch;
+    if (!live) nk = 0;
+  }
+  if (p.m_len) {
+    typedef const __attribute__((address_space(4))) int32_t* cptr_t;
+    if (m0 >= (int64_t)((cptr_t)p.m_len)[b0]) nk = 0;
+  }
+  f32x16 tot[SER ? TM : 1][SER ? TN : 1];
+  float cstot = 0.0f;
+  if constexpr (SER) {
+#pragma unroll
+    for (int i = 0; i < TM; ++i)
+#pragma unroll
+      for (int j = 0; j < TN; ++j)
+#pragma unroll
+        for (int r = 0; r < 16; ++r) tot[i][j][r] = 0.0f;
+  }
+  __shared__ float sred[SER && CS ? C::NT / MVA : 1][SER && CS ? BM : 1];
+  auto fold = [&]() {
+    if constexpr (SER) {
+#pragma unroll
+      for (int i = 0; i < TM; ++i)
+#pragma unroll
+        for (int j = 0; j < TN; ++j)
+#pragma unroll
+          for (int r = 0; r < 16; ++r) { tot[i][j][r] += acc[i][j][r]; acc[i][j][r] = 0.0f; }
+      if constexpr (CS) {
+        if (do_cs) {
+#pragma unroll
+          for (int e = 0; e < VEC; ++e) { sred[tid / MVA][(tid % MVA) * VEC + e] = cs[e]; cs[e] = 0.0f; }
+          __syncthreads();
+          if (tid < BM) {
+            float t = 0.0f;
+            for (int r = 0; r < NTHREADS / MVA; ++r) t += sred[r][tid];
+            cstot += t;
+          }
+        }
+      }
+    }
+  };
+  int pos = kt0;
+  auto fetch = [&](int kt) {
+    const int d = kt - pos;
+    if (d) {
+#pragma unroll
+      for (int i = 0; i < NVA; ++i) { pa[i] += (int64_t)d * step_a; ka[i] += d * BK; }
+#pragma unroll
+      for (int i = 0; i < NVB; ++i) { pb[i] += (int64_t)d * step_b; kb[i] += d * BK; }
+    }
+    load_any(kt);
+    pos = kt + 1;
+  };
+  auto tile_at = [&](int it) { return kskip ? klist[it] : kt0 + it; };
+
+  if (nk > 0) {
+    fetch(tile_at(0));
+    store_tile(0);
+  }
+  __syncthreads();
+  int cur = 0;
+  const int lrow = lane & 31, lk = 8 * (lane >> 5);
+  constexpr int WROWS = TM * 32, WCOLS = TN * 32;
+  for (int it = 0; it < nk; ++it) {
+    const bool more = it + 1 < nk;
+    if (more) fetch(tile_at(it + 1));
+    const T* sa = smem + cur * STAGE;
+    const T* sb = sa + A_ELEMS;
+#pragma unroll
+    for (int kk = 0; kk < BK; kk += 16) {
+      Frag<T> fa[TM], fb[TN];
+#pragma unroll
+      for (int i = 0; i < TM; ++i) {
+        if (A_KMAJOR) frag_load_contig(fa[i], sa + (wm * WROWS + i * 32 + lrow) * LDK + kk + lk);
+        else frag_load_tr(fa[i], sa, LDMA, wm * WROWS + i * 32, kk + lk, kk + lk + 4, lane);
+      }
+#pragma unroll
+      for (int j = 0; j < TN; ++j) {
+        if (B_KMAJOR) frag_load_contig(fb[j], sb + (wn * WCOLS + j * 32 + lrow) * LDK + kk + lk);
+        else frag_load_tr(fb[j], sb, LDMB, wn * WCOLS + j * 32, kk + lk, kk + lk + 4, lane);
+      }
+#pragma unroll
+      for (int i = 0; i < TM; ++i)
+#pragma unroll
+        for (int j = 0; j < TN; ++j) mma16(acc[i][j], fa[i], fb[j]);
+    }
+    if (SER && nsl && more && (it + 1) % per == 0) fold();
+    if (more) store_tile(cur ^ 1);
+    __syncthreads();
+    cur ^= 1;
+  }
+  if constexpr (SER) {
+    if (nsl) {
+#pragma unroll
+      for (int i = 0; i < TM; ++i)
+#pragma unroll
+        for (int j = 0; j < TN; ++j)
+#pragma unroll
+          for (int r = 0; r < 16; ++r) acc[i][j][r] = tot[i][j][r] + acc[i][j][r];
+    }
+  }
+
+  if (CS && do_cs) {
+    float* red = reinterpret_cast<float*>(smem_raw);
+#pragma unroll
+    for (int e = 0; e < VEC; ++e) red[(tid / MVA) * BM + (tid % MVA) * VEC + e] = cs[e];
+    __syncthreads();
+    if (tid < BM && m0 + tid < p.M) {
+      float tot = 0.0f;
+      for (int r = 0; r < NTHREADS / MVA; ++r) tot += red[r * BM + tid];
+      if (SER && nsl) tot = cstot + tot;
+      if (p.splits > 1) p.colsum_ws[((int64_t)bidx * p.splits + split) * p.M + m0 + tid] = tot;
+      else DT<T>::st((T*)p.colsum + (LIST ? 0 : bidx) * p.M + m0 + tid, tot);
+    }
+  }
+
+  constexpr int LDC = BN + 4;
+  constexpr int VPR = BN / 8;
+  constexpr int NPASS = BM / 64;
+  constexpr int ITERS = 64 * VPR / NTHREADS;
+  float* stage = reinterpret_cast<float*>(smem_raw);
+  float* wsp = p.splits > 1 ? p.ws + ((int64_t)z) * p.M * p.N : nullptr;
+  const bool ws_vec = (p.N % 4) == 0;
+#pragma unroll
+  for (int ps = 0; ps < NPASS; ++ps) {
+    __syncthreads();
+#pragma unroll
+    for (int i = 0; i < TM; ++i) {
+      const int trow = wm * WROWS + i * 32;
+      if (trow / 64 == ps) {
+#pragma unroll
+        for (int j = 0; j < TN; ++j)
+#pragma unroll
+          for (int r = 0; r < 16; ++r)
+            stage[(trow - 64 * ps + acc_row(r, lane)) * LDC + wn * WCOLS + j * 32 + lrow] = acc[i][j][r];
+      }
+    }
+    __syncthreads();
+#pragma unroll 2
+    for (int it = 0; it < ITERS; ++it) {
+      const int v = tid + NTHREADS * it;
+      const int rl = v / VPR, cl = (v % VPR) * 8;
+      const int64_t row = m0 + 64 * ps + rl, col = n0 + cl;
+      if (row >= p.M || col >= p.N) continue;
+      float x[8];
+      {
+        const f32x4 a = *reinterpret_cast<const f32x4*>(stage + rl * LDC + cl);
+        const f32x4 b = *reinterpret_cast<const f32x4*>(stage + rl * LDC + cl + 4);
+        x[0] = a[0]; x[1] = a[1]; x[2] = a[2]; x[3] = a[3]; x[4] = b[0]; x[5] = b[1]; x[6] = b[2]; x[7] = b[3];
+      }
+      const bool full = col + 8 <= p.N;
+      if (wsp) {
+        if (full && ws_vec) store8(wsp + row * p.N + col, x);
+        else
+          for (int e = 0; e < 8 && col + e < p.N; ++e) wsp[row * p.N + col + e] = x[e];
+      } else if (full && p.vec_epi) {
+        epilogue_store8<T>(p, cofs, bofs, row, col, x);
+      } else {
+        for (int e = 0; e < 8 && col + e < p.N; ++e) epilogue_store<T>(p, cofs, bofs, row, col + e, x[e]);
+      }
+    }
+  }
diff --git a/chimera-st_amd/functional.py b/chimera-st_amd/functional.py
--- a/chimera-st_amd/functional.py
+++ b/chimera-st_amd/functional.py
@@ -199,6 +199,9 @@
     db = torch.empty(n_out, dtype=w.dtype, device=w.device) if db_in_dw else None
     may = allow_defer and _may_defer(w, bias_obj if db_in_dw else None)
     big = not may or not K.dw_colsum_is_fused(n_out, n_in, M, w.dtype) or dz_travels_on
+    if not big and live is None and K.DEFER.group:
+        K.DEFER.push_dw(dz, x2, dw, db, n_out, n_in, M)
+        return dw, db
     K.side_gemm(big, (dz, x2, live[0] if live is not None else None), dz, x2, dw, n_out, n_in, M, a_kmajor=0, b_kmajor=0, lda=n_out, ldb=n_in,
                 ldc=n_in, split_k=-1, k_live=live, colsum=db, defer=may)
     return dw, db
diff --git a/chimera-st_amd/kernels.py b/chimera-st_amd/kernels.py
--- a/chimera-st_amd/kernels.py
+++ b/chimera-st_amd/kernels.py
@@ -21,9 +21,12 @@
 class _Deferred:
 
     MAX_BYTES = 32 << 20
+    DW_MAX_BYTES = 4 << 30
 
     def __init__(self):
-        self.on, self.items, self.keep, self.flushes = 0, [], [], 0
+        self.on, self.reduces, self.keep, self.flushes = 0, [], [], 0
+        self.group = False
+        self.dw, self.dw_bytes, self.dw_cap = {}, 0, self.DW_MAX_BYTES
         self.main = None
         self.side = None
         self.side_used = False
@@ -34,20 +37,50 @@
             dst.fill_(float("nan"))
         if self.side_used and torch.is_tensor(keep) and torch.cuda.current_stream() != self.main:
             keep.record_stream(self.main)
-        self.items.append((src_ptr, dst.data_ptr(), stride, Lr, P, L.dtype_code(dst.dtype), order))
+        self.reduces.append((src_ptr, dst.data_ptr(), stride, Lr, P, L.dtype_code(dst.dtype), order))
         self.keep.append((keep, dst.detach()))
+
+    @property
+    def items(self):
+        return self.reduces + [t for probs in self.dw.values() for pr in probs for t in pr[2:] if t is not None]
 
     def join(self):
         if self.side_used:
             torch.cuda.current_stream().wait_stream(self.side)
             self.side_used = False
 
+    def push_dw(self, dz, x2, dw, db, n_out, n_in, rows):
+        if self.poison:
+            dw.fill_(float("nan"))
+            if db is not None:
+                db.fill_(float("nan"))
+        key = (n_out, n_in, rows, n_out, n_in, n_in, dz.dtype, dw.dtype, db is not None)
+        self.dw.setdefault(key, []).append((dz, x2, dw.detach(), None if db is None else db.detach()))
+        self.dw_bytes += dz.numel() * dz.element_size() + x2.numel() * x2.element_size()
+        if self.dw_bytes > self.dw_cap:
+            self.flush_dw()
+
+    def flush_dw(self):
+        groups, self.dw, self.dw_bytes = self.dw, {}, 0
+        for (M, N, Kd, lda, ldb, ldc, dt, cdt, has_cs), probs in groups.items():
+            at = 0
+            while at < len(probs):
+                n = _dw_group_size(M, N, len(probs) - at)
+                if n == 1:
+                    dz, x2, dw, db = probs[at]
+                    gemm(dz, x2, dw, M, N, Kd, a_kmajor=0, b_kmajor=0, lda=lda, ldb=ldb, ldc=ldc, split_k=-1, colsum=db, defer=True)
+                else:
+                    gemm_list(probs[at:at + n], M, N, Kd, lda=lda, ldb=ldb, ldc=ldc, split_k=-1)
+                at += n
+
     def flush(self):
         self.join()
-        if self.items:
-            reduce_multi(self.items)
+        if self.dw:
+            self.flush_dw()
+        if self.reduces:
+            reduce_multi(self.reduces)
             self.flushes += 1
-            self.items, self.keep = [], []
+            self.reduces, self.keep = [], []
 
 
 DEFER = _Deferred()
@@ -73,6 +106,8 @@
             DEFER.on += 1
             DEFER.main = torch.cuda.current_stream()
             DEFER.poison = bool(os.environ.get("CST_DEFER_POISON"))
+            DEFER.group = not os.environ.get("CST_NO_DW_GROUP") and not os.environ.get("CST_SIDE_STREAM")
+            DEFER.dw_cap = int(os.environ.get("CST_DW_GROUP_MAX_BYTES", _Deferred.DW_MAX_BYTES))
         return self
 
     def __exit__(self, *exc):
@@ -127,6 +162,7 @@
          b_seg_stride=0, split_k=-1, a_off=0, b_off=0, c_off=0, drop_p=0.0, drop_key=0, k_live=None, m_live=None, k_len=None, m_len=None,
          ws=None, colsum=None, defer=False, reduce_to=None):
     lib = L.load()
+    STATS["cst_gemm"] = STATS.get("cst_gemm", 0) + 1
     d = L.GemmDesc()
     d.dtype = L.dtype_code(A.dtype)
     assert B.dtype == A.dtype, "A/B dtype mismatch"
@@ -204,6 +240,44 @@
     return C
 
 
+def gemm_list(probs, M, N, K, *, lda, ldb, ldc, split_k=-1):
+    lib = L.load()
+    A0, _, C0, cs0 = probs[0]
+    d = L.GemmDesc()
+    d.dtype, d.c_dtype = L.dtype_code(A0.dtype), L.dtype_code(C0.dtype)
+    d.a_kmajor = d.b_kmajor = 0
+    d.M, d.N, d.K = M, N, K
+    d.lda, d.ldb, d.ldc = lda, ldb, ldc
+    d.alpha = 1.0
+    d.batch0 = d.batch1 = 1
+    d.split_k = split_k
+    d.colsum = None if cs0 is None else cs0.data_ptr()
+    need = lib.cst_gemm_workspace(ctypes.byref(d)) * min(len(probs), L.GEMM_LIST_MAX)
+    if need > 0:
+        ws = workspace(need, A0.device)
+        d.workspace, d.workspace_bytes = ws.data_ptr(), ws.numel()
+    d.batch0 = len(probs)
+    arr = (L.GemmProblem * len(probs))()
+    for e, (A, B, C, cs) in zip(arr, probs):
+        assert A.dtype == A0.dtype and B.dtype == A0.dtype and C.dtype == C0.dtype and (cs is None) == (cs0 is None)
+        assert cs is None or (cs.dtype == A0.dtype and cs.is_contiguous() and cs.numel() == M)
+        e.A, e.B, e.C, e.colsum = A.data_ptr(), B.data_ptr(), C.data_ptr(), None if cs is None else cs.data_ptr()
+    n = -(-len(probs) // L.GEMM_LIST_MAX)
+    STATS["cst_gemm"] = STATS.get("cst_gemm", 0) + n
+    STATS["cst_gemm_list"] = STATS.get("cst_gemm_list", 0) + n
+    L.check(lib.cst_gemm_list(ctypes.byref(d), arr, L.stream_ptr()), "cst_gemm_list")
+
+
+_CUS = []
+
+
+def _dw_group_size(M, N, avail):
+    if not _CUS:
+        _CUS.append(torch.cuda.get_device_properties(torch.cuda.current_device()).multi_processor_count)
+    tiles = -(-M // 128) * -(-N // 128)
+    return max(1, min(avail, L.GEMM_LIST_MAX, _CUS[0] // tiles))
+
+
 _DW_FUSED = {}
 
 
diff --git a/chimera-st_amd/lib.py b/chimera-st_amd/lib.py
--- a/chimera-st_amd/lib.py
+++ b/chimera-st_amd/lib.py
@@ -44,6 +44,13 @@
     ]
 
 
+GEMM_LIST_MAX = 32
+
+
+class GemmProblem(ctypes.Structure):
+    _fields_ = [("A", c_p), ("B", c_p), ("C", c_p), ("colsum", c_p)]
+
+
 class ReduceItem(ctypes.Structure):
     _fields_ = [("src", c_p), ("dst", c_p), ("stride", c_i64), ("L", c_i64), ("P", ctypes.c_int32), ("dst_dtype", ctypes.c_int32),
                 ("block0", ctypes.c_int32), ("order", ctypes.c_int32)]
@@ -142,6 +149,7 @@
     ("cst_gemm_route", c_int, [ctypes.POINTER(GemmDesc), ctypes.c_char_p, c_i64]),
     ("cst_reduce_multi", c_int, [ctypes.POINTER(ReduceItem), c_int, c_p]),
     ("cst_gemm", c_int, [ctypes.POINTER(GemmDesc), c_p]),
+    ("cst_gemm_list", c_int, [ctypes.POINTER(GemmDesc), ctypes.POINTER(GemmProblem), c_p]),
     ("cst_posconv_fwd", c_int, [c_p, c_p, c_p, c_p, c_p, c_p, c_i64, c_i64, c_i64, c_i64, c_i64, c_p]),
     ("cst_posconv_dx", c_int, [c_p, c_p, c_p, c_p, c_p, c_i64, c_i64, c_i64, c_i64, c_i64, c_p]),
     ("cst_posconv_dw", c_int, [c_p, c_p, c_p, c_p, c_p, ctypes.c_uint32, c_i64, c_i64, c_i64, c_i64, c_i64, c_p]),
diff --git a/include/cst.h b/include/cst.h
--- a/include/cst.h
+++ b/include/cst.h
@@ -47,6 +47,11 @@
 
 typedef enum { CST_ACT_NONE = 0, CST_ACT_RELU = 1, CST_ACT_GELU = 2 } cst_act;
 typedef enum { CST_BIAS_NONE = 0, CST_BIAS_COL = 1, CST_BIAS_ROW = 2 } cst_bias_mode;
+
+#define CST_GEMM_LIST_MAX 32
+typedef struct cst_gemm_problem {
+  const void* A; const void* B; void* C; void* colsum;
+} cst_gemm_problem;
 
 typedef struct {
   int dtype;
@@ -83,6 +88,7 @@
 int cst_gemm_route(const cst_gemm_desc* d, char* out, int64_t out_bytes);
 int cst_gemm_reserve_cus(int n);
 int cst_gemm(const cst_gemm_desc* d, cst_stream stream);
+int cst_gemm_list(const cst_gemm_desc* d, const cst_gemm_problem* list, cst_stream stream);
 
 int cst_posconv_fwd(const void* x, const void* w, const void* bias, void* y, void* z, const int32_t* m_len, int64_t B, int64_t T,
                     int64_t C, int64_t groups, int64_t k, cst_stream stream);
```

Measured after the change: 515.0 (median of 6 runs). 1.9% higher.
